# vocdoni/gnark-crypto-primitives

Hardware: AMD Instinct MI355X
Metric: proofs/sec, Arbo-160 Poseidon SMT-verifier circuit, Groth16/BN254 (higher is better)
Workload: dtype u32x8 Montgomery (254-bit integer)

## Files before the change

gnark_crypto_primitives_amd/csrc/api.hip:

```cpp
#include <algorithm>

#include "zkmi_internal.h"
#include "ff29.h"
#include "ec29.h"

using namespace zk;

namespace zk {

int ensure_scratch(zkmi_ctx* ctx, DevBuf& s, size_t bytes, void** out) {
  if (s.bytes < bytes) {
    if (s.p) {
      hipStreamSynchronize(ctx->stream);
      if (ctx->stream2) hipStreamSynchronize(ctx->stream2);
      if (ctx->stream3) hipStreamSynchronize(ctx->stream3);
      hipFree(s.p);
      s.p = nullptr;
      s.bytes = 0;
    }
    hipError_t e = hipMalloc(&s.p, bytes);
    if (e != hipSuccess) {
      ctx->err = "hipMalloc(" + std::to_string(bytes) + " B) failed: " + hipGetErrorString(e) +
                 " (the working set of this batch does not fit beside the MSM tables: load the key"
                 " with zkmi_pk_desc.max_batch >= the batch size, or with a table_budget_bytes cap)";
      s.p = nullptr;
      return ZKMI_ERR_OOM;
    }
    s.bytes = bytes;
  }
  if (out) *out = s.p;
  return ZKMI_OK;
}

int require_idle(zkmi_ctx* ctx) {
  if (!ctx->sets[0].pending && !ctx->sets[1].pending) return ZKMI_OK;
  ctx->err = "a submitted prove batch is in flight; collect it first";
  return ZKMI_ERR_ARG;
}

template <class P>
__global__ __launch_bounds__(256) void field_mul_kernel(const Fp<P>* a, const Fp<P>* b, Fp<P>* r,
                                                        size_t n) {
  size_t i = (size_t)blockIdx.x * blockDim.x + threadIdx.x;
  const size_t stride = (size_t)gridDim.x * blockDim.x;
  for (; i < n; i += stride) r[i] = mul(a[i], b[i]);
}

template <class P>
__global__ __launch_bounds__(256) void field_mul_bench_kernel(Fp<P>* io, int iters) {
  const size_t i = (size_t)blockIdx.x * blockDim.x + threadIdx.x;
  Fp<P> x = io[i], y = io[i];
  y.v[0] ^= 1;
  for (int k = 0; k < iters; k++) {
    x = mul(x, y);
    y = mul(y, x);
  }
  io[i] = add(x, y);
}

__global__ __launch_bounds__(256) void field_mul_bench_f29_kernel(Fq* io, int iters) {
  const size_t i = (size_t)blockIdx.x * blockDim.x + threadIdx.x;
  Fq29 x = unpack29<Fq29Params>(io[i].v), y = x;
  y.v[0] ^= 1;
  for (int k = 0; k < iters; k++) {
    x = mul(x, y);
    y = mul(y, x);
  }
  pack_canonical<Fq29Params>(io[i].v, norm(add(x, y)));
}

enum { FF29_MUL_ASM, FF29_SQR_ASM, FF29_MUL_ADD2_ASM, FF29_MUL_ASM_S, FF29_MUL, FF29_SQR,
       FF29_MUL_ADD2, FF29_MUL_ILP, FF29_WRED_PACK, FF29_PACK, FF29_N_OPS };
static constexpr int ff29_arity(int op) {
  if (op == FF29_MUL_ADD2_ASM || op == FF29_MUL_ADD2) return 4;
  if (op == FF29_SQR_ASM || op == FF29_SQR || op == FF29_WRED_PACK || op == FF29_PACK) return 1;
  return 2;
}
template <class P>
__device__ __forceinline__ F29<P> ld_raw29(const int32_t* p) {
  F29<P> r;
#pragma unroll
  for (int l = 0; l < 9; l++) r.v[l] = p[l];
  return r;
}
template <class P, int OP>
__global__ __launch_bounds__(64) void ff29_op_kernel(const int32_t* __restrict__ in,
                                                     int32_t* __restrict__ out, size_t n) {
#if defined(__HIP_DEVICE_COMPILE__)
  constexpr int AR = ff29_arity(OP);
  for (size_t w = blockIdx.x; w * 64 < n; w += gridDim.x) {
    F29<P> bs = F29<P>::zero();
    if constexpr (OP == FF29_MUL_ASM_S) bs = ld_raw29<P>(in + w * 64 * (AR * 9) + 9);
    const size_t i = w * 64 + threadIdx.x;
    if (i >= n) continue;
    const int32_t* e = in + i * (AR * 9);
    const F29<P> a = ld_raw29<P>(e);
    F29<P> r = F29<P>::zero();
    if constexpr (OP == FF29_MUL_ASM) r = mul_asm(a, ld_raw29<P>(e + 9));
    if constexpr (OP == FF29_SQR_ASM) r = sqr_asm(a);
    if constexpr (OP == FF29_MUL_ADD2_ASM)
      r = mul_add2_asm(a, ld_raw29<P>(e + 9), ld_raw29<P>(e + 18), ld_raw29<P>(e + 27));
    if constexpr (OP == FF29_MUL_ASM_S) r = mul_asm_s(a, bs);
    if constexpr (OP == FF29_MUL) r = mul(a, ld_raw29<P>(e + 9));
    if constexpr (OP == FF29_SQR) r = sqr(a);
    if constexpr (OP == FF29_MUL_ADD2)
      r = mul_add2(a, ld_raw29<P>(e + 9), ld_raw29<P>(e + 18), ld_raw29<P>(e + 27));
    if constexpr (OP == FF29_MUL_ILP) r = mul_ilp(a, ld_raw29<P>(e + 9));
    if constexpr (OP == FF29_WRED_PACK || OP == FF29_PACK) {
      uint32_t img[8];
      pack_canonical<P>(img, OP == FF29_WRED_PACK ? wred(a) : a);
#pragma unroll
      for (int l = 0; l < 8; l++) r.v[l] = (int32_t)img[l];
      r.v[8] = 0;
    }
#pragma unroll
    for (int l = 0; l < 9; l++) out[i * 9 + l] = r.v[l];
  }
#endif
}
typedef void (*ff29_kernel_t)(const int32_t*, int32_t*, size_t);
template <class P, int OP = 0>
static ff29_kernel_t ff29_kernel(int op) {
  if constexpr (OP < FF29_N_OPS)
    return op == OP ? ff29_op_kernel<P, OP> : ff29_kernel<P, OP + 1>(op);
  else
    return nullptr;
}

struct PkConsts {
  G1Affine alpha, beta1;
  G2Affine beta2;
};
struct ProofOut {
  G1Affine ar, krs;
  G2Affine bs;
};

__global__ __launch_bounds__(64) void rs_prep_kernel(Fr* rs, size_t Bp) {
  const size_t i = (size_t)blockIdx.x * blockDim.x + threadIdx.x;
  if (i >= Bp) return;
  bi_st(rs, 2, i, Bp, neg(mul(bi_ld(rs, 0, i, Bp), bi_ld(rs, 1, i, Bp))));
}

__device__ __forceinline__ void dbl29(G1Acc29& acc) {
  if (acc.inf) return;
  const Fq29 u = norm(add(acc.y, acc.y));
  const Fq29 v = msqr(u);
  const Fq29 w = mmul(u, v);
  const Fq29 s = mmul(acc.x, v);
  const Fq29 x2 = msqr(acc.x);
  const Fq29 m = norm(add(add(x2, x2), x2));
  const Fq29 x3 = norm(sub(msqr(m), add(s, s)));
  const Fq29 y3 = norm(sub(mmul(m, sub(s, x3)), mmul(w, acc.y)));
  acc.zz = mmul(v, acc.zz);
  acc.zzz = mmul(w, acc.zzz);
  acc.x = x3;
  acc.y = y3;
}

__global__ __launch_bounds__(64) void assemble_kernel(const G1XYZZ* sA, const G1XYZZ* sB1,
                                                      const G1XYZZ* sK, const G1XYZZ* sZ,
                                                      const G1XYZZ* tR, const G1XYZZ* tS,
                                                      const G1XYZZ* tNRS, const Fr* rs, size_t Bp,
                                                      PkConsts pk, ProofOut* out) {
  const size_t i = (size_t)blockIdx.x * blockDim.x + threadIdx.x;
  if (i >= Bp) return;
  const Fr r = from_mont(bi_ld(rs, 0, i, Bp)), s = from_mont(bi_ld(rs, 1, i, Bp));
  G1XYZZ AR = sA[i];
  madd(AR, pk.alpha);
  padd(AR, tR[i]);
  const G1Affine ar = to_affine(AR);
  G1XYZZ BS1 = sB1[i];
  madd(BS1, pk.beta1);
  padd(BS1, tS[i]);
  const G1Affine bs1 = to_affine(BS1);
  const bool ar_fin = !ar.is_inf(), bs_fin = !bs1.is_inf();
  const Fq29 ax = from_std<Fq29Params>(ar.x), ay = from_std<Fq29Params>(ar.y);
  const Fq29 bx = from_std<Fq29Params>(bs1.x), by = from_std<Fq29Params>(bs1.y);
  G1Acc29 acc29 = G1Acc29::infinity();
  for (int w = 7; w >= 0; w--) {
    const uint32_t sw = s.v[w], rw = r.v[w];
#pragma unroll 1
    for (int b = 31; b >= 0; b--) {
      dbl29(acc29);
      if (((sw >> b) & 1u) && ar_fin) madd29(acc29, ax, ay);
      if (((rw >> b) & 1u) && bs_fin) madd29(acc29, bx, by);
    }
  }
  G1XYZZ acc = to_std(acc29);
  padd(acc, sK[i]);
  padd(acc, sZ[i]);
  padd(acc, tNRS[i]);
  out[i].ar = ar;
  out[i].krs = to_affine(acc);
}

__global__ __launch_bounds__(64) void assemble_g2_kernel(const G2XYZZ* sB2, const G2XYZZ* tS2,
                                                         size_t Bp, G2Affine beta2, ProofOut* out) {
  const size_t i = (size_t)blockIdx.x * blockDim.x + threadIdx.x;
  if (i >= Bp) return;
  G2XYZZ BS = sB2[i];
  madd(BS, beta2);
  padd(BS, tS2[i]);
  out[i].bs = to_affine(BS);
}

struct SumsView {
  G1XYZZ *sA, *sB1, *sK, *sZ, *tR, *tS, *tNRS;
  G2XYZZ *sB2, *tS2;
  ProofOut* proofs;
  G1XYZZ* w1[4];
  G2XYZZ* w2;
  SumsView(void* base, size_t Bp) {
    char* m = (char*)base;
    sA = (G1XYZZ*)m;   m += Bp * 128;
    sB1 = (G1XYZZ*)m;  m += Bp * 128;
    sK = (G1XYZZ*)m;   m += Bp * 128;
    sZ = (G1XYZZ*)m;   m += Bp * 128;
    tR = (G1XYZZ*)m;   m += Bp * 128;
    tS = (G1XYZZ*)m;   m += Bp * 128;
    tNRS = (G1XYZZ*)m; m += Bp * 128;
    sB2 = (G2XYZZ*)m;  m += Bp * 256;
    tS2 = (G2XYZZ*)m;  m += Bp * 256;
    proofs = (ProofOut*)m;  m += Bp * 256;
    for (int i = 0; i < 4; i++) {
      w1[i] = (G1XYZZ*)m;
      m += 256 * Bp * 128;
    }
    w2 = (G2XYZZ*)m;
  }
};
static size_t sums_bytes(size_t Bp) { return Bp * (7 * 128 + 2 * 256 + 256 + 256 * (4 * 128 + 256)); }

struct SetBytes {
  size_t slots, abc, misc;
};
static SetBytes prove_set_bytes(size_t value_rows, size_t n, size_t n_staged, size_t batch, size_t Bp) {
  return {value_rows * Bp * 32, n * Bp * 32, Bp * (96 + 4) + batch * (n_staged * 32 + 64)};
}

int device_view(zkmi_ctx* ctx, const void* src, size_t bytes, void* stage, const void** out) {
  *out = src;
  if (pointer_kind(src) == PTR_DEVICE) return ZKMI_OK;
  ZK_HIP(hipMemcpyAsync(stage, src, bytes, hipMemcpyHostToDevice, ctx->stream));
  *out = stage;
  return ZKMI_OK;
}

int prove_set_begin(zkmi_ctx* ctx, const zkmi_pk* pk, size_t value_rows, size_t n_staged,
                    size_t batch, const void* rs, hipStream_t* main, char** stage) {
  zkmi_ctx::ProveSet& S = ctx->sets[ctx->next_submit];
  if (S.pending) {
    ctx->err = "prove: two batches already in flight; collect one first";
    return ZKMI_ERR_ARG;
  }
  const size_t Bp = round_up(batch, 64);
  const SetBytes sb = prove_set_bytes(value_rows, (size_t)1 << pk->log_n, n_staged, batch, Bp);
  int rc;
  for (zkmi_ctx::ProveSet* T : {&ctx->sets[ctx->next_submit ^ 1], &S}) {
    if (T->pending) continue;
    if ((rc = ensure_scratch(ctx, T->slots, sb.slots)) || (rc = ensure_scratch(ctx, T->a, sb.abc)) ||
        (rc = ensure_scratch(ctx, T->b, sb.abc)) || (rc = ensure_scratch(ctx, T->c, sb.abc)) ||
        (rc = ensure_scratch(ctx, T->misc, sb.misc)) ||
        (rc = ensure_scratch(ctx, T->sums, sums_bytes(Bp))))
      return rc;
  }
  char* const staged = (char*)S.misc.p + Bp * 100;
  S.rs = S.misc.p;
  S.st = (char*)S.misc.p + Bp * 96;
  if (stage) *stage = staged;
  S.heavy_enqueued = false;
  S.batch = batch;
  S.Bp = Bp;
  S.pk = pk;
  *main = ctx->stream;
  ctx->stream = ctx->stream2;
  hipEventRecord(S.ev0, ctx->stream);
  const void* rs_dev;
  rc = device_view(ctx, rs, batch * 64, staged + batch * n_staged * 32, &rs_dev);
  if (!rc) rc = transpose_in(ctx, rs_dev, S.rs, 2, batch, Bp, 32);
  return rc ? prove_set_end(ctx, *main, rc) : ZKMI_OK;
}

int prove_set_end(zkmi_ctx* ctx, hipStream_t main, int rc) {
  zkmi_ctx::ProveSet& S = ctx->sets[ctx->next_submit];
  hipEventRecord(S.ev1, ctx->stream);
  ctx->stream = main;
  if (rc) {
    hipStreamSynchronize(ctx->stream2);
    return rc;
  }
  S.pending = true;
  ctx->next_submit ^= 1;
  return ZKMI_OK;
}

}

extern "C" {

int zkmi_init(int device, zkmi_ctx** out) {
  if (!out) return ZKMI_ERR_ARG;
  *out = nullptr;
  int count = 0;
  if (hipGetDeviceCount(&count) != hipSuccess || count <= 0) return ZKMI_ERR_NO_DEVICE;
  if (device < 0 || device >= count) return ZKMI_ERR_ARG;
  if (hipSetDevice(device) != hipSuccess) return ZKMI_ERR_HIP;
  auto* ctx = new zkmi_ctx();
  ctx->device = device;
  if (hipStreamCreateWithFlags(&ctx->stream, hipStreamNonBlocking) != hipSuccess) {
    delete ctx;
    return ZKMI_ERR_HIP;
  }
  if (hipStreamCreateWithFlags(&ctx->stream2, hipStreamNonBlocking) != hipSuccess) {
    hipStreamDestroy(ctx->stream);
    delete ctx;
    return ZKMI_ERR_HIP;
  }
  if (hipStreamCreateWithFlags(&ctx->stream3, hipStreamNonBlocking) != hipSuccess) {
    hipStreamDestroy(ctx->stream2);
    hipStreamDestroy(ctx->stream);
    delete ctx;
    return ZKMI_ERR_HIP;
  }
  for (auto& st : ctx->sets) {
    hipEventCreate(&st.ev0);
    hipEventCreate(&st.ev1);
    for (auto& e : st.evq) hipEventCreate(&e);
    for (auto& e : st.eva) hipEventCreate(&e);
    for (auto& p : st.msm_ev) {
      hipEventCreate(&p[0]);
      hipEventCreate(&p[1]);
    }
  }
  for (auto& e : ctx->ev) hipEventCreate(&e);
  for (auto& e : ctx->part_ev) hipEventCreateWithFlags(&e, hipEventDisableTiming);
  for (auto& e : ctx->acc_ev) hipEventCreateWithFlags(&e, hipEventDisableTiming);
  ctx->plans.reserve(32);
  *out = ctx;
  return ZKMI_OK;
}

void zkmi_destroy(zkmi_ctx* ctx) {
  if (!ctx) return;
  hipSetDevice(ctx->device);
  hipStreamSynchronize(ctx->stream);
  hipStreamSynchronize(ctx->stream2);
  hipStreamSynchronize(ctx->stream3);
  for (auto& st : ctx->sets) {
    if (st.ev0) hipEventDestroy(st.ev0);
    if (st.ev1) hipEventDestroy(st.ev1);
    for (auto& e : st.evq)
      if (e) hipEventDestroy(e);
    for (auto& e : st.eva)
      if (e) hipEventDestroy(e);
    for (auto& p : st.msm_ev) {
      if (p[0]) hipEventDestroy(p[0]);
      if (p[1]) hipEventDestroy(p[1]);
    }
  }
  hipStreamDestroy(ctx->stream2);
  hipStreamDestroy(ctx->stream3);
  for (auto& p : ctx->plans) free_plan(p);
  for (auto& st : ctx->sets)
    for (DevBuf* b : {&st.slots, &st.a, &st.b, &st.c, &st.misc, &st.sums, &st.commit})
      if (b->p) hipFree(b->p);
  for (DevBuf* b : {&ctx->ntt_tmp, &ctx->build_tmp, &ctx->msm_digits, &ctx->msm_sint,
                    &ctx->msm_part[0], &ctx->msm_part[1], &ctx->side_part2, &ctx->side_part3})
    if (b->p) hipFree(b->p);
  witness_ring_free(ctx);
  for (auto& e : ctx->ev)
    if (e) hipEventDestroy(e);
  for (auto& e : ctx->part_ev)
    if (e) hipEventDestroy(e);
  for (auto& e : ctx->acc_ev)
    if (e) hipEventDestroy(e);
  hipStreamDestroy(ctx->stream);
  delete ctx;
}

const char* zkmi_last_error(zkmi_ctx* ctx) { return ctx ? ctx->err.c_str() : "null context"; }

int zkmi_sync(zkmi_ctx* ctx) {
  ZK_HIP(hipStreamSynchronize(ctx->stream));
  return ZKMI_OK;
}

void* zkmi_stream(zkmi_ctx* ctx) { return (void*)ctx->stream; }

int zkmi_field_mul(zkmi_ctx* ctx, int which, const void* a, const void* b, void* r, size_t n) {
  ZK_HIP(hipSetDevice(ctx->device));
  Staged sa(ctx), sb(ctx), sr(ctx);
  int rc;
  if ((rc = sa.in(a, n * 32)) || (rc = sb.in(b, n * 32)) || (rc = sr.out(r, n * 32))) return rc;
  if (n == 0) return ZKMI_OK;
  unsigned g = (unsigned)((n + 255) / 256);
  if (g > 8192) g = 8192;
  if (which == 0)
    hipLaunchKernelGGL((field_mul_kernel<FrParams>), dim3(g), dim3(256), 0, ctx->stream,
                       (const Fr*)sa.dev, (const Fr*)sb.dev, (Fr*)sr.dev, n);
  else
    hipLaunchKernelGGL((field_mul_kernel<FqParams>), dim3(g), dim3(256), 0, ctx->stream,
                       (const Fq*)sa.dev, (const Fq*)sb.dev, (Fq*)sr.dev, n);
  ZK_HIP(hipGetLastError());
  if ((rc = sr.finish())) return rc;
  ZK_HIP(hipStreamSynchronize(ctx->stream));
  return ZKMI_OK;
}

int zkmi_ff29_op(zkmi_ctx* ctx, int field, int op, const int32_t* in, int32_t* out, size_t n) {
  ZK_HIP(hipSetDevice(ctx->device));
  const ff29_kernel_t k = field == 0   ? ff29_kernel<Fr29Params>(op)
                          : field == 1 ? ff29_kernel<Fq29Params>(op)
                                       : nullptr;
  if (!k) {
    ctx->err = "ff29_op: field must be 0 (fr) or 1 (fq), op in [0, 9]";
    return ZKMI_ERR_ARG;
  }
  if (n == 0) return ZKMI_OK;
  Staged si(ctx), so(ctx);
  int rc;
  if ((rc = si.in(in, n * ff29_arity(op) * 36)) || (rc = so.out(out, n * 36))) return rc;
  const size_t waves = (n + 63) / 64;
  hipLaunchKernelGGL(k, dim3((unsigned)std::min(waves, (size_t)65536)), dim3(64), 0, ctx->stream,
                     (const int32_t*)si.dev, (int32_t*)so.dev, n);
  ZK_HIP(hipGetLastError());
  if ((rc = so.finish())) return rc;
  ZK_HIP(hipStreamSynchronize(ctx->stream));
  return ZKMI_OK;
}

int zkmi_field_mul_bench(zkmi_ctx* ctx, int which, size_t n_threads, int iters, double* rate) {
  ZK_HIP(hipSetDevice(ctx->device));
  int rc;
  if ((rc = require_idle(ctx))) return rc;
  n_threads = round_up(n_threads, 256);
  void* buf;
  if ((rc = ensure_scratch(ctx, ctx->sets[0].misc, n_threads * 32, &buf))) return rc;
  ZK_HIP(hipMemsetAsync(buf, 0x11, n_threads * 32, ctx->stream));
  auto launch = [&]() {
    if (which == 0)
      hipLaunchKernelGGL((field_mul_bench_kernel<FrParams>), dim3((unsigned)(n_threads / 256)),
                         dim3(256), 0, ctx->stream, (Fr*)buf, iters);
    else if (which == 2)
      hipLaunchKernelGGL(field_mul_bench_f29_kernel, dim3((unsigned)(n_threads / 256)), dim3(256),
                         0, ctx->stream, (Fq*)buf, iters);
    else
      hipLaunchKernelGGL((field_mul_bench_kernel<FqParams>), dim3((unsigned)(n_threads / 256)),
                         dim3(256), 0, ctx->stream, (Fq*)buf, iters);
  };
  launch();
  ZK_HIP(hipEventRecord(ctx->ev[6], ctx->stream));
  launch();
  ZK_HIP(hipEventRecord(ctx->ev[7], ctx->stream));
  ZK_HIP(hipEventSynchronize(ctx->ev[7]));
  float ms = 0;
  ZK_HIP(hipEventElapsedTime(&ms, ctx->ev[6], ctx->ev[7]));
  *rate = (double)n_threads * iters * 2.0 / (ms * 1e-3);
  return ZKMI_OK;
}

int zkmi_ntt_batch(zkmi_ctx* ctx, void* data, int log_n, size_t batch, int inverse, int coset) {
  ZK_HIP(hipSetDevice(ctx->device));
  int rc;
  if ((rc = require_idle(ctx))) return rc;
  if (batch == 0) return ZKMI_OK;
  NttPlan* plan;
  if ((rc = get_plan(ctx, log_n, &plan))) return rc;
  const size_t n = (size_t)1 << log_n, Bp = round_up(batch, 64);
  Staged sd(ctx), so(ctx);
  if ((rc = sd.in(data, batch * n * 32)) || (rc = so.out(data, batch * n * 32))) return rc;
  void *t0, *t1;
  if ((rc = ensure_scratch(ctx, ctx->sets[0].a, n * Bp * 32, &t0)) ||
      (rc = ensure_scratch(ctx, ctx->sets[0].b, n * Bp * 32, &t1)))
    return rc;
  if ((rc = transpose_in(ctx, sd.dev, t0, n, batch, Bp, 32))) return rc;
  if ((rc = ntt_bi(ctx, plan, (const Fr*)t0, (Fr*)t1, Bp, inverse != 0, coset != 0, n))) return rc;
  if ((rc = transpose_out(ctx, t1, so.dev, n, batch, Bp, 32))) return rc;
  if ((rc = so.finish())) return rc;
  ZK_HIP(hipStreamSynchronize(ctx->stream));
  return ZKMI_OK;
}

int zkmi_h_batch(zkmi_ctx* ctx, const void* a, const void* b, const void* c, void* h_out,
                 int log_n, size_t batch) {
  ZK_HIP(hipSetDevice(ctx->device));
  int rc;
  if ((rc = require_idle(ctx))) return rc;
  if (batch == 0) return ZKMI_OK;
  NttPlan* plan;
  if ((rc = get_plan(ctx, log_n, &plan))) return rc;
  const size_t n = (size_t)1 << log_n, Bp = round_up(batch, 64);
  Staged sa(ctx), sb(ctx), sc(ctx), sh(ctx);
  if ((rc = sa.in(a, batch * n * 32)) || (rc = sb.in(b, batch * n * 32)) ||
      (rc = sc.in(c, batch * n * 32)) || (rc = sh.out(h_out, batch * n * 32)))
    return rc;
  void* t[4];
  DevBuf* tb[4] = {&ctx->sets[0].a, &ctx->sets[0].b, &ctx->sets[0].c, &ctx->ntt_tmp};
  for (int i = 0; i < 4; i++)
    if ((rc = ensure_scratch(ctx, *tb[i], n * Bp * 32, &t[i]))) return rc;
  if ((rc = transpose_in(ctx, sa.dev, t[0], n, batch, Bp, 32)) ||
      (rc = transpose_in(ctx, sb.dev, t[1], n, batch, Bp, 32)) ||
      (rc = transpose_in(ctx, sc.dev, t[2], n, batch, Bp, 32)))
    return rc;
  Fr* h;
  if ((rc = compute_h_bi(ctx, plan, (Fr*)t[0], (Fr*)t[1], (Fr*)t[2], (Fr*)t[3], Bp, n, &h)))
    return rc;
  if ((rc = transpose_out(ctx, h, sh.dev, n, batch, Bp, 32))) return rc;
  if ((rc = sh.finish())) return rc;
  ZK_HIP(hipStreamSynchronize(ctx->stream));
  return ZKMI_OK;
}

int zkmi_ab_coset_batch(zkmi_ctx* ctx, const void* a, const void* b, void* out, int log_n,
                        size_t batch) {
  ZK_HIP(hipSetDevice(ctx->device));
  int rc;
  if ((rc = require_idle(ctx))) return rc;
  if (batch == 0) return ZKMI_OK;
  NttPlan* plan;
  if ((rc = get_plan(ctx, log_n, &plan))) return rc;
  const size_t n = (size_t)1 << log_n, Bp = round_up(batch, 64);
  Staged sa(ctx), sb(ctx), so(ctx);
  if ((rc = sa.in(a, batch * n * 32)) || (rc = sb.in(b, batch * n * 32)) ||
      (rc = so.out(out, batch * n * 32)))
    return rc;
  void* t[3];
  DevBuf* tb[3] = {&ctx->sets[0].a, &ctx->sets[0].b, &ctx->ntt_tmp};
  for (int i = 0; i < 3; i++)
    if ((rc = ensure_scratch(ctx, *tb[i], n * Bp * 32, &t[i]))) return rc;
  if ((rc = transpose_in(ctx, sa.dev, t[0], n, batch, Bp, 32)) ||
      (rc = transpose_in(ctx, sb.dev, t[1], n, batch, Bp, 32)))
    return rc;
  Fr* u;
  if ((rc = compute_ab_coset_bi(ctx, plan, (Fr*)t[0], (Fr*)t[1], (Fr*)t[2], Bp, n, &u))) return rc;
  if ((rc = transpose_out(ctx, u, so.dev, n, batch, Bp, 32))) return rc;
  if ((rc = so.finish())) return rc;
  ZK_HIP(hipStreamSynchronize(ctx->stream));
  return ZKMI_OK;
}

static int bases_load_plan(zkmi_ctx* ctx, int group, const void* bases_dev, size_t n, WinPlan plan,
                           bool may_relax, zkmi_msm_bases** out) {
  for (;;) {
    int rc = msm_bases_build(ctx, group, bases_dev, n, plan, out);
    if (rc != ZKMI_ERR_OOM || !may_relax) return rc;
    if (plan.comb) {
      if (plan.comb <= 8) return rc;
      plan = plan_comb(plan.comb - 1, plan.comb_signed != 0);
    } else if (plan.shared) {
      if (plan.bits[0] <= 4) return rc;
      plan = plan_shared(plan.bits[0] - 1);
    } else {
      if (plan.W >= 64) return rc;
      plan = plan_with_windows(plan.W + 1);
    }
  }
}

static bool window_bits_ok(int wb) {
  return wb == 0 || (wb >= 2 && wb <= 16) || (wb >= 104 && wb <= 116) ||
         (wb >= 202 && wb <= 220) || (wb >= 303 && wb <= 321);
}
static WinPlan plan_explicit(int wb) {
  return wb >= 300   ? plan_comb(wb - 300, true)
         : wb >= 200 ? plan_comb(wb - 200, false)
         : wb >= 100 ? plan_shared(wb - 100)
                     : plan_uniform(wb);
}
static double prove_working_set_bytes(uint32_t log_n, size_t n_slots, size_t n_in, size_t max_batch,
                                      size_t n_msm_max, size_t n_commitments) {
  const size_t Bp = round_up(max_batch ? max_batch : 1024, 64);
  const size_t n = (size_t)1 << log_n;
  const SetBytes sb = prove_set_bytes(n_slots, n, n_in, Bp, Bp);
  const double set = (double)(sb.slots + 3 * sb.abc + sb.misc + sums_bytes(Bp) +
                              commit_buffer_bytes(n_commitments, Bp));
  const double digits = 254.0 * (double)((n_msm_max + 15) / 16) * Bp * 4;
  const double sint = (double)n_msm_max * Bp * 32;
  const double partials = 2 * 21.0 * 254 * Bp * 256;
  const double ring = 3.0 * std::max(68e6, (double)n_in * 32 * 64);
  return 2 * set + (double)n * Bp * 32 + digits + sint + partials + ring + 2e9 + 1e9;
}
static double free_hbm_bytes() {
  size_t free_b = 0, total_b = 0;
  if (hipMemGetInfo(&free_b, &total_b) != hipSuccess) free_b = (size_t)64 << 30;
  return (double)free_b;
}
static double usable_table_bytes_standalone(size_t n) {
  const double ws = (double)n * 1024 * 32 * 2 + 254.0 * ((n + 15) / 16) * 1024 * 4 +
                    21.0 * 254 * 1024 * 256 + 3e9;
  const double usable = free_hbm_bytes() - ws;
  return usable > 0 ? usable : 0.0;
}

int zkmi_msm_bases_load(zkmi_ctx* ctx, int group, const void* bases, size_t n, int window_bits,
                        zkmi_msm_bases** out) {
  ZK_HIP(hipSetDevice(ctx->device));
  if (!out) return ZKMI_ERR_ARG;
  if (!window_bits_ok(window_bits)) {
    ctx->err = "window_bits must be 0 (auto), in [2,16], 100 + [4,16], 200 + [2,20] or 300 + [3,21]";
    return ZKMI_ERR_ARG;
  }
  Staged sb(ctx);
  int rc = sb.in(bases, n * (group == 1 ? 64 : 128));
  if (rc) return rc;
  WinPlan plan;
  if (window_bits) {
    plan = plan_explicit(window_bits);
  } else {
    const double usable = usable_table_bytes_standalone(n);
    plan = plan_windows_for_budget(n, group, (group == 1 ? 0.64 : 0.34) * usable);
    int c1, c2;
    plan_shared_for_budget(group == 1 ? n : 0, group == 2 ? n : 0, 0.9 * usable, &c1, &c2);
    const WinPlan ps = plan_shared(group == 1 ? c1 : c2);
    if (ps.W < plan.W) plan = ps;
    if (n >= 64) {
      int k1, k2;
      bool s1, s2;
      plan_comb_for_budget(group == 1 ? n : 0, group == 2 ? n : 0, 0.9 * usable, &k1, &k2, &s1, &s2);
      const int k = group == 1 ? k1 : k2;
      if ((double)COMB_W / k < (double)plan.W) plan = plan_comb(k, group == 1 ? s1 : s2);
    }
  }
  return bases_load_plan(ctx, group, sb.dev, n, plan, window_bits == 0, out);
}

void zkmi_msm_bases_free(zkmi_ctx* ctx, zkmi_msm_bases* b) {
  if (!b) return;
  if (ctx) {
    hipSetDevice(ctx->device);
    hipStreamSynchronize(ctx->stream);
  }
  if (b->table) hipFree(b->table);
  if (b->inf) hipFree(b->inf);
  delete b;
}

uint32_t zkmi_comb_min_groups_per_chunk(void) { return COMB_MIN_GROUPS_PER_CHUNK; }

int zkmi_msm_batch(zkmi_ctx* ctx, const zkmi_msm_bases* bases, const void* scalars, size_t batch,
                   void* out) {
  ZK_HIP(hipSetDevice(ctx->device));
  int rc;
  if ((rc = require_idle(ctx))) return rc;
  if (batch == 0) return ZKMI_OK;
  const size_t n = bases->n, Bp = round_up(batch, 64);
  const size_t pt = bases->group == 1 ? 64 : 128;
  Staged ss(ctx), so(ctx);
  if ((rc = ss.in(scalars, batch * n * 32)) || (rc = so.out(out, batch * pt))) return rc;
  void *sbi, *acc, *aff;
  if ((rc = ensure_scratch(ctx, ctx->sets[0].a, (n ? n : 1) * Bp * 32, &sbi)) ||
      (rc = ensure_scratch(ctx, ctx->sets[0].b, Bp * pt * 2, &acc)) ||
      (rc = ensure_scratch(ctx, ctx->sets[0].c, Bp * pt, &aff)))
    return rc;
  if ((rc = transpose_in(ctx, ss.dev, sbi, n, batch, Bp, 32))) return rc;
  if ((rc = msm_run(ctx, bases, (const Fr*)sbi, nullptr, Bp, batch, acc))) return rc;
  if ((rc = xyzz_to_affine(ctx, bases->group, acc, aff, Bp))) return rc;
  ZK_HIP(hipMemcpyAsync(so.dev, aff, batch * pt, hipMemcpyDeviceToDevice, ctx->stream));
  if ((rc = so.finish())) return rc;
  ZK_HIP(hipStreamSynchronize(ctx->stream));
  return ZKMI_OK;
}

int zkmi_fixed_base_mul(zkmi_ctx* ctx, int group, const void* base, const void* scalars, size_t n,
                        void* out) {
  ZK_HIP(hipSetDevice(ctx->device));
  int rc;
  if ((rc = require_idle(ctx))) return rc;
  if (n == 0) return ZKMI_OK;
  zkmi_msm_bases* b = nullptr;
  if ((rc = zkmi_msm_bases_load(ctx, group, base, 1, 8, &b))) return rc;
  const size_t Bp = round_up(n, 64);
  const size_t pt = group == 1 ? 64 : 128;
  Staged ss(ctx), so(ctx);
  void *sbi = nullptr, *acc = nullptr, *aff = nullptr;
  if ((rc = ss.in(scalars, n * 32)) || (rc = so.out(out, n * pt)) ||
      (rc = ensure_scratch(ctx, ctx->sets[0].a, Bp * 32, &sbi)) ||
      (rc = ensure_scratch(ctx, ctx->sets[0].b, Bp * pt * 2, &acc)) ||
      (rc = ensure_scratch(ctx, ctx->sets[0].c, Bp * pt, &aff))) {
    zkmi_msm_bases_free(ctx, b);
    return rc;
  }
  rc = transpose_in(ctx, ss.dev, sbi, 1, n, Bp, 32);
  if (!rc) rc = msm_run(ctx, b, (const Fr*)sbi, nullptr, Bp, n, acc);
  if (!rc) rc = xyzz_to_affine(ctx, group, acc, aff, Bp);
  if (!rc) {
    hipMemcpyAsync(so.dev, aff, n * pt, hipMemcpyDeviceToDevice, ctx->stream);
    rc = so.finish();
  }
  hipStreamSynchronize(ctx->stream);
  zkmi_msm_bases_free(ctx, b);
  return rc;
}

static int upload_u32(zkmi_ctx* ctx, const uint32_t* src, size_t n, uint32_t** out) {
  *out = nullptr;
  if (n == 0) return ZKMI_OK;
  ZK_HIP(hipMalloc((void**)out, n * 4));
  ZK_HIP(hipMemcpy(*out, src, n * 4, hipMemcpyDefault));
  return ZKMI_OK;
}

void zkmi_pk_free(zkmi_ctx* ctx, zkmi_pk* pk) {
  if (!pk) return;
  if (ctx) hipSetDevice(ctx->device);
  zkmi_msm_bases_free(ctx, pk->A);
  zkmi_msm_bases_free(ctx, pk->B1);
  zkmi_msm_bases_free(ctx, pk->K);
  zkmi_msm_bases_free(ctx, pk->Z);
  zkmi_msm_bases_free(ctx, pk->B2);
  zkmi_msm_bases_free(ctx, pk->D1);
  zkmi_msm_bases_free(ctx, pk->D2);
  commit_keys_free(ctx, pk);
  if (pk->idx3) hipFree(pk->idx3);
  if (pk->a_wire) hipFree(pk->a_wire);
  if (pk->b_wire) hipFree(pk->b_wire);
  if (pk->k_wire) hipFree(pk->k_wire);
  delete pk;
}

static int wires_from_infinity(zkmi_ctx* ctx, const uint8_t* inf, uint32_t n_wires, uint32_t want,
                               const char* name, std::vector<uint32_t>* out) {
  std::vector<uint8_t> host(n_wires);
  if (n_wires && hipMemcpy(host.data(), inf, n_wires, hipMemcpyDefault) != hipSuccess) {
    ctx->err = std::string("pk: cannot read ") + name;
    return ZKMI_ERR_HIP;
  }
  out->clear();
  for (uint32_t i = 0; i < n_wires; i++)
    if (!host[i]) out->push_back(i);
  if (out->size() != want) {
    ctx->err = std::string("pk: ") + name + " retains " + std::to_string(out->size()) +
               " wires but the key holds " + std::to_string(want) + " points";
    return ZKMI_ERR_ARG;
  }
  return ZKMI_OK;
}

int zkmi_pk_load(zkmi_ctx* ctx, const zkmi_pk_desc* d, zkmi_pk** out) {
  ZK_HIP(hipSetDevice(ctx->device));
  if (!d || !out) return ZKMI_ERR_ARG;
  if (d->log_n < 1 || d->log_n > 28) {
    ctx->err = "pk: log_n out of range [1,28]";
    return ZKMI_ERR_ARG;
  }
  if (d->n_z + 1 < (1u << d->log_n)) {
    ctx->err = "pk: n_z must be at least 2^log_n - 1";
    return ZKMI_ERR_ARG;
  }
  const uint32_t n_z = (1u << d->log_n) - 1;
  std::vector<uint32_t> wa, wb, wk;
  {
    int rc;
    struct { const uint32_t* p; uint32_t n; const char* name; std::vector<uint32_t>* v; } idx[3] = {
        {d->a_wire, d->n_a, "a_wire", &wa}, {d->b_wire, d->n_b, "b_wire", &wb},
        {d->k_wire, d->n_k, "k_wire", &wk}};
    for (auto& t : idx) {
      if (!t.p) continue;
      t.v->resize(t.n);
      if (t.n && hipMemcpy(t.v->data(), t.p, (size_t)t.n * 4, hipMemcpyDefault) != hipSuccess) {
        ctx->err = std::string("pk: cannot read ") + t.name;
        return ZKMI_ERR_HIP;
      }
    }
    if (!d->a_wire) {
      if (!d->infinity_a) {
        ctx->err = "pk: neither a_wire nor infinity_a given";
        return ZKMI_ERR_ARG;
      }
      if ((rc = wires_from_infinity(ctx, d->infinity_a, d->n_wires, d->n_a, "infinity_a", &wa)))
        return rc;
    }
    if (!d->b_wire) {
      if (!d->infinity_b) {
        ctx->err = "pk: neither b_wire nor infinity_b given";
        return ZKMI_ERR_ARG;
      }
      if ((rc = wires_from_infinity(ctx, d->infinity_b, d->n_wires, d->n_b, "infinity_b", &wb)))
        return rc;
    }
    if (!d->k_wire) {
      if (d->n_public < 1 || d->n_public > d->n_wires ||
          (d->n_commitments == 0 && d->n_wires - d->n_public != d->n_k)) {
        ctx->err = "pk: without k_wire, n_public must satisfy n_wires - n_public == n_k";
        return ZKMI_ERR_ARG;
      }
      std::vector<uint8_t> taken(d->n_wires, 0);
      for (uint32_t i = 0; i < d->n_commitments && d->commitments; i++) {
        const zkmi_commitment_desc& c = d->commitments[i];
        std::vector<uint32_t> pw(c.n_private);
        if (c.n_private && (!c.private_wires || hipMemcpy(pw.data(), c.private_wires, (size_t)c.n_private * 4,
                                                           hipMemcpyDefault) != hipSuccess)) {
          ctx->err = "pk: cannot read the private wires of commitment " + std::to_string(i);
          return ZKMI_ERR_ARG;
        }
        for (uint32_t w : pw)
          if (w < d->n_wires) taken[w] = 1;
        if (c.commitment_wire < d->n_wires) taken[c.commitment_wire] = 1;
      }
      wk.clear();
      for (uint32_t w = d->n_public; w < d->n_wires; w++)
        if (!taken[w]) wk.push_back(w);
      if (wk.size() != d->n_k) {
        ctx->err = "pk: n_k does not match n_wires - n_public - committed wires";
        return ZKMI_ERR_ARG;
      }
    }
    for (auto& t : idx)
      for (uint32_t w : *t.v)
        if (w >= d->n_wires) {
          ctx->err = std::string("pk: ") + t.name + " holds a wire index >= n_wires";
          return ZKMI_ERR_ARG;
        }
  }
  if (!window_bits_ok((int)d->window_bits_g1) || !window_bits_ok((int)d->window_bits_g2)) {
    ctx->err = "pk: window_bits must be 0 (auto), in [2,16], 100 + [4,16], 200 + [2,20] or 300 + [3,21]";
    return ZKMI_ERR_ARG;
  }
  if (d->msm_chunk_factor > 64) {
    ctx->err = "pk: msm_chunk_factor must be in [0,64]";
    return ZKMI_ERR_ARG;
  }
  FoldedKey fold;
  if (d->fold_r1cs) {
    const int frc = quotient_fold_key(ctx, d, wk, &fold);
    if (frc) return frc;
  }
  const uint32_t n_kb = fold.folded ? (uint32_t)fold.k_wire.size() : d->n_k;
  const uint32_t n_zb = fold.folded ? n_z + 1 : n_z;
  auto* pk = new zkmi_pk();
  pk->log_n = d->log_n;
  pk->n_wires = d->n_wires;
  pk->n_a = d->n_a;
  pk->n_b = d->n_b;
  pk->n_k = n_kb;
  pk->n_z = n_zb;
  pk->folded = fold.folded;
  pk->fold_n_constraints = fold.folded ? d->fold_r1cs->n_constraints : 0;
  pk->max_batch = d->max_batch ? d->max_batch : 1024;
  int rc;
  if ((rc = commit_keys_load(ctx, d, pk))) {
    zkmi_pk_free(ctx, pk);
    return rc;
  }
  const bool auto1 = d->window_bits_g1 == 0, auto2 = d->window_bits_g2 == 0;
  const size_t n1 = (size_t)d->n_a + d->n_b + n_kb + n_zb;
  const size_t n_msm_max = std::max(std::max((size_t)d->n_a, (size_t)d->n_b),
                                    std::max((size_t)n_kb, (size_t)n_zb));
  const size_t n_slots = d->n_slots_hint ? d->n_slots_hint : (size_t)d->n_wires + d->n_wires / 20;
  const double ws = prove_working_set_bytes(d->log_n, n_slots, d->n_wires, pk->max_batch, n_msm_max,
                                            pk->commits.size());
  double usable = free_hbm_bytes() - ws;
  if (usable < 0) usable = 0;
  if (d->table_budget_bytes && (double)d->table_budget_bytes < usable)
    usable = (double)d->table_budget_bytes;
  int sc1 = 0, sc2 = 0;
  plan_shared_for_budget(n1, d->n_b, 0.98 * usable, &sc1, &sc2);
  WinPlan p1 = auto1 ? plan_windows_for_budget(n1, 1, 0.64 * usable)
                     : plan_explicit((int)d->window_bits_g1);
  WinPlan p2 = auto2 ? plan_windows_for_budget(d->n_b, 2, 0.34 * usable)
                     : plan_explicit((int)d->window_bits_g2);
  if (auto1 && sc1 && plan_shared(sc1).W < p1.W) p1 = plan_shared(sc1);
  if (auto2 && sc2 && plan_shared(sc2).W < p2.W) p2 = plan_shared(sc2);
  if (n1 >= 4096) {
    int k1 = 0, k2 = 0;
    bool s1 = true, s2 = true;
    plan_comb_for_budget(auto1 ? n1 : 0, auto2 ? d->n_b : 0, 0.98 * usable, &k1, &k2, &s1, &s2,
                         d->sparse_witness == 0);
    if (auto1 && (double)COMB_W / k1 < (double)p1.W) p1 = plan_comb(k1, s1);
    if (auto2 && (double)COMB_W / k2 < (double)p2.W) p2 = plan_comb(k2, s2);
  }
  WinPlan p1z = p1;
  if (d->sparse_witness >= 2 && auto1 && auto2 && n1 >= 4096 && n_zb >= 4096) {
    const int kw = 12;
    const double wire_bytes =
        (double)((d->n_a + kw - 1) / kw + (d->n_b + kw - 1) / kw + (n_kb + kw - 1) / kw) *
            (double)(1u << kw) * 64.0 +
        (double)((d->n_b + kw - 1) / kw) * (double)(1u << kw) * 128.0;
    if (wire_bytes < 0.5 * usable) {
      int kz = 0, k2 = 0;
      bool sz = true, s2 = true;
      plan_comb_for_budget(n_zb, 0, 0.98 * usable - wire_bytes, &kz, &k2, &sz, &s2, true);
      p1 = plan_comb(kw, false);
      p2 = plan_comb(kw, false);
      p1z = plan_comb(kz, sz);
    }
  }
  auto load = [&](int group, const void* pts, size_t n, const WinPlan& plan, bool relax,
                  zkmi_msm_bases** out) -> int {
    Staged sb(ctx);
    int r = sb.in(pts, n * (group == 1 ? 64 : 128));
    if (r) return r;
    r = bases_load_plan(ctx, group, sb.dev, n, plan, relax, out);
    if (!r) (*out)->chunk_factor = d->msm_chunk_factor;
    return r;
  };
  if ((rc = upload_u32(ctx, wa.data(), d->n_a, &pk->a_wire)) ||
      (rc = upload_u32(ctx, wb.data(), d->n_b, &pk->b_wire)) ||
      (rc = upload_u32(ctx, fold.folded ? fold.k_wire.data() : wk.data(), n_kb, &pk->k_wire)) ||
      (rc = load(1, d->g1_a, d->n_a, p1, auto1, &pk->A)) ||
      (rc = load(1, d->g1_b, d->n_b, p1, auto1, &pk->B1)) ||
      (rc = load(1, fold.folded ? (const void*)fold.k.data() : d->g1_k, n_kb, p1, auto1, &pk->K)) ||
      (rc = load(1, fold.folded ? (const void*)fold.e.data() : d->g1_z, n_zb, p1z, auto1, &pk->Z)) ||
      (rc = load(2, d->g2_b, d->n_b, p2, auto2, &pk->B2))) {
    zkmi_pk_free(ctx, pk);
    return rc;
  }
  {
    const uint32_t idx[3] = {0, 1, 2};
    if ((rc = upload_u32(ctx, idx, 3, &pk->idx3)) ||
        (rc = zkmi_msm_bases_load(ctx, 1, d->g1_delta, 1, 8, &pk->D1)) ||
        (rc = zkmi_msm_bases_load(ctx, 2, d->g2_delta, 1, 8, &pk->D2))) {
      zkmi_pk_free(ctx, pk);
      return rc;
    }
    pk->D1->side = pk->D2->side = 2;
  }
  hipMemcpy(&pk->alpha, d->g1_alpha, 64, hipMemcpyDefault);
  hipMemcpy(&pk->beta1, d->g1_beta, 64, hipMemcpyDefault);
  hipMemcpy(&pk->delta1, d->g1_delta, 64, hipMemcpyDefault);
  hipMemcpy(&pk->beta2, d->g2_beta, 128, hipMemcpyDefault);
  hipMemcpy(&pk->delta2, d->g2_delta, 128, hipMemcpyDefault);
  *out = pk;
  return ZKMI_OK;
}

int zkmi_pk_info(const zkmi_pk* pk, uint64_t* info) {
  if (!pk || !info) return ZKMI_ERR_ARG;
  info[0] = (uint64_t)pk->Z->plan.W;
  info[1] = pk->Z->plan.per_base;
  info[2] = (uint64_t)pk->B2->plan.W;
  info[3] = pk->B2->plan.per_base;
  info[4] = pk->A->table_bytes + pk->B1->table_bytes + pk->K->table_bytes + pk->Z->table_bytes;
  info[5] = pk->B2->table_bytes;
  info[6] = pk->Z->plan.shared;
  info[7] = pk->B2->plan.shared;
  info[8] = pk->Z->plan.comb;
  info[9] = pk->B2->plan.comb;
  return ZKMI_OK;
}

int zkmi_pk_folded(const zkmi_pk* pk) { return pk && pk->folded ? 1 : 0; }

void zkmi_cs_free(zkmi_ctx* ctx, zkmi_cs* cs) {
  if (!cs) return;
  if (ctx) hipSetDevice(ctx->device);
  if (cs->program) hipFree(cs->program);
  if (cs->consts) hipFree(cs->consts);
  delete cs;
}

int zkmi_cs_load(zkmi_ctx* ctx, const zkmi_cs_desc* d, zkmi_cs** out) {
  ZK_HIP(hipSetDevice(ctx->device));
  if (!d || !out) return ZKMI_ERR_ARG;
  auto* cs = new zkmi_cs();
  const std::string err =
      vprog_validate({d->n_wires, d->n_slots, d->n_consts, d->n_constraints, d->n_rows,
                      d->lanes_per_proof},
                     d->program, &cs->commit_rows, &cs->has_emul);
  if (!err.empty()) {
    delete cs;
    ctx->err = err;
    return ZKMI_ERR_ARG;
  }
  cs->n_wires = d->n_wires;
  cs->n_public = d->n_public;
  cs->n_secret = d->n_secret;
  cs->n_constraints = d->n_constraints;
  cs->n_slots = d->n_slots;
  cs->n_rows = d->n_rows;
  cs->n_consts = d->n_consts;
  cs->lanes_per_proof = d->lanes_per_proof;
  int rc = upload_u32(ctx, d->program, (size_t)d->n_rows * (1 + d->lanes_per_proof) * 4,
                      &cs->program);
  if (rc) {
    delete cs;
    return rc;
  }
  if (d->n_consts) {
    if (hipMalloc((void**)&cs->consts, (size_t)d->n_consts * 32) != hipSuccess ||
        hipMemcpy(cs->consts, d->consts, (size_t)d->n_consts * 32, hipMemcpyDefault) !=
            hipSuccess) {
      ctx->err = "cs: constant pool upload failed";
      zkmi_cs_free(ctx, cs);
      return ZKMI_ERR_HIP;
    }
    if ((rc = array_to_f_domain(ctx, cs->consts, d->n_consts)) ||
        hipStreamSynchronize(ctx->stream) != hipSuccess) {
      zkmi_cs_free(ctx, cs);
      return rc ? rc : ZKMI_ERR_HIP;
    }
  }
  *out = cs;
  return ZKMI_OK;
}

static int stage_inputs(zkmi_ctx* ctx, const zkmi_cs* cs, const void* inputs_dev, size_t batch,
                        size_t Bp, Fr* slots) {
  const size_t n_in = cs->n_public - 1 + cs->n_secret;
  int rc = transpose_in(ctx, inputs_dev, slots + Bp, n_in, batch, Bp, 32);
  if (rc) return rc;
  return rows_to_f_domain(ctx, slots + Bp, n_in, Bp);
}

int zkmi_solve_batch(zkmi_ctx* ctx, const zkmi_cs* cs, const void* inputs, size_t batch,
                     void* wires_out, void* abc_out, int32_t* status_out) {
  ZK_HIP(hipSetDevice(ctx->device));
  int rc;
  if ((rc = require_idle(ctx))) return rc;
  if (batch == 0) return ZKMI_OK;
  if (!cs->commit_rows.empty()) {
    ctx->err = "solve_batch: this system has commitments; its commitment wires come from the "
               "proving key's Pedersen bases: use zkmi_prove_submit";
    return ZKMI_ERR_ARG;
  }
  const size_t Bp = round_up(batch, 64);
  const size_t n_in = cs->n_public - 1 + cs->n_secret;
  const size_t nc = cs->n_constraints ? cs->n_constraints : 1;
  Staged si(ctx), sw(ctx), sabc(ctx), sst(ctx);
  if ((rc = si.in(inputs, batch * n_in * 32))) return rc;
  if (wires_out && (rc = sw.out(wires_out, batch * (size_t)cs->n_wires * 32))) return rc;
  if (abc_out && (rc = sabc.out(abc_out, 3 * batch * (size_t)cs->n_constraints * 32))) return rc;
  if ((rc = sst.out(status_out, batch * 4))) return rc;
  void *slots, *a, *b, *c, *st;
  zkmi_ctx::ProveSet& S = ctx->sets[0];
  if ((rc = ensure_scratch(ctx, S.slots, (size_t)cs->n_slots * Bp * 32, &slots)) ||
      (rc = ensure_scratch(ctx, S.a, nc * Bp * 32, &a)) ||
      (rc = ensure_scratch(ctx, S.b, nc * Bp * 32, &b)) ||
      (rc = ensure_scratch(ctx, S.c, nc * Bp * 32, &c)) ||
      (rc = ensure_scratch(ctx, S.misc, Bp * 4, &st)))
    return rc;
  if ((rc = stage_inputs(ctx, cs, si.dev, batch, Bp, (Fr*)slots))) return rc;
  if ((rc = solve_bi(ctx, cs, (Fr*)slots, (Fr*)a, (Fr*)b, (Fr*)c, (int32_t*)st, Bp))) return rc;
  if (wires_out && ((rc = rows_to_std_domain(ctx, (Fr*)slots, cs->n_wires, Bp)) ||
                    (rc = transpose_out(ctx, slots, sw.dev, cs->n_wires, batch, Bp, 32))))
    return rc;
  if (abc_out) {
    if ((rc = rows_to_std_domain(ctx, (Fr*)a, cs->n_constraints, Bp)) ||
        (rc = rows_to_std_domain(ctx, (Fr*)b, cs->n_constraints, Bp)) ||
        (rc = rows_to_std_domain(ctx, (Fr*)c, cs->n_constraints, Bp)))
      return rc;
    const size_t stride = batch * (size_t)cs->n_constraints * 32;
    if ((rc = transpose_out(ctx, a, sabc.dev, cs->n_constraints, batch, Bp, 32)) ||
        (rc = transpose_out(ctx, b, (char*)sabc.dev + stride, cs->n_constraints, batch, Bp, 32)) ||
        (rc = transpose_out(ctx, c, (char*)sabc.dev + 2 * stride, cs->n_constraints, batch, Bp,
                            32)))
      return rc;
  }
  ZK_HIP(hipMemcpyAsync(sst.dev, st, batch * 4, hipMemcpyDeviceToDevice, ctx->stream));
  if ((rc = sw.finish()) || (rc = sabc.finish()) || (rc = sst.finish())) return rc;
  ZK_HIP(hipStreamSynchronize(ctx->stream));
  return ZKMI_OK;
}

int zkmi_prove_submit(zkmi_ctx* ctx, const zkmi_pk* pk, const zkmi_cs* cs, const void* inputs,
                      size_t batch, const void* rs) {
  ZK_HIP(hipSetDevice(ctx->device));
  if (batch == 0) {
    ctx->err = "prove: empty batch";
    return ZKMI_ERR_ARG;
  }
  if (pk->n_wires != cs->n_wires) {
    ctx->err = "prove: proving key and constraint system disagree on the number of wires";
    return ZKMI_ERR_ARG;
  }
  if (cs->n_constraints > (1u << pk->log_n)) {
    ctx->err = "prove: domain smaller than the number of constraints";
    return ZKMI_ERR_ARG;
  }
  if (pk->folded && cs->n_constraints != pk->fold_n_constraints) {
    ctx->err = "prove: the key was folded (zkmi_pk_desc.fold_r1cs) with a system of " +
               std::to_string(pk->fold_n_constraints) + " constraints, this one has " +
               std::to_string(cs->n_constraints);
    return ZKMI_ERR_ARG;
  }
  if (cs->commit_rows.size() != pk->commits.size()) {
    ctx->err = "prove: the constraint system has " + std::to_string(cs->commit_rows.size()) +
               " commitments, the proving key " + std::to_string(pk->commits.size());
    return ZKMI_ERR_ARG;
  }
  for (size_t i = 0; i < pk->commits.size(); i++)
    if (cs->commit_rows[i].second != pk->commits[i].wire) {
      ctx->err = "prove: commitment " + std::to_string(i) + " lands on different wires in the "
                 "constraint system and in the proving key";
      return ZKMI_ERR_ARG;
    }
  const size_t n_in = cs->n_public - 1 + cs->n_secret;
  hipStream_t main;
  char* stage;
  int rc = prove_set_begin(ctx, pk, cs->n_slots, n_in, batch, rs, &main, &stage);
  if (rc) return rc;
  zkmi_ctx::ProveSet& S = ctx->sets[ctx->next_submit];
  const size_t Bp = S.Bp;
  S.cs = cs;
  S.n_constraints = cs->n_constraints;
  S.f_domain = true;
  Fr *slots = (Fr*)S.slots.p, *a = (Fr*)S.a.p, *b = (Fr*)S.b.p, *c = (Fr*)S.c.p;
  int32_t* st = (int32_t*)S.st;
  const void* in_dev;
  rc = device_view(ctx, inputs, batch * n_in * 32, stage, &in_dev);
  if (!rc) rc = stage_inputs(ctx, cs, in_dev, batch, Bp, slots);
  if (!rc && cs->commit_rows.empty()) {
    rc = solve_bi(ctx, cs, slots, a, b, c, st, Bp);
  } else if (!rc) {
    rc = solve_init(ctx, slots, st, Bp);
    uint32_t begin = 0;
    for (size_t i = 0; !rc && i < cs->commit_rows.size(); i++) {
      rc = solve_rows(ctx, cs, slots, a, b, c, st, Bp, begin, cs->commit_rows[i].first);
      if (!rc) rc = commit_phase(ctx, S, (uint32_t)i, true);
      begin = cs->commit_rows[i].first + 1;
    }
    if (!rc) rc = solve_rows(ctx, cs, slots, a, b, c, st, Bp, begin, cs->n_rows);
    if (!rc) rc = commit_finish_submit(ctx, S);
  }
  return prove_set_end(ctx, main, rc);
}

static int enqueue_heavy(zkmi_ctx* ctx, int si) {
  zkmi_ctx::ProveSet& S = ctx->sets[si];
  const zkmi_pk* pk = S.pk;
  const bool fd = S.f_domain;
  const size_t Bp = S.Bp, batch = S.batch, n = (size_t)1 << pk->log_n;
  NttPlan* plan;
  int rc = get_plan(ctx, (int)pk->log_n, &plan);
  if (rc) return rc;
  void* t0;
  if ((rc = ensure_scratch(ctx, ctx->ntt_tmp, n * Bp * 32, &t0))) return rc;
  SumsView v(S.sums.p, Bp);
  Fr* rs_bi = (Fr*)S.rs;
  Fr* slots = (Fr*)S.slots.p;
  ZK_HIP(hipStreamWaitEvent(ctx->stream, S.ev1, 0));
  hipEventRecord(S.evq[0], ctx->stream);
  Fr* h;
  if ((rc = pk->folded ? compute_ab_coset_bi(ctx, plan, (Fr*)S.a.p, (Fr*)S.b.p, (Fr*)t0, Bp,
                                             S.n_constraints, &h, fd)
                       : compute_h_bi(ctx, plan, (Fr*)S.a.p, (Fr*)S.b.p, (Fr*)S.c.p, (Fr*)t0, Bp,
                                      S.n_constraints, &h, fd)))
    return rc;
  hipEventRecord(S.evq[1], ctx->stream);
  S.msm_ev_used = 0;
  ctx->msm_ev_set = si;
  const bool d1 = pk->Z->plan.shared || pk->Z->plan.comb;
  const bool d2 = pk->B2->plan.shared || pk->B2->plan.comb;
  hipStream_t q3 = ctx->stream3;
  if ((rc = msm_run(ctx, pk->A, slots, pk->a_wire, Bp, batch, v.sA, fd, d1 ? v.w1[0] : nullptr, q3)) ||
      (rc = msm_run(ctx, pk->B1, slots, pk->b_wire, Bp, batch, v.sB1, fd, d1 ? v.w1[1] : nullptr, q3)) ||
      (rc = msm_run(ctx, pk->K, slots, pk->k_wire, Bp, batch, v.sK, fd, d1 ? v.w1[2] : nullptr, q3)) ||
      (rc = msm_run(ctx, pk->Z, h, nullptr, Bp, batch, v.sZ, false, d1 ? v.w1[3] : nullptr, q3))) {
    ctx->msm_ev_set = -1;
    return rc;
  }
  hipEventRecord(S.evq[2], ctx->stream);
  rc = msm_run(ctx, pk->B2, slots, pk->b_wire, Bp, batch, v.sB2, fd, d2 ? v.w2 : nullptr, q3);
  ctx->msm_ev_set = -1;
  if (rc) return rc;
  hipEventRecord(S.evq[3], ctx->stream);
  {
    hipStream_t main_stream = ctx->stream;
    ZK_HIP(hipStreamWaitEvent(q3, S.ev1, 0));
    ctx->stream = q3;
    hipLaunchKernelGGL(rs_prep_kernel, dim3((unsigned)(Bp / 64)), dim3(64), 0, q3, rs_bi, Bp);
    (void)((rc = msm_run(ctx, pk->D1, rs_bi, pk->idx3 + 0, Bp, batch, v.tR)) ||
           (rc = msm_run(ctx, pk->D1, rs_bi, pk->idx3 + 1, Bp, batch, v.tS)) ||
           (rc = msm_run(ctx, pk->D1, rs_bi, pk->idx3 + 2, Bp, batch, v.tNRS)) ||
           (rc = msm_run(ctx, pk->D2, rs_bi, pk->idx3 + 1, Bp, batch, v.tS2)));
    ctx->stream = main_stream;
    if (rc) return rc;
  }
  if ((rc = commit_pok(ctx, S))) return rc;
  hipEventRecord(S.evq[4], ctx->stream);
  S.heavy_enqueued = true;
  return ZKMI_OK;
}

int zkmi_prove_collect(zkmi_ctx* ctx, void* proofs_out, int32_t* status_out) {
  return zkmi_prove_collect_ex(ctx, proofs_out, status_out, nullptr);
}

int zkmi_prove_collect_ex(zkmi_ctx* ctx, void* proofs_out, int32_t* status_out,
                          void* commitments_out) {
  ZK_HIP(hipSetDevice(ctx->device));
  const int si = ctx->next_collect;
  zkmi_ctx::ProveSet& S = ctx->sets[si];
  if (!S.pending) {
    ctx->err = "prove: nothing submitted";
    return ZKMI_ERR_ARG;
  }
  if (!S.pk->commits.empty() && !commitments_out) {
    ctx->err = "prove: this key has commitments: collect with zkmi_prove_collect_ex";
    return ZKMI_ERR_ARG;
  }
  const zkmi_pk* pk = S.pk;
  const size_t batch = S.batch, Bp = S.Bp;
  int rc;
  if (!S.heavy_enqueued && (rc = enqueue_heavy(ctx, si))) return rc;
  SumsView v(S.sums.p, Bp);
  hipStream_t q3 = ctx->stream3;
  ZK_HIP(hipStreamWaitEvent(q3, S.evq[4], 0));
  hipEventRecord(S.eva[0], q3);
  if (pk->Z->plan.shared || pk->Z->plan.comb) {
    void* ws[4] = {v.w1[0], v.w1[1], v.w1[2], v.w1[3]};
    void* os[4] = {v.sA, v.sB1, v.sK, v.sZ};
    const zkmi_msm_bases* ms[4] = {pk->A, pk->B1, pk->K, pk->Z};
    bool same = true;
    for (int i = 0; i < 3; i++)
      same = same && ms[i]->plan.bits[0] == pk->Z->plan.bits[0] &&
             ms[i]->plan.comb == pk->Z->plan.comb &&
             ms[i]->plan.comb_signed == pk->Z->plan.comb_signed;
    if (same) {
      if ((rc = msm_horner_run(ctx, q3, 4, ms, ws, os, Bp))) return rc;
    } else {
      for (int i = 0; i < 4; i++)
        if ((rc = msm_horner_run(ctx, q3, 1, ms + i, ws + i, os + i, Bp))) return rc;
    }
  }
  if (pk->B2->plan.shared || pk->B2->plan.comb) {
    void* ws[1] = {v.w2};
    void* os[1] = {v.sB2};
    const zkmi_msm_bases* ms[1] = {pk->B2};
    if ((rc = msm_horner_run(ctx, q3, 1, ms, ws, os, Bp))) return rc;
  }
  PkConsts pc{pk->alpha, pk->beta1, pk->beta2};
  hipLaunchKernelGGL(assemble_kernel, dim3((unsigned)(Bp / 64)), dim3(64), 0, q3, v.sA, v.sB1, v.sK,
                     v.sZ, v.tR, v.tS, v.tNRS, (const Fr*)S.rs, Bp, pc, v.proofs);
  hipLaunchKernelGGL(assemble_g2_kernel, dim3((unsigned)(Bp / 64)), dim3(64), 0, q3, v.sB2, v.tS2,
                     Bp, pk->beta2, v.proofs);
  ZK_HIP(hipGetLastError());
  ZK_HIP(hipMemcpyAsync(proofs_out, v.proofs, batch * 256, hipMemcpyDefault, q3));
  ZK_HIP(hipMemcpyAsync(status_out, S.st, batch * 4, hipMemcpyDefault, q3));
  if (const size_t nc = pk->commits.size()) {
    const size_t pitch = (nc + 1) * 64;
    for (size_t i = 0; i < nc; i++)
      ZK_HIP(hipMemcpy2DAsync((char*)commitments_out + i * 64, pitch,
                              (const char*)S.commit_pts + i * Bp * 64, 64, 64, batch, hipMemcpyDefault, q3));
    ZK_HIP(hipMemcpy2DAsync((char*)commitments_out + nc * 64, pitch,
                            (const char*)S.commit_pok + Bp * 128, 64, 64, batch, hipMemcpyDefault, q3));
  }
  hipEventRecord(S.eva[1], q3);
  zkmi_ctx::ProveSet& N = ctx->sets[si ^ 1];
  if (N.pending && !N.heavy_enqueued && (rc = enqueue_heavy(ctx, si ^ 1))) return rc;
  ZK_HIP(hipEventSynchronize(S.eva[1]));
  S.pending = false;
  S.heavy_enqueued = false;
  ctx->next_collect ^= 1;
  float ms = 0;
  hipEventElapsedTime(&ms, S.ev0, S.ev1);
  ctx->timings[0] = ms;
  for (int i = 0; i < 3; i++) {
    hipEventElapsedTime(&ms, S.evq[i], S.evq[i + 1]);
    ctx->timings[1 + i] = ms;
  }
  hipEventElapsedTime(&ms, S.eva[0], S.eva[1]);
  ctx->timings[4] = ms;
  hipEventElapsedTime(&ms, S.evq[0], S.evq[4]);
  ctx->timings[5] = ms;
  ctx->timings[6] = ctx->timings[7] = 0;
  for (int i = 0; i < S.msm_ev_used; i++) {
    hipEventElapsedTime(&ms, S.msm_ev[i][0], S.msm_ev[i][1]);
    ctx->timings[S.msm_ev_group[i] == 1 ? 6 : 7] += ms;
  }
  return ZKMI_OK;
}

int zkmi_prove_batch(zkmi_ctx* ctx, const zkmi_pk* pk, const zkmi_cs* cs, const void* inputs,
                     size_t batch, const void* rs, void* proofs_out, int32_t* status_out) {
  if (batch == 0) return ZKMI_OK;
  int rc;
  if ((rc = require_idle(ctx)) || (rc = zkmi_prove_submit(ctx, pk, cs, inputs, batch, rs))) return rc;
  return zkmi_prove_collect(ctx, proofs_out, status_out);
}

int zkmi_last_timings(zkmi_ctx* ctx, double* ms_out) {
  for (int i = 0; i < 8; i++) ms_out[i] = ctx->timings[i];
  return ZKMI_OK;
}

}
```

gnark_crypto_primitives_amd/csrc/msm.hip:

```cpp
#include "msm_impl.h"

namespace zk {

WinPlan plan_with_windows(int W) {
  WinPlan p;
  if (W < 16) W = 16;
  if (W > 64) W = 64;
  p.W = W;
  const int c0 = 255 / W, rem = 255 - c0 * W;
  uint32_t off = 0;
  for (int j = 0; j < W; j++) {
    p.bits[j] = (uint8_t)(j < rem ? c0 + 1 : c0);
    p.off[j] = off;
    off += 1u << (p.bits[j] - 1);
  }
  p.per_base = off;
  return p;
}
WinPlan plan_uniform(int c) {
  WinPlan p;
  p.W = (255 + c - 1) / c;
  uint32_t off = 0;
  for (int j = 0; j < p.W; j++) {
    p.bits[j] = (uint8_t)c;
    p.off[j] = off;
    off += 1u << (c - 1);
  }
  p.per_base = off;
  return p;
}
WinPlan plan_shared(int c) {
  WinPlan p;
  if (c < 4) c = 4;
  if (c > 16) c = 16;
  p.shared = 1;
  p.W = (255 + c - 1) / c;
  for (int j = 0; j < p.W; j++) {
    p.bits[j] = (uint8_t)(j + 1 < p.W ? c : 255 - (p.W - 1) * c);
    p.off[j] = 0;
  }
  p.per_base = 1u << (c - 1);
  return p;
}
WinPlan plan_comb(int k, bool signed_tables) {
  WinPlan p;
  if (k < 2) k = 2;
  if (k > 21) k = 21;
  if (!signed_tables && k > 20) k = 20;
  p.comb = (uint8_t)k;
  p.comb_signed = signed_tables ? 1 : 0;
  p.W = COMB_W + (signed_tables ? 1 : 0);
  p.per_base = 0;
  return p;
}
void plan_comb_for_budget(size_t n1, size_t n2, double usable_bytes, int* k1, int* k2, bool* sg1,
                          bool* sg2, bool allow_signed) {
  double best = 1e300;
  *k1 = *k2 = 8;
  *sg1 = *sg2 = allow_signed;
  for (int s1 = 0; s1 < (allow_signed ? 2 : 1); s1++)
    for (int s2 = 0; s2 < (allow_signed ? 2 : 1); s2++)
      for (int a = 8; a <= (s1 ? 21 : 20); a++)
        for (int b = 8; b <= (s2 ? 21 : 20); b++) {
          const double g1 = (double)((n1 + a - 1) / a), g2 = (double)((n2 + b - 1) / b);
          const double bytes = g1 * (double)(1u << (a - s1)) * 64.0 + g2 * (double)(1u << (b - s2)) * 128.0;
          if (bytes > usable_bytes) continue;
          const double cost = g1 * (s1 ? 255 * 62.8 : 254 * 61.1) + g2 * (s2 ? 255 * 178.5 : 254 * 171.6);
          if (cost < best) {
            best = cost;
            *k1 = a;
            *k2 = b;
            *sg1 = s1 != 0;
            *sg2 = s2 != 0;
          }
        }
}
void plan_shared_for_budget(size_t n1, size_t n2, double usable_bytes, int* c1, int* c2) {
  double best = 1e300;
  *c1 = *c2 = 4;
  for (int a = 4; a <= 16; a++)
    for (int b = 4; b <= 16; b++) {
      const double bytes = (double)n1 * (1u << (a - 1)) * 64.0 + (double)n2 * (1u << (b - 1)) * 128.0;
      if (bytes > usable_bytes) continue;
      const double cost = (double)n1 * ((255 + a - 1) / a) + 3.0 * (double)n2 * ((255 + b - 1) / b);
      if (cost < best) {
        best = cost;
        *c1 = a;
        *c2 = b;
      }
    }
}
WinPlan plan_windows_for_budget(size_t n_total, int group, double budget_bytes) {
  const double entry = group == 1 ? 64.0 : 128.0;
  for (int W = 16; W <= 64; W++) {
    WinPlan p = plan_with_windows(W);
    if ((double)n_total * p.per_base * entry <= budget_bytes) return p;
  }
  return plan_with_windows(64);
}

extern template int build_comb<Fq2>(zkmi_ctx*, const Affine<Fq2>*, size_t, const WinPlan&,
                                    Affine<Fq2>*, int*, Affine<Fq2>*);
extern template int build_impl<Fq2>(zkmi_ctx*, const Affine<Fq2>*, size_t, const WinPlan&,
                                    Affine<Fq2>*);
extern template int run_impl<Fq2>(zkmi_ctx*, const zkmi_msm_bases*, const Fr*, const uint32_t*,
                                  size_t, size_t, XYZZ<Fq2>*, bool, XYZZ<Fq2>*, hipStream_t);

template <class Fn>
static auto by_group(int group, Fn&& fn) {
  return group == 1 ? fn(Fq{}) : fn(Fq2{});
}

int msm_bases_build(zkmi_ctx* ctx, int group, const void* bases_dev, size_t n, const WinPlan& plan,
                    zkmi_msm_bases** out) {
  if (group != 1 && group != 2) {
    ctx->err = "group must be 1 (G1) or 2 (G2)";
    return ZKMI_ERR_ARG;
  }
  auto* b = new zkmi_msm_bases();
  b->group = group;
  b->n = n;
  b->plan = plan;
  const size_t entry = group == 1 ? sizeof(G1Affine) : sizeof(G2Affine);
  b->n_groups = plan.comb ? (n + plan.comb - 1) / plan.comb : 0;
  b->table_bytes = plan.comb ? b->n_groups * ((size_t)1 << (plan.comb - plan.comb_signed)) * entry
                             : n * (size_t)plan.per_base * entry;
  if (n == 0) {
    *out = b;
    return ZKMI_OK;
  }
  hipError_t e = hipMalloc(&b->table, b->table_bytes);
  if (e != hipSuccess) {
    (void)hipGetLastError();
    ctx->err = "hipMalloc of MSM window table failed (" + std::to_string(b->table_bytes) +
               " bytes): " + hipGetErrorString(e);
    delete b;
    return ZKMI_ERR_OOM;
  }
  if (hipMalloc(&b->inf, n) != hipSuccess) {
    (void)hipGetLastError();
    hipFree(b->table);
    delete b;
    return ZKMI_ERR_OOM;
  }
  const int rc = by_group(group, [&](auto f) {
    using F = decltype(f);
    const Affine<F>* bases = (const Affine<F>*)bases_dev;
    hipLaunchKernelGGL((msm_inf_flags<F>), dim3((unsigned)((n + 255) / 256)), dim3(256), 0,
                       ctx->stream, bases, (uint32_t)n, b->inf);
    return plan.comb ? build_comb<F>(ctx, bases, n, plan, (Affine<F>*)b->table,
                                     &b->entries_may_be_inf, &stotal_of(b, f))
                     : build_impl<F>(ctx, bases, n, plan, (Affine<F>*)b->table);
  });
  if (rc) {
    hipFree(b->table);
    hipFree(b->inf);
    delete b;
    return rc;
  }
  *out = b;
  return ZKMI_OK;
}

int msm_horner_run(zkmi_ctx* ctx, hipStream_t stream, int count,
                   const zkmi_msm_bases* const* bases, void* const* wsums, void* const* outs,
                   size_t Bp) {
  if (count < 1 || count > 4) return ZKMI_ERR_ARG;
  const WinPlan& plan = bases[0]->plan;
  by_group(bases[0]->group, [&](auto f) {
    using F = decltype(f);
    if (plan.comb) {
      HornerArgsRW<F> hw{};
      for (int i = 0; i < count; i++) {
        hw.wsum[i] = (XYZZ<F>*)wsums[i];
        hw.out[i] = (XYZZ<F>*)outs[i];
        hw.stotal[i] = stotal_of(bases[i], f);
      }
      launch_comb_horner<F>(stream, hw, count, Bp, plan);
    } else {
      HornerArgs<F> ha{};
      for (int i = 0; i < count; i++) {
        ha.wsum[i] = (const XYZZ<F>*)wsums[i];
        ha.out[i] = (XYZZ<F>*)outs[i];
      }
      hipLaunchKernelGGL((msm_horner<F>), dim3((unsigned)(Bp / 64), (unsigned)count), dim3(64), 0,
                         stream, ha, Bp, plan);
    }
  });
  ZK_HIP(hipGetLastError());
  return ZKMI_OK;
}

int msm_run(zkmi_ctx* ctx, const zkmi_msm_bases* bases, const Fr* scalars, const uint32_t* row_idx,
            size_t Bp, size_t batch, void* out_xyzz, bool scalars_f, void* wsum_out,
            hipStream_t finish_stream) {
  return by_group(bases->group, [&](auto f) -> int {
    using F = decltype(f);
    if (bases->n == 0) {
      const bool sums = wsum_out && (bases->plan.shared || bases->plan.comb);
      const size_t cnt = sums ? (size_t)bases->plan.W * Bp : Bp;
      hipLaunchKernelGGL((fill_inf<F>), dim3((unsigned)((cnt + 63) / 64)), dim3(64), 0, ctx->stream,
                         (XYZZ<F>*)(sums ? wsum_out : out_xyzz), cnt);
      ZK_HIP(hipGetLastError());
      return ZKMI_OK;
    }
    if (batch == 0 || batch > Bp) {
      ctx->err = "msm: batch must be in [1, Bp]";
      return ZKMI_ERR_ARG;
    }
    return run_impl<F>(ctx, bases, scalars, row_idx, Bp, batch, (XYZZ<F>*)out_xyzz, scalars_f,
                       (XYZZ<F>*)wsum_out, finish_stream);
  });
}

int xyzz_to_affine(zkmi_ctx* ctx, int group, const void* in, void* out, size_t n) {
  if (n == 0) return ZKMI_OK;
  by_group(group, [&](auto f) {
    using F = decltype(f);
    hipLaunchKernelGGL((xyzz_to_affine_kernel<F>), dim3((unsigned)((n + 63) / 64)), dim3(64), 0,
                       ctx->stream, (const XYZZ<F>*)in, (Affine<F>*)out, n);
  });
  ZK_HIP(hipGetLastError());
  return ZKMI_OK;
}

}
```

gnark_crypto_primitives_amd/csrc/msm_g2.hip:

```cpp
#include "msm_impl.h"

namespace zk {

template int build_comb<Fq2>(zkmi_ctx*, const Affine<Fq2>*, size_t, const WinPlan&, Affine<Fq2>*,
                             int*, Affine<Fq2>*);
template int build_impl<Fq2>(zkmi_ctx*, const Affine<Fq2>*, size_t, const WinPlan&, Affine<Fq2>*);
template int run_impl<Fq2>(zkmi_ctx*, const zkmi_msm_bases*, const Fr*, const uint32_t*, size_t,
                           size_t, XYZZ<Fq2>*, bool, XYZZ<Fq2>*, hipStream_t);

}
```

gnark_crypto_primitives_amd/csrc/msm_impl.h:

```cpp
#pragma once
#include "zkmi_internal.h"
#include "ec29.h"

namespace zk {

ZK_HD Fq to_r261_domain(const Fq& x) {
  Fq k;
#pragma unroll
  for (int i = 0; i < 8; i++) k.v[i] = Fq29Params::k261(i);
  return mul(x, k);
}
ZK_HD Fq2 to_r261_domain(const Fq2& x) { return Fq2{to_r261_domain(x.c0), to_r261_domain(x.c1)}; }

template <class F>
struct SegInv {
  F *szz, *szzz, *spre;
  size_t T;
  F pref = F::one();
  __device__ SegInv(F* scratch, uint32_t t, uint32_t T_, uint32_t seg_len)
      : szz(scratch + t), szzz(scratch + (size_t)seg_len * T_ + t),
        spre(scratch + (size_t)2 * seg_len * T_ + t), T(T_) {}
  __device__ void push(Affine<F>* seg, uint32_t d, const F& x, const F& y, const F& zz,
                       const F& zzz) {
    seg[d].x = x;
    seg[d].y = y;
    szz[d * T] = zz;
    szzz[d * T] = zzz;
    spre[d * T] = pref;
    pref = mul(pref, zzz);
  }
  __device__ void finish(Affine<F>* seg, uint32_t len) {
    F inv = inverse(pref);
    for (uint32_t d = len; d-- > 0;) {
      const F zzz = szzz[d * T];
      const F izzz = mul(inv, spre[d * T]);
      inv = mul(inv, zzz);
      const F izz = sqr(mul(izzz, szz[d * T]));
      seg[d].x = to_r261_domain(mul(seg[d].x, izz));
      seg[d].y = to_r261_domain(mul(seg[d].y, izzz));
    }
    pref = F::one();
  }
};

template <class F>
__global__ __launch_bounds__(64) void msm_build_table(const Affine<F>* __restrict__ bases,
                                                      uint64_t r0, uint64_t n_rows, WinPlan plan,
                                                      Affine<F>* __restrict__ table,
                                                      F* __restrict__ scratch, uint32_t T,
                                                      uint32_t seg_len) {
  const uint32_t t = blockIdx.x * blockDim.x + threadIdx.x;
  const uint64_t r = r0 + t;
  if (t >= T || r >= n_rows) return;
  uint32_t D;
  Affine<F>* row;
  Affine<F> Q;
  if (plan.shared) {
    D = plan.per_base;
    row = table + (size_t)r * plan.per_base;
    Q = bases[r];
  } else {
    const uint32_t i = (uint32_t)(r / (uint32_t)plan.W), j = (uint32_t)(r % (uint32_t)plan.W);
    D = 1u << (plan.bits[j] - 1);
    row = table + (size_t)i * plan.per_base + plan.off[j];
    Q = bases[i];
    if (!Q.is_inf() && j) {
      uint32_t shift = 0;
      for (uint32_t k = 0; k < j; k++) shift += plan.bits[k];
      XYZZ<F> a = XYZZ<F>::from_affine(Q);
      for (uint32_t k = 0; k < shift; k++) a = dbl(a);
      Q = to_affine(a);
    }
  }
  if (Q.is_inf()) {
    for (uint32_t d = 0; d < D; d++) row[d] = Affine<F>::inf();
    return;
  }
  SegInv<F> inv(scratch, t, T, seg_len);
  XYZZ<F> acc = XYZZ<F>::inf();
  for (uint32_t s0 = 0; s0 < D; s0 += seg_len) {
    Affine<F>* seg = row + s0;
    const uint32_t len = D - s0 < seg_len ? D - s0 : seg_len;
    for (uint32_t d = 0; d < len; d++) {
      madd(acc, Q);
      inv.push(seg, d, acc.x, acc.y, acc.zz, acc.zzz);
    }
    inv.finish(seg, len);
  }
}

template <class F> struct Acc29;
template <> struct Acc29<Fq> {
  typedef G1Acc29 type;
  static __device__ __forceinline__ void add(G1Acc29& acc, const G1Affine& e, bool negd) {
    madd29(acc, unpack29<Fq29Params>(e.x.v), cneg(unpack29<Fq29Params>(e.y.v), negd));
  }
};
template <> struct Acc29<Fq2> {
  typedef G2Acc29 type;
  static __device__ __forceinline__ void add(G2Acc29& acc, const G2Affine& e, bool negd) {
    madd29(acc, unpack2_29(e.x), cneg(unpack2_29(e.y), negd));
  }
};

template <class F> struct CombAcc;
template <> struct CombAcc<Fq> {
  static constexpr int LDS_ROWS = 1;
  typedef G1Acc29 type;
  static __device__ __forceinline__ type init(int32_t (*)[256], uint32_t) { return G1Acc29::infinity(); }
  static __device__ __forceinline__ void add(type& acc, const G1Affine& e, bool negd,
                                             int32_t (*)[256], uint32_t) {
    Acc29<Fq>::add(acc, e, negd);
  }
  static __device__ __forceinline__ Part29<Fq> result(const type& acc, int32_t (*)[256], uint32_t) {
    return pack_part(acc);
  }
};
struct G2AccL {
  Fq2_29 x, y;
  bool inf;
};
static __device__ __forceinline__ Fq2_29 lds_ld2(int32_t (*z)[256], int row0, uint32_t t) {
  Fq2_29 r;
#pragma unroll
  for (int l = 0; l < 9; l++) {
    r.c0.v[l] = z[row0 + l][t];
    r.c1.v[l] = z[row0 + 9 + l][t];
  }
  return r;
}
static __device__ __forceinline__ void lds_st2(int32_t (*z)[256], int row0, uint32_t t,
                                               const Fq2_29& a) {
#pragma unroll
  for (int l = 0; l < 9; l++) {
    z[row0 + l][t] = a.c0.v[l];
    z[row0 + 9 + l][t] = a.c1.v[l];
  }
}
template <> struct CombAcc<Fq2> {
  static constexpr int LDS_ROWS = 36;
  typedef G2AccL type;
  static __device__ __forceinline__ type init(int32_t (*)[256], uint32_t) {
    G2AccL a;
    a.x = a.y = Fq2_29::zero();
    a.inf = true;
    return a;
  }
  static __device__ __forceinline__ void add(type& acc, const G2Affine& e, bool negd,
                                             int32_t (*z)[256], uint32_t t) {
    const Fq2_29 qx = unpack2_29(e.x), qy = cneg(unpack2_29(e.y), negd);
    if (acc.inf) {
      acc.x = qx;
      acc.y = norm(qy);
      lds_st2(z, 0, t, Fq2_29::one());
      lds_st2(z, 18, t, Fq2_29::one());
      acc.inf = false;
      return;
    }
    const Fq2_29 u2 = mmul(qx, lds_ld2(z, 0, t));
    const Fq2_29 s2 = mmul(qy, lds_ld2(z, 18, t));
    const Fq2_29 p = sub(u2, acc.x);
    const Fq2_29 r = sub(s2, acc.y);
    const Fq2_29 pp = msqr(p);
    const Fq2_29 rr = msqr(r);
    if (is_zero_mulout(pp)) {
      if (is_zero_mulout(rr)) {
        G2Acc29 d;
        d.inf = false;
        mdbl29(d, qx, qy);
        acc.x = d.x;
        acc.y = d.y;
        lds_st2(z, 0, t, d.zz);
        lds_st2(z, 18, t, d.zzz);
      } else {
        acc.inf = true;
      }
      return;
    }
    const Fq2_29 ppp = mmul(p, pp);
    const Fq2_29 q = mmul(acc.x, pp);
    const Fq2_29 x3 = wred(sub(sub(rr, ppp), zk::add(q, q)));
    const Fq2_29 y3 = wred(sub(mmul(r, sub(q, x3)), mmul(acc.y, ppp)));
    uint32_t t2 = t;
    asm volatile("" : "+v"(t2));
    lds_st2(z, 0, t2, mmul(lds_ld2(z, 0, t2), pp));
    lds_st2(z, 18, t2, mmul(lds_ld2(z, 18, t2), ppp));
    acc.x = x3;
    acc.y = y3;
  }
  static __device__ __forceinline__ Part29<Fq2> result(const type& acc, int32_t (*z)[256], uint32_t t) {
    G2Acc29 a = G2Acc29::infinity();
    if (!acc.inf) {
      a.x = acc.x;
      a.y = acc.y;
      a.zz = lds_ld2(z, 0, t);
      a.zzz = lds_ld2(z, 18, t);
      a.inf = false;
    }
    return pack_part(a);
  }
};

template <class F, bool ONE_BASE>
__global__ __launch_bounds__(256) __attribute__((amdgpu_waves_per_eu(2))) void msm_accumulate(const Affine<F>* __restrict__ table,
                                                      const Fr* __restrict__ scalars,
                                                      const uint32_t* __restrict__ row_idx,
                                                      size_t Bp, uint32_t n, uint32_t per_chunk,
                                                      WinPlan plan, Part29<F>* __restrict__ partial,
                                                      Fr kmul, const uint8_t* __restrict__ inf) {
  const size_t b = (size_t)blockIdx.x * blockDim.x + threadIdx.x;
  const uint32_t chunk = blockIdx.y;
  const uint32_t i0 = chunk * per_chunk;
  uint32_t i1 = i0 + per_chunk;
  if (i1 > n) i1 = n;
  const int W = plan.W;
  typename Acc29<F>::type acc = Acc29<F>::type::infinity();
  for (uint32_t i = i0; i < i1; i++) {
    if (inf[i]) continue;
    const uint32_t row = row_idx ? row_idx[i] : i;
    Fr s = mul(bi_ld(scalars, row, b, Bp), kmul);
    if (s.is_zero()) continue;
    const Affine<F>* trow = table + (size_t)i * plan.per_base;
    uint32_t carry = 0;
    for (int j = 0; j < W; j++) {
      const int c = plan.bits[j];
      const uint32_t mask = (1u << c) - 1u;
      const uint32_t half = 1u << (c - 1);
      uint32_t d = (s.v[0] & mask) + carry;
#pragma unroll
      for (int l = 0; l < 7; l++) s.v[l] = (s.v[l] >> c) | (s.v[l + 1] << (32 - c));
      s.v[7] >>= c;
      const bool negd = d > half;
      carry = negd ? 1u : 0u;
      const uint32_t mag = negd ? (mask + 1u - d) : d;
      if (mag) {
        const Affine<F> e = trow[plan.off[j] + (mag - 1)];
        Acc29<F>::add(acc, e, negd);
      }
    }
  }
  partial[(size_t)chunk * Bp + b] = pack_part(acc);
}

static __global__ __launch_bounds__(256) void msm_digits_kernel(const Fr* __restrict__ scalars,
                                                         const uint32_t* __restrict__ row_idx,
                                                         size_t Bp, uint32_t n, WinPlan plan,
                                                         int32_t kmul32, Fr koff,
                                                         const uint8_t* __restrict__ inf,
                                                         int16_t* __restrict__ digits) {
  const size_t b = (size_t)blockIdx.x * blockDim.x + threadIdx.x;
  for (uint32_t i = blockIdx.y; i < n; i += gridDim.y) {
    if (inf[i]) {
      for (int j = 0; j < plan.W; j++) digits[((size_t)j * n + i) * Bp + b] = 0;
      continue;
    }
    const uint32_t row = row_idx ? row_idx[i] : i;
    Fr29 k = Fr29::zero();
    k.v[0] = kmul32;
    const Fr raw = bi_ld(scalars, row, b, Bp);
    Fr s;
    pack_canonical<Fr29Params>(s.v, mul(unpack29<Fr29Params>(raw.v), k));
    uint64_t cy = 0;
#pragma unroll
    for (int l = 0; l < 8; l++) {
      cy += (uint64_t)s.v[l] + koff.v[l];
      s.v[l] = (uint32_t)cy;
      cy >>= 32;
    }
    uint32_t pos = 0;
    for (int j = 0; j < plan.W; j++) {
      const uint32_t c = plan.bits[j];
      const uint32_t w = pos >> 5, sh = pos & 31u;
      uint32_t v = s.v[w] >> sh;
      if (sh && w + 1 < 8) v |= s.v[w + 1] << (32u - sh);
      const int32_t d = (int32_t)(v & ((1u << c) - 1u)) - (int32_t)(1u << (c - 1));
      digits[((size_t)j * n + i) * Bp + b] = (int16_t)d;
      pos += c;
    }
  }
}

template <class F>
__global__ __launch_bounds__(256) __attribute__((amdgpu_waves_per_eu(2))) void
msm_accumulate_shared(const Affine<F>* __restrict__ table, const int16_t* __restrict__ digits,
                      size_t Bp, uint32_t n, uint32_t per_chunk, uint32_t per_base,
                      Part29<F>* __restrict__ partial) {
  const size_t b = (size_t)blockIdx.x * blockDim.x + threadIdx.x;
  const uint32_t chunk = blockIdx.z, j = blockIdx.y;
  const uint32_t i0 = chunk * per_chunk;
  uint32_t i1 = i0 + per_chunk;
  if (i1 > n) i1 = n;
  const int16_t* dj = digits + (size_t)j * n * Bp + b;
  typename Acc29<F>::type acc = Acc29<F>::type::infinity();
  for (uint32_t i = i0; i < i1; i++) {
    const int32_t d = dj[(size_t)i * Bp];
    if (d) {
      const bool negd = d < 0;
      const uint32_t mag = (uint32_t)(negd ? -d : d);
      const Affine<F> e = table[(size_t)i * per_base + (mag - 1)];
      Acc29<F>::add(acc, e, negd);
    }
  }
  partial[((size_t)j * gridDim.z + chunk) * Bp + b] = pack_part(acc);
}

template <class F>
struct HornerArgs {
  const XYZZ<F>* wsum[4];
  XYZZ<F>* out[4];
};
template <class F>
__global__ __launch_bounds__(64) void msm_horner(HornerArgs<F> args, size_t Bp, WinPlan plan) {
  const size_t b = (size_t)blockIdx.x * blockDim.x + threadIdx.x;
  if (b >= Bp) return;
  const XYZZ<F>* __restrict__ wsum = args.wsum[blockIdx.y];
  XYZZ<F>* __restrict__ out = args.out[blockIdx.y];
  XYZZ<F> acc = wsum[(size_t)(plan.W - 1) * Bp + b];
  for (int j = plan.W - 2; j >= 0; j--) {
    const int c = plan.bits[j];
    for (int k = 0; k < c; k++)
      if (!acc.is_inf()) acc = dbl(acc);
    const XYZZ<F> p = wsum[(size_t)j * Bp + b];
    padd(acc, p);
  }
  out[b] = acc;
}

template <class F>
__global__ void comb_prep(const Affine<F>* __restrict__ bases, uint32_t n, uint32_t k,
                          uint32_t n_groups, Affine<F>* __restrict__ dpts,
                          Affine<F>* __restrict__ gsum, int twice) {
  const uint32_t g = blockIdx.x * blockDim.x + threadIdx.x;
  if (g >= n_groups) return;
  XYZZ<F> s = XYZZ<F>::inf();
  for (uint32_t t = 0; t < k; t++) {
    const size_t i = (size_t)g * k + t;
    const Affine<F> P = i < n ? bases[i] : Affine<F>::inf();
    XYZZ<F> d = s;
    d.y = neg(d.y);
    madd(d, P);
    if (twice) d = dbl(d);
    dpts[i] = to_affine(d);
    madd(s, P);
  }
  gsum[g] = to_affine(s);
}
template <class F>
__global__ void comb_total(const Affine<F>* __restrict__ gsum, uint32_t n_groups,
                           Affine<F>* __restrict__ out) {
  XYZZ<F> s = XYZZ<F>::inf();
  for (uint32_t g = 0; g < n_groups; g++) madd(s, gsum[g]);
  *out = to_affine(s);
}

template <class F, bool SIGNED>
__global__ __launch_bounds__(64) void comb_build(const Affine<F>* __restrict__ bases,
                                                 const Affine<F>* __restrict__ dpts, uint32_t n,
                                                 uint32_t k, uint64_t r0, uint64_t n_rows,
                                                 Affine<F>* __restrict__ table,
                                                 F* __restrict__ scratch, uint32_t T,
                                                 uint32_t seg_len, int* __restrict__ any_inf) {
  const uint32_t t = blockIdx.x * blockDim.x + threadIdx.x;
  const uint64_t r = r0 + t;
  if (t >= T || r >= n_rows) return;
  const uint32_t idx_bits = SIGNED ? k - 1 : k;
  const uint32_t per_group = 1u << idx_bits, segs = per_group / seg_len;
  const uint32_t g = (uint32_t)(r / segs), m0 = (uint32_t)(r % segs) * seg_len;
  Affine<F>* seg = table + (size_t)g * per_group + m0;
  XYZZ<F> acc = XYZZ<F>::inf();
  uint32_t live = 0;
  for (uint32_t i = 0; i < k; i++) {
    const size_t bi = (size_t)g * k + i;
    if (bi >= n) continue;
    const Affine<F> P = bases[bi];
    if (!P.is_inf()) live |= 1u << i;
    if (SIGNED) {
      if (i == k - 1 || ((m0 >> i) & 1u))
        madd(acc, P);
      else
        madd(acc, neg(P));
    } else if ((m0 >> i) & 1u) {
      madd(acc, P);
    }
  }
  SegInv<F> inv(scratch, t, T, seg_len);
  bool inf_seen = false;
  for (uint32_t d = 0; d < seg_len; d++) {
    const bool is_inf = acc.is_inf();
    const uint32_t m = m0 + d;
    inf_seen = inf_seen || (is_inf && (SIGNED ? live != 0 : (m != 0 && (m & ~live) == 0)));
    if (is_inf)
      inv.push(seg, d, F::zero(), F::zero(), F::one(), F::one());
    else
      inv.push(seg, d, acc.x, acc.y, acc.zz, acc.zzz);
    const uint32_t tz = (uint32_t)__builtin_ctz(m + 1);
    if (tz < idx_bits) madd(acc, dpts[(size_t)g * k + tz]);
  }
  inv.finish(seg, seg_len);
  if (inf_seen) atomicOr(any_inf, 1);
}

template <bool SIGNED>
__global__ __launch_bounds__(256) void comb_scalars_kernel(const Fr* __restrict__ scalars,
                                                           const uint32_t* __restrict__ row_idx,
                                                           size_t Bp, uint32_t n, int32_t kmul32,
                                                           const uint8_t* __restrict__ inf,
                                                           Fr* __restrict__ out, size_t batch,
                                                           uint32_t k, uint32_t* __restrict__ gvar) {
  const size_t b = (size_t)blockIdx.x * blockDim.x + threadIdx.x;
  for (uint32_t i = blockIdx.y; i < n; i += gridDim.y) {
    Fr s = Fr::zero();
    if (!inf[i]) {
      Fr29 kk = Fr29::zero();
      kk.v[0] = kmul32;
      const uint32_t row = row_idx ? row_idx[i] : i;
      const Fr raw = bi_ld(scalars, row, b, Bp);
      const Fr raw0 = bi_ld(scalars, row, 0, Bp);
      uint32_t diff = 0;
#pragma unroll
      for (int l = 0; l < 8; l++) diff |= raw.v[l] ^ raw0.v[l];
      if (__ballot(b < batch && diff != 0) != 0 && (threadIdx.x & 63u) == 0) gvar[i / k] = 1u;
      pack_canonical<Fr29Params>(s.v, mul(unpack29<Fr29Params>(raw.v), kk));
      if (SIGNED) {
        const uint32_t odd = s.v[0] & 1u;
        uint64_t cy = 0;
#pragma unroll
        for (int l = 0; l < 8; l++) {
          cy += (uint64_t)s.v[l] + (odd ? FrParams::p(l) : 0u);
          s.v[l] = (uint32_t)cy;
          cy >>= 32;
        }
#pragma unroll
        for (int l = 0; l < 7; l++) s.v[l] = (s.v[l] >> 1) | (s.v[l + 1] << 31);
        s.v[7] >>= 1;
        const uint32_t e = (s.v[0] & 1u) ^ 1u;
        s.v[0] &= ~1u;
        cy = 0;
#pragma unroll
        for (int l = 0; l < 8; l++) {
          cy += (uint64_t)s.v[l] + (l == 7 ? 0x40000000u : 0u);
          s.v[l] = (uint32_t)cy;
          cy >>= 32;
        }
#pragma unroll
        for (int l = 0; l < 7; l++) s.v[l] = (s.v[l] >> 1) | (s.v[l + 1] << 31);
        s.v[7] = (s.v[7] >> 1) | (e << 31);
      }
    }
    bi_st(out, i, b, Bp, s);
  }
}

static __global__ __launch_bounds__(1024) void comb_split_kernel(const uint32_t* __restrict__ gvar,
                                                                 uint32_t n_groups,
                                                                 uint32_t* __restrict__ vlist,
                                                                 uint32_t* __restrict__ ulist,
                                                                 uint32_t* __restrict__ vpos,
                                                                 uint32_t* __restrict__ counts) {
  __shared__ uint32_t wave_nv[16];
  const uint32_t t = threadIdx.x, lane = t & 63u, w = t >> 6;
  uint32_t nv = 0, nu = 0;
  for (uint32_t g0 = 0; g0 < n_groups; g0 += 1024) {
    const uint32_t g = g0 + t;
    const bool live = g < n_groups;
    const bool var = live && gvar[g] != 0;
    const unsigned long long vm = __ballot(var);
    if (lane == 0) wave_nv[w] = (uint32_t)__popcll(vm);
    __syncthreads();
    uint32_t before = 0, tile_nv = 0;
    for (uint32_t q = 0; q < 16; q++) {
      before += q < w ? wave_nv[q] : 0u;
      tile_nv += wave_nv[q];
    }
    const uint32_t vb = before + (uint32_t)__popcll(vm & ((1ull << lane) - 1ull));
    if (var) {
      vlist[nv + vb] = g;
      vpos[g] = nv + vb;
    } else if (live) {
      ulist[nu + t - vb] = g;
      vpos[g] = ~0u;
    }
    const uint32_t tile = n_groups - g0 < 1024u ? n_groups - g0 : 1024u;
    nv += tile_nv;
    nu += tile - tile_nv;
    __syncthreads();
  }
  if (t == 0) {
    counts[0] = nv;
    counts[1] = nu;
  }
}

template <int KMAX, bool SIGNED>
__global__ __launch_bounds__(256) void comb_digits_kernel(const Fr* __restrict__ sint, size_t Bp,
                                                          uint32_t n, uint32_t k, uint32_t n_groups,
                                                          const uint32_t* __restrict__ vpos,
                                                          uint32_t* __restrict__ digits,
                                                          uint32_t* __restrict__ d0) {
  const size_t b = (size_t)blockIdx.x * blockDim.x + threadIdx.x;
  const uint4* base = reinterpret_cast<const uint4*>(sint);
  const uint32_t low = (1u << (k - 1)) - 1u;
  for (uint32_t g = blockIdx.y; g < n_groups; g += gridDim.y) {
    const uint32_t p = vpos[g];
    const bool uni = p == ~0u;
    if (uni && (blockIdx.x != 0 || threadIdx.x >= 64)) continue;
#pragma unroll
    for (int h = 0; h < 2; h++) {
      uint4 wv[KMAX];
#pragma unroll
      for (int i = 0; i < KMAX; i++) {
        const size_t bi = (size_t)g * k + i;
        wv[i] = (i < (int)k && bi < n) ? base[(bi * 2 + h) * Bp + b] : make_uint4(0, 0, 0, 0);
      }
#pragma unroll
      for (int c = 0; c < 4; c++) {
        uint32_t m[32];
#pragma unroll
        for (int i = 0; i < 32; i++)
          m[i] = i < KMAX ? (c == 0 ? wv[i].x : c == 1 ? wv[i].y : c == 2 ? wv[i].z : wv[i].w) : 0u;
#pragma unroll
        for (int jj = 16; jj != 0; jj >>= 1) {
          const uint32_t mask = jj == 16 ? 0x0000ffffu : jj == 8 ? 0x00ff00ffu : jj == 4 ? 0x0f0f0f0fu
                                : jj == 2 ? 0x33333333u : 0x55555555u;
#pragma unroll
          for (int kk = 0; kk < 32; kk = (kk + jj + 1) & ~jj) {
            const uint32_t t = ((m[kk] >> jj) ^ m[kk + jj]) & mask;
            m[kk] ^= t << jj;
            m[kk + jj] ^= t;
          }
        }
#pragma unroll
        for (int bit = 0; bit < 32; bit++) {
          int j = (h * 4 + c) * 32 + bit;
          if (SIGNED) {
            if (j == 254) continue;
            if (j == 255) j = 254;
          } else if (j >= COMB_W) {
            break;
          }
          uint32_t idx = m[bit];
          if (SIGNED) idx = ((idx >> (k - 1)) & 1u) ? (idx & low) : ((~idx & low) | 0x80000000u);
          if (!uni)
            digits[((size_t)j * n_groups + p) * Bp + b] = idx;
          else if (b == 0)
            d0[(size_t)j * n_groups + g] = idx;
        }
      }
    }
  }
}

__host__ __device__ inline uint32_t comb_eff_chunks(uint32_t nv, uint32_t grid_chunks) {
  const uint32_t want = (nv + COMB_MIN_GROUPS_PER_CHUNK - 1) / COMB_MIN_GROUPS_PER_CHUNK;
  return want < 1 ? 1 : want > grid_chunks ? grid_chunks : want;
}

template <class F, bool CHECK_INF, bool SIGNED>
__global__ __launch_bounds__(256) __attribute__((amdgpu_waves_per_eu(2))) void
msm_accumulate_comb(const Affine<F>* __restrict__ table, const uint32_t* __restrict__ digits,
                    size_t Bp, uint32_t n_groups, const uint32_t* __restrict__ vlist,
                    const uint32_t* __restrict__ counts, uint32_t per_group,
                    Part29<F>* __restrict__ partial) {
  const uint32_t chunk = blockIdx.z, j = blockIdx.y;
  const uint32_t nv = counts[0];
  const uint32_t eff = comb_eff_chunks(nv, gridDim.z);
  if (chunk >= eff) return;
  const size_t b = (size_t)blockIdx.x * blockDim.x + threadIdx.x;
  const uint32_t per_chunk = (nv + eff - 1) / eff;
  const uint32_t p0 = chunk * per_chunk;
  uint32_t p1 = p0 + per_chunk;
  if (p1 > nv) p1 = nv;
  const uint32_t* dj = digits + (size_t)j * n_groups * Bp + b;
  __shared__ int32_t zl[CombAcc<F>::LDS_ROWS][256];
  const uint32_t t = threadIdx.x;
  typename CombAcc<F>::type acc = CombAcc<F>::init(zl, t);
  for (uint32_t p = p0; p < p1; p++) {
    const uint32_t m = dj[(size_t)p * Bp];
    const Affine<F>* tg = table + (size_t)vlist[p] * per_group;
    if (SIGNED) {
      const Affine<F> e = tg[m & 0x7fffffffu];
      if (CHECK_INF && e.is_inf()) continue;
      CombAcc<F>::add(acc, e, (m >> 31) != 0, zl, t);
    } else if (m) {
      const Affine<F> e = tg[m];
      if (CHECK_INF && e.is_inf()) continue;
      CombAcc<F>::add(acc, e, false, zl, t);
    }
  }
  partial[((size_t)j * gridDim.z + chunk) * Bp + b] = CombAcc<F>::result(acc, zl, t);
}

template <class T>
static __device__ __forceinline__ T shfl_xor_words(const T& x, int mask) {
  static_assert(sizeof(T) % 4 == 0, "word-sized value");
  T r;
  const uint32_t* s = reinterpret_cast<const uint32_t*>(&x);
  uint32_t* d = reinterpret_cast<uint32_t*>(&r);
#pragma unroll
  for (int i = 0; i < (int)(sizeof(T) / 4); i++) d[i] = (uint32_t)__shfl_xor((int)s[i], mask);
  return r;
}

template <class F, bool CHECK_INF, bool SIGNED>
__global__ __launch_bounds__(256) void comb_common_sums(const Affine<F>* __restrict__ table,
                                                        const uint32_t* __restrict__ d0,
                                                        uint32_t n_groups,
                                                        const uint32_t* __restrict__ ulist,
                                                        const uint32_t* __restrict__ counts,
                                                        uint32_t per_group,
                                                        Part29<F>* __restrict__ usum) {
  const uint32_t j = blockIdx.x, t = threadIdx.x;
  const uint32_t nu = counts[1];
  const uint32_t* dj = d0 + (size_t)j * n_groups;
  typename Acc29<F>::type acc = Acc29<F>::type::infinity();
  for (uint32_t c = t; c < nu; c += blockDim.x) {
    const uint32_t g = ulist[c];
    const uint32_t m = dj[g];
    if (!SIGNED && !m) continue;
    const Affine<F> e = table[(size_t)g * per_group + (SIGNED ? (m & 0x7fffffffu) : m)];
    if (CHECK_INF && e.is_inf()) continue;
    Acc29<F>::add(acc, e, SIGNED && (m >> 31) != 0);
  }
  XYZZ<F> s = to_std(acc);
#pragma unroll 1
  for (int off = 32; off > 0; off >>= 1) {
    const XYZZ<F> o = shfl_xor_words(s, off);
    padd(s, o);
  }
  constexpr int NW = (int)(sizeof(XYZZ<F>) / 4);
  __shared__ uint32_t wave_sum[4][NW];
  if ((t & 63u) == 0) {
    const uint32_t* sw = reinterpret_cast<const uint32_t*>(&s);
    for (int i = 0; i < NW; i++) wave_sum[t >> 6][i] = sw[i];
  }
  __syncthreads();
  if (t == 0) {
    for (uint32_t q = 1; q < blockDim.x / 64; q++) {
      XYZZ<F> o;
      uint32_t* ow = reinterpret_cast<uint32_t*>(&o);
      for (int i = 0; i < NW; i++) ow[i] = wave_sum[q][i];
      padd(s, o);
    }
    usum[j] = pack_part(from_std(s));
  }
}

template <class F>
struct HornerArgsRW {
  XYZZ<F>* wsum[4];
  XYZZ<F>* out[4];
  Affine<F> stotal[4];
};
template <class F>
__global__ __launch_bounds__(64) void comb_fold8(HornerArgsRW<F> args, size_t Bp, int W) {
  const size_t b = (size_t)blockIdx.x * blockDim.x + threadIdx.x;
  if (b >= Bp) return;
  XYZZ<F>* __restrict__ wsum = args.wsum[blockIdx.y];
  const int j0 = 8 * (int)blockIdx.z;
  int top = j0 + 7;
  if (top > W - 1) top = W - 1;
  XYZZ<F> acc = wsum[(size_t)top * Bp + b];
  for (int j = top - 1; j >= j0; j--) {
    acc = dbl(acc);
    const XYZZ<F> p = wsum[(size_t)j * Bp + b];
    padd(acc, p);
  }
  wsum[(size_t)j0 * Bp + b] = acc;
}
template <class F>
__global__ __launch_bounds__(64) void msm_horner_comb(HornerArgsRW<F> args, size_t Bp, int W,
                                                      int signed_tail) {
  const size_t b = (size_t)blockIdx.x * blockDim.x + threadIdx.x;
  if (b >= Bp) return;
  const XYZZ<F>* __restrict__ wsum = args.wsum[blockIdx.y];
  const int Q = (W + 7) / 8;
  XYZZ<F> acc = wsum[(size_t)(8 * (Q - 1)) * Bp + b];
  for (int q = Q - 2; q >= 0; q--) {
#pragma unroll 1
    for (int i = 0; i < 8; i++) acc = dbl(acc);
    const XYZZ<F> p = wsum[(size_t)(8 * q) * Bp + b];
    padd(acc, p);
  }
  if (signed_tail) {
    acc = dbl(acc);
    XYZZ<F> corr = wsum[(size_t)W * Bp + b];
    corr.y = neg(corr.y);
    padd(acc, corr);
    madd(acc, neg(args.stotal[blockIdx.y]));
  }
  args.out[blockIdx.y][b] = acc;
}
template <class F>
static void launch_comb_horner(hipStream_t stream, const HornerArgsRW<F>& ha, int count, size_t Bp,
                               const WinPlan& plan) {
  const int W = COMB_W;
  hipLaunchKernelGGL((comb_fold8<F>),
                     dim3((unsigned)(Bp / 64), (unsigned)count, (unsigned)((W + 7) / 8)), dim3(64), 0,
                     stream, ha, Bp, W);
  hipLaunchKernelGGL((msm_horner_comb<F>), dim3((unsigned)(Bp / 64), (unsigned)count), dim3(64), 0,
                     stream, ha, Bp, W, (int)plan.comb_signed);
}

template <class F, bool LAST>
__global__ __launch_bounds__(64) void msm_reduce(
    const Part29<F>* __restrict__ partial, size_t Bp, uint32_t chunks, uint32_t group,
    typename std::conditional<LAST, XYZZ<F>, Part29<F>>::type* __restrict__ out, size_t in_zstride,
    size_t out_zstride, const Part29<F>* __restrict__ addend, const uint32_t* __restrict__ counts,
    uint32_t grid_chunks, uint32_t div) {
  const size_t b = (size_t)blockIdx.x * blockDim.x + threadIdx.x;
  if (b >= Bp) return;
  if (counts) chunks = (comb_eff_chunks(counts[0], grid_chunks) + div - 1) / div;
  partial += (size_t)blockIdx.z * in_zstride;
  out += (size_t)blockIdx.z * out_zstride;
  const uint32_t k0 = blockIdx.y * group;
  if (k0 >= chunks) return;
  uint32_t k1 = k0 + group;
  if (k1 > chunks) k1 = chunks;
  typename Acc29<F>::type acc = unpack_part(partial[(size_t)k0 * Bp + b]);
  for (uint32_t k = k0 + 1; k < k1; k++) padd29(acc, unpack_part(partial[(size_t)k * Bp + b]));
  if (addend) padd29(acc, unpack_part(addend[blockIdx.z]));
  if constexpr (LAST)
    out[(size_t)blockIdx.y * Bp + b] = to_std(acc);
  else
    out[(size_t)blockIdx.y * Bp + b] = pack_part(acc);
}

template <class F>
__global__ __launch_bounds__(64) void xyzz_to_affine_kernel(const XYZZ<F>* __restrict__ in,
                                                            Affine<F>* __restrict__ out, size_t n) {
  const size_t i = (size_t)blockIdx.x * blockDim.x + threadIdx.x;
  if (i >= n) return;
  out[i] = to_affine(in[i]);
}

template <class F>
__global__ void msm_inf_flags(const Affine<F>* __restrict__ bases, uint32_t n,
                              uint8_t* __restrict__ inf) {
  const uint32_t i = blockIdx.x * blockDim.x + threadIdx.x;
  if (i < n) inf[i] = bases[i].is_inf() ? 1 : 0;
}

template <class F>
__global__ void fill_inf(XYZZ<F>* out, size_t n) {
  size_t i = (size_t)blockIdx.x * blockDim.x + threadIdx.x;
  if (i < n) out[i] = XYZZ<F>::inf();
}

struct BuildSlab {
  size_t T, bytes;
};
template <class F>
static BuildSlab build_slab(uint32_t seg_len, uint64_t n_rows) {
  const size_t per_thread = (size_t)3 * seg_len * sizeof(F);
  size_t T = (size_t)2e9 / per_thread;
  if (T > n_rows) T = (size_t)n_rows;
  T = round_up(T, 64);
  if (T > 262144) T = 262144;
  return {T, per_thread * T};
}

template <class B> static auto& stotal_of(B* b, Fq) { return b->stotal1; }
template <class B> static auto& stotal_of(B* b, Fq2) { return b->stotal2; }

template <class F>
int build_comb(zkmi_ctx* ctx, const Affine<F>* bases_dev, size_t n, const WinPlan& plan,
               Affine<F>* table, int* any_inf_host, Affine<F>* stotal_host) {
  const uint32_t k = plan.comb;
  const bool sg = plan.comb_signed != 0;
  const size_t n_groups = (n + k - 1) / k;
  const uint32_t per_group = 1u << (sg ? k - 1 : k);
  const uint32_t seg_len = per_group < 512u ? per_group : 512u;
  const uint64_t n_rows = (uint64_t)n_groups * (per_group / seg_len);
  const BuildSlab slab = build_slab<F>(seg_len, n_rows);
  const size_t T = slab.T;
  void* scratch;
  const size_t dp_bytes = round_up(n_groups * k * sizeof(Affine<F>), 256);
  const size_t gs_bytes = round_up((n_groups + 1) * sizeof(Affine<F>), 256);
  int rc = ensure_scratch(ctx, ctx->build_tmp, dp_bytes + gs_bytes + 256 + slab.bytes, &scratch);
  if (rc) return rc;
  Affine<F>* dpts = (Affine<F>*)scratch;
  Affine<F>* gsum = (Affine<F>*)((char*)scratch + dp_bytes);
  int* any_inf = (int*)((char*)scratch + dp_bytes + gs_bytes);
  F* inv_scratch = (F*)((char*)scratch + dp_bytes + gs_bytes + 256);
  ZK_HIP(hipMemsetAsync(any_inf, 0, sizeof(int), ctx->stream));
  hipLaunchKernelGGL((comb_prep<F>), dim3((unsigned)((n_groups + 63) / 64)), dim3(64), 0,
                     ctx->stream, bases_dev, (uint32_t)n, k, (uint32_t)n_groups, dpts, gsum,
                     sg ? 1 : 0);
  hipLaunchKernelGGL((comb_total<F>), dim3(1), dim3(1), 0, ctx->stream, (const Affine<F>*)gsum,
                     (uint32_t)n_groups, gsum + n_groups);
  const auto build = sg ? comb_build<F, true> : comb_build<F, false>;
  for (uint64_t r0 = 0; r0 < n_rows; r0 += T)
    hipLaunchKernelGGL(build, dim3((unsigned)(T / 64)), dim3(64), 0, ctx->stream, bases_dev,
                       (const Affine<F>*)dpts, (uint32_t)n, k, r0, n_rows, table, inv_scratch,
                       (uint32_t)T, seg_len, any_inf);
  ZK_HIP(hipGetLastError());
  ZK_HIP(hipMemcpyAsync(any_inf_host, any_inf, sizeof(int), hipMemcpyDeviceToHost, ctx->stream));
  ZK_HIP(hipMemcpyAsync(stotal_host, gsum + n_groups, sizeof(Affine<F>), hipMemcpyDeviceToHost,
                        ctx->stream));
  ZK_HIP(hipStreamSynchronize(ctx->stream));
  return ZKMI_OK;
}

template <class F>
int build_impl(zkmi_ctx* ctx, const Affine<F>* bases_dev, size_t n, const WinPlan& plan,
               Affine<F>* table) {
  const uint32_t Dmax = plan.shared ? plan.per_base : 1u << (plan.bits[0] - 1);
  const uint32_t seg_len = Dmax < 512u ? Dmax : 512u;
  const uint64_t n_rows = plan.shared ? (uint64_t)n : (uint64_t)n * (uint64_t)plan.W;
  const BuildSlab slab = build_slab<F>(seg_len, n_rows);
  const size_t T = slab.T;
  void* scratch;
  int rc = ensure_scratch(ctx, ctx->build_tmp, slab.bytes, &scratch);
  if (rc) return rc;
  for (uint64_t r0 = 0; r0 < n_rows; r0 += T)
    hipLaunchKernelGGL((msm_build_table<F>), dim3((unsigned)(T / 64)), dim3(64), 0, ctx->stream,
                       bases_dev, r0, n_rows, plan, table, (F*)scratch, (uint32_t)T, seg_len);
  ZK_HIP(hipGetLastError());
  ZK_HIP(hipStreamSynchronize(ctx->stream));
  return ZKMI_OK;
}

struct ChunkSplit {
  size_t chunks;
  uint32_t per_chunk, group, ngroups;
};
static inline ChunkSplit split_chunks(size_t items, size_t want) {
  size_t chunks = want;
  if (chunks < 1) chunks = 1;
  if (chunks > items) chunks = items;
  const uint32_t per_chunk = (uint32_t)((items + chunks - 1) / chunks);
  chunks = (items + per_chunk - 1) / per_chunk;
  uint32_t group = 1;
  while ((size_t)group * group < chunks) group++;
  return {chunks, per_chunk, group, (uint32_t)((chunks + group - 1) / group)};
}

template <class F>
static void reduce_partials(hipStream_t stream, const XYZZ<F>* partial, XYZZ<F>* mid, XYZZ<F>* out,
                            size_t Bp, const ChunkSplit& cs, int W, const XYZZ<F>* addend,
                            const uint32_t* counts) {
  const Part29<F>* in = (const Part29<F>*)partial;
  uint32_t count = (uint32_t)cs.chunks, div = 1;
  if (cs.ngroups > 1) {
    hipLaunchKernelGGL((msm_reduce<F, false>), dim3((unsigned)(Bp / 64), cs.ngroups, (unsigned)W),
                       dim3(64), 0, stream, in, Bp, count, cs.group, (Part29<F>*)mid,
                       (size_t)count * Bp, (size_t)cs.ngroups * Bp, (const Part29<F>*)nullptr, counts,
                       (uint32_t)cs.chunks, div);
    in = (const Part29<F>*)mid;
    count = cs.ngroups;
    div = cs.group;
  }
  hipLaunchKernelGGL((msm_reduce<F, true>), dim3((unsigned)(Bp / 64), 1, (unsigned)W), dim3(64), 0,
                     stream, in, Bp, count, count, out, (size_t)count * Bp, Bp,
                     (const Part29<F>*)addend, counts, (uint32_t)cs.chunks, div);
}

template <class F>
struct PartView {
  XYZZ<F> *partial, *mid, *wsum, *usum;
  uint32_t* counts;
  static size_t bytes(const ChunkSplit& cs, int W, size_t Bp, bool common_sums) {
    return ((cs.chunks + cs.ngroups + 1) * W * Bp + (common_sums ? W : 0)) * sizeof(XYZZ<F>) +
           (common_sums ? 2 * sizeof(uint32_t) : 0);
  }
  PartView(void* base, const ChunkSplit& cs, int W, size_t Bp) {
    partial = (XYZZ<F>*)base;
    mid = partial + cs.chunks * W * Bp;
    wsum = mid + (size_t)cs.ngroups * W * Bp;
    usum = wsum + (size_t)W * Bp;
    counts = (uint32_t*)(usum + W);
  }
};

static inline int wait_partials_free(zkmi_ctx* ctx, int pb) {
  if (ctx->part_ev_valid[pb]) {
    ZK_HIP(hipStreamWaitEvent(ctx->stream, ctx->part_ev[pb], 0));
    ctx->part_ev_valid[pb] = false;
  }
  return ZKMI_OK;
}

static inline hipEvent_t acc_timer_begin(zkmi_ctx* ctx, const zkmi_msm_bases* bases) {
  if (ctx->msm_ev_set < 0) return nullptr;
  zkmi_ctx::ProveSet& es = ctx->sets[ctx->msm_ev_set];
  if (es.msm_ev_used >= 8) return nullptr;
  const int ev = es.msm_ev_used++;
  es.msm_ev_group[ev] = bases->group;
  hipEventRecord(es.msm_ev[ev][0], ctx->stream);
  return es.msm_ev[ev][1];
}
static inline void acc_timer_end(zkmi_ctx* ctx, hipEvent_t end) {
  if (end) hipEventRecord(end, ctx->stream);
}

template <class F>
int run_comb(zkmi_ctx* ctx, const zkmi_msm_bases* bases, const Fr* scalars, const uint32_t* row_idx,
             size_t Bp, size_t batch, XYZZ<F>* out, bool scalars_f, XYZZ<F>* wsum_out,
             hipStream_t finish_stream) {
  const size_t n = bases->n;
  const uint32_t k = bases->plan.comb;
  const bool sg = bases->plan.comb_signed != 0;
  const size_t G = bases->n_groups;
  const int W = bases->plan.W;
  const size_t comb_factor = bases->chunk_factor ? bases->chunk_factor : 16;
  const ChunkSplit cs = split_chunks(G, comb_factor * 262144 / Bp / (size_t)W);
  void *part, *digits, *sint;
  const bool defer = wsum_out && finish_stream && finish_stream != ctx->stream;
  const int pb = defer ? (int)(ctx->part_next++ & 1u) : 0;
  int rc = ensure_scratch(ctx, ctx->msm_part[pb], PartView<F>::bytes(cs, W, Bp, true), &part);
  if (rc) return rc;
  if ((rc = wait_partials_free(ctx, pb))) return rc;
  if ((rc = ensure_scratch(ctx, ctx->msm_digits,
                           ((size_t)W * G * Bp + (size_t)(W + 4) * G) * sizeof(uint32_t),
                           &digits)))
    return rc;
  if ((rc = ensure_scratch(ctx, ctx->msm_sint, n * Bp * sizeof(Fr), &sint))) return rc;
  uint32_t* d0 = (uint32_t*)digits + (size_t)W * G * Bp;
  uint32_t* gvar = d0 + (size_t)W * G;
  uint32_t* vlist = gvar + G;
  uint32_t* ulist = vlist + G;
  uint32_t* vpos = ulist + G;
  const PartView<F> pv(part, cs, W, Bp);
  uint32_t* counts = pv.counts;
  XYZZ<F>* wsum = wsum_out ? wsum_out : pv.wsum;
  const unsigned bx = (Bp % 256 == 0) ? 256 : 64;
  const dim3 sgrid((unsigned)(Bp / bx), (unsigned)(n < 16384 ? n : 16384));
  const dim3 dgrid((unsigned)(Bp / bx), (unsigned)(G < 8192 ? G : 8192));
  const int32_t km = (int32_t)(scalars_f ? 1 : 32);
  ZK_HIP(hipMemsetAsync(gvar, 0, G * sizeof(uint32_t), ctx->stream));
  hipLaunchKernelGGL((sg ? comb_scalars_kernel<true> : comb_scalars_kernel<false>), sgrid, dim3(bx), 0,
                     ctx->stream, scalars, row_idx, Bp, (uint32_t)n, km, (const uint8_t*)bases->inf,
                     (Fr*)sint, batch, k, gvar);
  hipLaunchKernelGGL(comb_split_kernel, dim3(1), dim3(1024), 0, ctx->stream, (const uint32_t*)gvar,
                     (uint32_t)G, vlist, ulist, vpos, counts);
  hipLaunchKernelGGL((sg ? comb_digits_kernel<21, true> : comb_digits_kernel<20, false>), dgrid,
                     dim3(bx), 0, ctx->stream, (const Fr*)sint, Bp, (uint32_t)n, k, (uint32_t)G,
                     (const uint32_t*)vpos, (uint32_t*)digits, d0);
  const hipEvent_t timed = acc_timer_begin(ctx, bases);
  const dim3 grid((unsigned)(Bp / bx), (unsigned)W, (unsigned)cs.chunks);
  const uint32_t per_group = 1u << (sg ? k - 1 : k);
  const bool ci = bases->entries_may_be_inf != 0;
  const auto sums = ci ? (sg ? comb_common_sums<F, true, true> : comb_common_sums<F, true, false>)
                       : (sg ? comb_common_sums<F, false, true> : comb_common_sums<F, false, false>);
  const auto accumulate =
      ci ? (sg ? msm_accumulate_comb<F, true, true> : msm_accumulate_comb<F, true, false>)
         : (sg ? msm_accumulate_comb<F, false, true> : msm_accumulate_comb<F, false, false>);
  hipLaunchKernelGGL(sums, dim3((unsigned)W), dim3(256), 0, ctx->stream,
                     (const Affine<F>*)bases->table, (const uint32_t*)d0, (uint32_t)G,
                     (const uint32_t*)ulist, (const uint32_t*)counts, per_group,
                     (Part29<F>*)pv.usum);
  hipLaunchKernelGGL(accumulate, grid, dim3(bx), 0, ctx->stream, (const Affine<F>*)bases->table,
                     (const uint32_t*)digits, Bp, (uint32_t)G, (const uint32_t*)vlist,
                     (const uint32_t*)counts, per_group, (Part29<F>*)pv.partial);
  acc_timer_end(ctx, timed);
  hipStream_t rq = ctx->stream;
  if (defer) {
    ZK_HIP(hipEventRecord(ctx->acc_ev[pb], ctx->stream));
    ZK_HIP(hipStreamWaitEvent(finish_stream, ctx->acc_ev[pb], 0));
    rq = finish_stream;
  }
  reduce_partials<F>(rq, pv.partial, pv.mid, wsum, Bp, cs, W, pv.usum, counts);
  if (defer) {
    ZK_HIP(hipEventRecord(ctx->part_ev[pb], finish_stream));
    ctx->part_ev_valid[pb] = true;
  }
  if (!wsum_out) {
    HornerArgsRW<F> ha{};
    ha.wsum[0] = wsum;
    ha.out[0] = out;
    ha.stotal[0] = stotal_of(bases, F{});
    launch_comb_horner<F>(ctx->stream, ha, 1, Bp, bases->plan);
  }
  ZK_HIP(hipGetLastError());
  return ZKMI_OK;
}

template <class F>
int run_shared(zkmi_ctx* ctx, const zkmi_msm_bases* bases, const Fr* scalars,
               const uint32_t* row_idx, size_t Bp, XYZZ<F>* out, bool scalars_f,
               XYZZ<F>* wsum_out) {
  const size_t n = bases->n;
  const WinPlan& plan = bases->plan;
  const int W = plan.W;
  Fr koff = Fr::zero();
  {
    uint32_t pos = 0;
    for (int j = 0; j < W; j++) {
      const uint32_t bit = pos + plan.bits[j] - 1;
      koff.v[bit >> 5] |= 1u << (bit & 31);
      pos += plan.bits[j];
    }
  }
  const size_t shared_factor = bases->chunk_factor ? bases->chunk_factor : 8;
  const ChunkSplit cs = split_chunks(n, shared_factor * 262144 / Bp / (size_t)W);
  void *part, *digits;
  int rc = ensure_scratch(ctx, ctx->msm_part[0], PartView<F>::bytes(cs, W, Bp, false), &part);
  if (rc) return rc;
  if ((rc = wait_partials_free(ctx, 0))) return rc;
  if ((rc = ensure_scratch(ctx, ctx->msm_digits, (size_t)W * n * Bp * sizeof(int16_t), &digits)))
    return rc;
  const PartView<F> pv(part, cs, W, Bp);
  XYZZ<F>* wsum = wsum_out ? wsum_out : pv.wsum;
  const unsigned bx = (Bp % 256 == 0) ? 256 : 64;
  hipLaunchKernelGGL(msm_digits_kernel,
                     dim3((unsigned)(Bp / bx), (unsigned)(n < 16384 ? n : 16384)), dim3(bx), 0,
                     ctx->stream, scalars, row_idx, Bp, (uint32_t)n, plan,
                     (int32_t)(scalars_f ? 1 : 32), koff, (const uint8_t*)bases->inf,
                     (int16_t*)digits);
  const hipEvent_t timed = acc_timer_begin(ctx, bases);
  hipLaunchKernelGGL((msm_accumulate_shared<F>),
                     dim3((unsigned)(Bp / bx), (unsigned)W, (unsigned)cs.chunks), dim3(bx), 0,
                     ctx->stream, (const Affine<F>*)bases->table, (const int16_t*)digits, Bp,
                     (uint32_t)n, cs.per_chunk, plan.per_base, (Part29<F>*)pv.partial);
  acc_timer_end(ctx, timed);
  reduce_partials<F>(ctx->stream, pv.partial, pv.mid, wsum, Bp, cs, W, nullptr, nullptr);
  if (!wsum_out) {
    HornerArgs<F> ha{};
    ha.wsum[0] = wsum;
    ha.out[0] = out;
    hipLaunchKernelGGL((msm_horner<F>), dim3((unsigned)(Bp / 64), 1), dim3(64), 0, ctx->stream,
                       ha, Bp, plan);
  }
  ZK_HIP(hipGetLastError());
  return ZKMI_OK;
}

template <class F>
int run_windows(zkmi_ctx* ctx, const zkmi_msm_bases* bases, const Fr* scalars,
                const uint32_t* row_idx, size_t Bp, XYZZ<F>* out, bool scalars_f) {
  const size_t n = bases->n;
  Fr kmul = Fr::zero();
  kmul.v[0] = 1;
  if (scalars_f) {
    Fr t = Fr::zero();
    t.v[0] = 32;
    kmul = from_mont(inverse(to_mont(t)));
  }
  const size_t chunk_factor = bases->chunk_factor ? bases->chunk_factor : 8;
  const ChunkSplit cs = split_chunks(n, chunk_factor * (size_t)262144 / Bp);
  void* part;
  DevBuf& buf = bases->side == 2 ? ctx->side_part3 : bases->side ? ctx->side_part2 : ctx->msm_part[0];
  int rc = ensure_scratch(ctx, buf, (cs.chunks + 256) * Bp * sizeof(XYZZ<F>), &part);
  if (rc) return rc;
  if (!bases->side && (rc = wait_partials_free(ctx, 0))) return rc;
  XYZZ<F>* partial = (XYZZ<F>*)part;
  const unsigned bx = (Bp % 256 == 0) ? 256 : 64;
  const dim3 grid((unsigned)(Bp / bx), (unsigned)cs.chunks);
  const hipEvent_t timed = (bases->side || n == 1) ? nullptr : acc_timer_begin(ctx, bases);
  hipLaunchKernelGGL((n == 1 ? msm_accumulate<F, true> : msm_accumulate<F, false>), grid, dim3(bx), 0,
                     ctx->stream, (const Affine<F>*)bases->table, scalars, row_idx, Bp, (uint32_t)n,
                     cs.per_chunk, bases->plan, (Part29<F>*)partial, kmul,
                     (const uint8_t*)bases->inf);
  acc_timer_end(ctx, timed);
  reduce_partials<F>(ctx->stream, partial, partial + cs.chunks * Bp, out, Bp, cs, 1, nullptr,
                     nullptr);
  ZK_HIP(hipGetLastError());
  return ZKMI_OK;
}

template <class F>
int run_impl(zkmi_ctx* ctx, const zkmi_msm_bases* bases, const Fr* scalars,
             const uint32_t* row_idx, size_t Bp, size_t batch, XYZZ<F>* out, bool scalars_f,
             XYZZ<F>* wsum_out, hipStream_t finish_stream) {
  if (bases->plan.comb)
    return run_comb<F>(ctx, bases, scalars, row_idx, Bp, batch, out, scalars_f, wsum_out,
                       finish_stream);
  if (bases->plan.shared)
    return run_shared<F>(ctx, bases, scalars, row_idx, Bp, out, scalars_f, wsum_out);
  if (wsum_out) {
    ctx->err = "msm: deferred window sums need a shared-table plan";
    return ZKMI_ERR_ARG;
  }
  return run_windows<F>(ctx, bases, scalars, row_idx, Bp, out, scalars_f);
}

}
```

gnark_crypto_primitives_amd/csrc/zkmi_internal.h:

```cpp
#pragma once
#include <hip/hip_runtime.h>
#include <stdint.h>
#include <string>
#include <utility>
#include <vector>

#include "../../include/zkmi.h"
#include "ec.h"
#include "vprog.h"

namespace zk {


struct DevBuf {
  void* p = nullptr;
  size_t bytes = 0;
};

struct NttPlan {
  int log_n = 0;
  Fr* tw_fwd = nullptr;
  Fr* tw_inv = nullptr;
  Fr* coset_fwd = nullptr;
  Fr* coset_inv = nullptr;
  Fr* coset_inv_den = nullptr;
  Fr n_inv;
  Fr den;
  Fr ninv_den;
  Fr* tw29_fwd = nullptr;
  Fr* tw29_inv = nullptr;
  Fr* coset29_fwd = nullptr;
  Fr* coset29n_fwd = nullptr;
};

}

struct zkmi_ctx {
  int device = 0;
  hipStream_t stream = nullptr;
  std::string err;
  std::vector<zk::NttPlan> plans;
  hipEvent_t ev[8] = {};
  double timings[8] = {};
  zk::DevBuf ntt_tmp;
  zk::DevBuf build_tmp;
  zk::DevBuf msm_digits, msm_sint;
  zk::DevBuf msm_part[2];
  zk::DevBuf side_part2;
  zk::DevBuf side_part3;
  hipStream_t stream2 = nullptr, stream3 = nullptr;
  struct ProveSet {
    bool pending = false;
    bool heavy_enqueued = false;
    zk::DevBuf slots, a, b, c, misc, sums, commit;
    hipEvent_t evq[5] = {};
    hipEvent_t eva[2] = {};
    hipEvent_t msm_ev[8][2] = {};
    int msm_ev_group[8] = {};
    int msm_ev_used = 0;
    size_t batch = 0, Bp = 0;
    const zkmi_pk* pk = nullptr;
    const zkmi_cs* cs = nullptr;
    size_t n_constraints = 0;
    bool f_domain = true;
    void *rs = nullptr, *st = nullptr;
    hipEvent_t ev0 = nullptr, ev1 = nullptr;
    void *commit_pts = nullptr, *commit_ch = nullptr, *commit_pok = nullptr, *commit_acc = nullptr;
    std::vector<zk::Fr> commit_host;
  } sets[2];
  int next_submit = 0, next_collect = 0;
  int msm_ev_set = -1;
  hipEvent_t part_ev[2] = {}, acc_ev[2] = {};
  bool part_ev_valid[2] = {false, false};
  unsigned part_next = 0;
  struct StageRing {
    void* pinned[3] = {};
    void* dev[3] = {};
    hipEvent_t done[3] = {};
    bool busy[3] = {false, false, false};
    size_t bytes = 0;
    unsigned next = 0;
  } ring;
  int copy_threads = 0;
};

struct WinPlan {
  int W = 0;
  uint32_t per_base = 0;
  uint8_t bits[64] = {};
  uint32_t off[64] = {};
  uint8_t shared = 0;
  uint8_t comb = 0;
  uint8_t comb_signed = 0;
};

struct zkmi_msm_bases {
  int group = 1;
  size_t n = 0;
  WinPlan plan;
  void* table = nullptr;
  size_t table_bytes = 0;
  uint8_t* inf = nullptr;
  size_t n_groups = 0;
  int entries_may_be_inf = 0;
  uint32_t chunk_factor = 0;
  zk::G1Affine stotal1 = {};
  zk::G2Affine stotal2 = {};
  int side = 0;
};

struct zkmi_commit_key {
  uint32_t n_private = 0, n_hashed = 0, wire = 0;
  std::vector<uint32_t> hashed;
  std::vector<uint32_t> priv;
  uint32_t* private_dev = nullptr;
  zkmi_msm_bases* basis = nullptr;
  zkmi_msm_bases* sigma = nullptr;
};

struct zkmi_pk {
  uint32_t log_n = 0, n_wires = 0, n_a = 0, n_b = 0, n_k = 0, n_z = 0, max_batch = 1024;
  uint32_t *a_wire = nullptr, *b_wire = nullptr, *k_wire = nullptr;
  zkmi_msm_bases *A = nullptr, *B1 = nullptr, *K = nullptr, *Z = nullptr, *B2 = nullptr;
  zkmi_msm_bases *D1 = nullptr, *D2 = nullptr;
  uint32_t* idx3 = nullptr;
  zk::G1Affine alpha, beta1, delta1;
  zk::G2Affine beta2, delta2;
  std::vector<zkmi_commit_key> commits;
  bool folded = false;
  uint32_t fold_n_constraints = 0;
};

struct zkmi_cs {
  uint32_t n_wires = 0, n_public = 0, n_secret = 0, n_constraints = 0, n_slots = 0, n_rows = 0,
           n_consts = 0, lanes_per_proof = 1;
  uint32_t* program = nullptr;
  zk::Fr* consts = nullptr;
  std::vector<std::pair<uint32_t, uint32_t>> commit_rows;
  bool has_emul = false;
};

struct zkmi_r1cs {
  uint32_t n_wires = 0, n_constraints = 0, n_coeffs = 0;
  uint32_t* ptr[3] = {};
  uint2* terms[3] = {};
  size_t nnz[3] = {};
  zk::Fr* coeffs = nullptr;
};

namespace zk {

#if defined(__HIPCC__)
__device__ __forceinline__ Fr bi_ld(const Fr* base, size_t row, size_t b, size_t Bp) {
  const uint4* p = reinterpret_cast<const uint4*>(base) + row * 2 * Bp + b;
  const uint4 lo = p[0], hi = p[Bp];
  Fr r;
  r.v[0] = lo.x; r.v[1] = lo.y; r.v[2] = lo.z; r.v[3] = lo.w;
  r.v[4] = hi.x; r.v[5] = hi.y; r.v[6] = hi.z; r.v[7] = hi.w;
  return r;
}
__device__ __forceinline__ void bi_st(Fr* base, size_t row, size_t b, size_t Bp, const Fr& x) {
  uint4* p = reinterpret_cast<uint4*>(base) + row * 2 * Bp + b;
  p[0] = make_uint4(x.v[0], x.v[1], x.v[2], x.v[3]);
  p[Bp] = make_uint4(x.v[4], x.v[5], x.v[6], x.v[7]);
}
__device__ __forceinline__ void bi_st_nt(Fr* base, size_t row, size_t b, size_t Bp, const Fr& x) {
  typedef uint32_t u32x4 __attribute__((ext_vector_type(4)));
  u32x4* p = reinterpret_cast<u32x4*>(base) + row * 2 * Bp + b;
  u32x4 lo = {x.v[0], x.v[1], x.v[2], x.v[3]}, hi = {x.v[4], x.v[5], x.v[6], x.v[7]};
  __builtin_nontemporal_store(lo, p);
  __builtin_nontemporal_store(hi, p + Bp);
}
#endif

#define ZK_HIP(call)                                                         \
  do {                                                                       \
    hipError_t _e = (call);                                                  \
    if (_e != hipSuccess) {                                                  \
      ctx->err = std::string(#call) + ": " + hipGetErrorString(_e);          \
      return ZKMI_ERR_HIP;                                                   \
    }                                                                        \
  } while (0)

static inline size_t round_up(size_t x, size_t m) { return (x + m - 1) / m * m; }

int ensure_scratch(zkmi_ctx* ctx, DevBuf& buf, size_t bytes, void** out = nullptr);
int require_idle(zkmi_ctx* ctx);
enum { PTR_PAGEABLE = 0, PTR_PINNED = 1, PTR_DEVICE = 2 };
int pointer_kind(const void* p);
void witness_ring_free(zkmi_ctx* ctx);

struct Staged {
  zkmi_ctx* ctx;
  void* dev = nullptr;
  void* host = nullptr;
  size_t bytes = 0;
  bool owned = false;
  Staged(zkmi_ctx* c) : ctx(c) {}
  int in(const void* p, size_t n) {
    bytes = n;
    if (n == 0) return ZKMI_OK;
    if (pointer_kind(p) == PTR_DEVICE) {
      dev = const_cast<void*>(p);
      return ZKMI_OK;
    }
    ZK_HIP(hipMalloc(&dev, n));
    owned = true;
    ZK_HIP(hipMemcpyAsync(dev, p, n, hipMemcpyHostToDevice, ctx->stream));
    return ZKMI_OK;
  }
  int out(void* p, size_t n) {
    bytes = n;
    if (n == 0) return ZKMI_OK;
    if (pointer_kind(p) == PTR_DEVICE) {
      dev = p;
      return ZKMI_OK;
    }
    ZK_HIP(hipMalloc(&dev, n));
    owned = true;
    host = p;
    return ZKMI_OK;
  }
  int finish() {
    if (host && dev) {
      ZK_HIP(hipMemcpyAsync(host, dev, bytes, hipMemcpyDeviceToHost, ctx->stream));
      ZK_HIP(hipStreamSynchronize(ctx->stream));
      host = nullptr;
    }
    return ZKMI_OK;
  }
  ~Staged() {
    if (owned && dev) {
      hipStreamSynchronize(ctx->stream);
      hipFree(dev);
    }
  }
};
int device_view(zkmi_ctx* ctx, const void* src, size_t bytes, void* stage, const void** out);

int prove_set_begin(zkmi_ctx* ctx, const zkmi_pk* pk, size_t value_rows, size_t n_staged,
                    size_t batch, const void* rs, hipStream_t* main, char** stage);
int prove_set_end(zkmi_ctx* ctx, hipStream_t main, int rc);

int transpose_in(zkmi_ctx* ctx, const void* src_pm, void* dst_bi, size_t rows, size_t batch,
                 size_t Bp, size_t elem_bytes);
int transpose_out(zkmi_ctx* ctx, const void* src_bi, void* dst_pm, size_t rows, size_t batch,
                  size_t Bp, size_t elem_bytes);

int get_plan(zkmi_ctx* ctx, int log_n, NttPlan** out);
void free_plan(NttPlan& p);
int ntt_bi(zkmi_ctx* ctx, const NttPlan* plan, const Fr* src, Fr* dst, size_t Bp, bool inverse,
           bool coset, size_t n_valid);
int compute_h_bi(zkmi_ctx* ctx, const NttPlan* plan, Fr* a, Fr* b, Fr* c, Fr* t0, size_t Bp,
                 size_t n_valid, Fr** h_out, bool abc_f = false);

int compute_ab_coset_bi(zkmi_ctx* ctx, const NttPlan* plan, Fr* a, Fr* b, Fr* t0, size_t Bp,
                        size_t n_valid, Fr** u_out, bool abc_f = false);

struct FoldedKey {
  bool folded = false;
  std::vector<G1Affine> e, k;
  std::vector<uint32_t> k_wire;
};
int quotient_fold_key(zkmi_ctx* ctx, const zkmi_pk_desc* d, const std::vector<uint32_t>& k_wire,
                      FoldedKey* out);
int quotient_bases_dev(zkmi_ctx* ctx, const NttPlan* plan, const G1Affine* z_dev, uint32_t n_z,
                       G1Affine* pts);

constexpr int COMB_W = 254;
constexpr uint32_t COMB_MIN_GROUPS_PER_CHUNK = 32;
WinPlan plan_with_windows(int W);
WinPlan plan_uniform(int c);
WinPlan plan_shared(int c);
WinPlan plan_comb(int k, bool signed_tables = true);
WinPlan plan_windows_for_budget(size_t n_total, int group, double budget_bytes);
void plan_comb_for_budget(size_t n1, size_t n2, double usable_bytes, int* k1, int* k2, bool* sg1,
                          bool* sg2, bool allow_signed = true);
void plan_shared_for_budget(size_t n1, size_t n2, double usable_bytes, int* c1, int* c2);
int msm_bases_build(zkmi_ctx* ctx, int group, const void* bases_dev, size_t n, const WinPlan& plan,
                    zkmi_msm_bases** out);
int msm_run(zkmi_ctx* ctx, const zkmi_msm_bases* bases, const Fr* scalars, const uint32_t* row_idx,
            size_t Bp, size_t batch, void* out_xyzz, bool scalars_f = false,
            void* wsum_out = nullptr, hipStream_t finish_stream = nullptr);
int msm_horner_run(zkmi_ctx* ctx, hipStream_t stream, int count,
                   const zkmi_msm_bases* const* bases, void* const* wsums, void* const* outs,
                   size_t Bp);
int xyzz_to_affine(zkmi_ctx* ctx, int group, const void* in, void* out, size_t n);

int solve_bi(zkmi_ctx* ctx, const zkmi_cs* cs, Fr* slots, Fr* a, Fr* b, Fr* c, int32_t* status,
             size_t Bp);
int solve_init(zkmi_ctx* ctx, Fr* slots, int32_t* status, size_t Bp);
int solve_rows(zkmi_ctx* ctx, const zkmi_cs* cs, Fr* slots, Fr* a, Fr* b, Fr* c, int32_t* status,
               size_t Bp, uint32_t row_begin, uint32_t row_end);

size_t commit_buffer_bytes(size_t n_commitments, size_t Bp);
int commit_phase(zkmi_ctx* ctx, zkmi_ctx::ProveSet& S, uint32_t index, bool write_wire);
int commit_finish_submit(zkmi_ctx* ctx, zkmi_ctx::ProveSet& S);
int commit_pok(zkmi_ctx* ctx, zkmi_ctx::ProveSet& S);
int commit_keys_load(zkmi_ctx* ctx, const zkmi_pk_desc* d, zkmi_pk* pk);
void commit_keys_free(zkmi_ctx* ctx, zkmi_pk* pk);
int rows_to_f_domain(zkmi_ctx* ctx, Fr* base, size_t rows, size_t Bp);
int rows_to_std_domain(zkmi_ctx* ctx, Fr* base, size_t rows, size_t Bp);
int array_to_f_domain(zkmi_ctx* ctx, Fr* a, size_t n);

}
```

gnark_crypto_primitives_amd/lib.py:

```python
from __future__ import annotations

import ctypes as C
import os

import numpy as np

_HERE = os.path.dirname(os.path.abspath(__file__))
LIB_PATH = os.environ.get("ZKMI_LIB", os.path.join(_HERE, "libzkmi.so"))

ZKMI_OK = 0
ZKMI_ERR_UNSATISFIED = -5


class ZkmiError(RuntimeError):
    pass


class PkDesc(C.Structure):
    _fields_ = [("log_n", C.c_uint32), ("n_wires", C.c_uint32), ("n_a", C.c_uint32),
                ("n_b", C.c_uint32), ("n_k", C.c_uint32), ("n_z", C.c_uint32),
                ("a_wire", C.c_void_p), ("b_wire", C.c_void_p), ("k_wire", C.c_void_p),
                ("g1_a", C.c_void_p), ("g1_b", C.c_void_p), ("g1_k", C.c_void_p),
                ("g1_z", C.c_void_p), ("g2_b", C.c_void_p), ("g1_alpha", C.c_void_p),
                ("g1_beta", C.c_void_p), ("g1_delta", C.c_void_p), ("g2_beta", C.c_void_p),
                ("g2_delta", C.c_void_p), ("window_bits_g1", C.c_uint32),
                ("window_bits_g2", C.c_uint32),
                ("infinity_a", C.c_void_p), ("infinity_b", C.c_void_p), ("n_public", C.c_uint32),
                ("max_batch", C.c_uint32), ("table_budget_bytes", C.c_uint64),
                ("n_slots_hint", C.c_uint32), ("msm_chunk_factor", C.c_uint32),
                ("sparse_witness", C.c_uint32), ("n_commitments", C.c_uint32),
                ("commitments", C.c_void_p), ("fold_r1cs", C.c_void_p)]


class CommitmentDesc(C.Structure):
    _fields_ = [("n_private", C.c_uint32), ("n_hashed", C.c_uint32),
                ("commitment_wire", C.c_uint32), ("reserved", C.c_uint32),
                ("private_wires", C.c_void_p), ("hashed_wires", C.c_void_p),
                ("basis", C.c_void_p), ("basis_exp_sigma", C.c_void_p)]


class CsDesc(C.Structure):
    _fields_ = [("n_wires", C.c_uint32), ("n_public", C.c_uint32), ("n_secret", C.c_uint32),
                ("n_constraints", C.c_uint32), ("n_slots", C.c_uint32), ("n_rows", C.c_uint32),
                ("n_consts", C.c_uint32), ("lanes_per_proof", C.c_uint32), ("program", C.c_void_p),
                ("consts", C.c_void_p)]


class R1csDesc(C.Structure):
    _fields_ = [("n_wires", C.c_uint32), ("n_constraints", C.c_uint32), ("n_coeffs", C.c_uint32),
                ("coeffs", C.c_void_p), ("l_ptr", C.c_void_p), ("l_terms", C.c_void_p),
                ("r_ptr", C.c_void_p), ("r_terms", C.c_void_p), ("o_ptr", C.c_void_p),
                ("o_terms", C.c_void_p)]


class R1csSolverDesc(C.Structure):
    _fields_ = [("n_public", C.c_uint32), ("n_secret", C.c_uint32), ("n_instr", C.c_uint32),
                ("n_hints", C.c_uint32), ("instr", C.c_void_p), ("hint_kind", C.c_void_p),
                ("hint_in_ptr", C.c_void_p), ("hint_lc_ptr", C.c_void_p), ("hint_terms", C.c_void_p),
                ("hint_out_ptr", C.c_void_p), ("hint_out", C.c_void_p),
                ("lanes_per_proof", C.c_uint32), ("hint_set", C.c_uint32)]


HINTS_BASIC, HINTS_STD = 0, 1


_P, _SZ, _I = C.c_void_p, C.c_size_t, C.c_int
SYMBOLS = [
    ("zkmi_init", _I, [_I, C.POINTER(_P)]),
    ("zkmi_destroy", None, [_P]),
    ("zkmi_last_error", C.c_char_p, [_P]),
    ("zkmi_sync", _I, [_P]),
    ("zkmi_stream", _P, [_P]),
    ("zkmi_field_mul", _I, [_P, _I, _P, _P, _P, _SZ]),
    ("zkmi_ff29_op", _I, [_P, _I, _I, _P, _P, _SZ]),
    ("zkmi_field_mul_bench", _I, [_P, _I, _SZ, _I, C.POINTER(C.c_double)]),
    ("zkmi_ntt_batch", _I, [_P, _P, _I, _SZ, _I, _I]),
    ("zkmi_h_batch", _I, [_P, _P, _P, _P, _P, _I, _SZ]),
    ("zkmi_ab_coset_batch", _I, [_P, _P, _P, _P, _I, _SZ]),
    ("zkmi_quotient_bases", _I, [_P, _P, _SZ, _I, _P, _P]),
    ("zkmi_msm_bases_load", _I, [_P, _I, _P, _SZ, _I, C.POINTER(_P)]),
    ("zkmi_msm_bases_free", None, [_P, _P]),
    ("zkmi_msm_batch", _I, [_P, _P, _P, _SZ, _P]),
    ("zkmi_comb_min_groups_per_chunk", C.c_uint32, []),
    ("zkmi_fixed_base_mul", _I, [_P, _I, _P, _P, _SZ, _P]),
    ("zkmi_pk_load", _I, [_P, C.POINTER(PkDesc), C.POINTER(_P)]),
    ("zkmi_pk_free", None, [_P, _P]),
    ("zkmi_pk_info", _I, [_P, C.POINTER(C.c_uint64)]),
    ("zkmi_pk_folded", _I, [_P]),
    ("zkmi_cs_load", _I, [_P, C.POINTER(CsDesc), C.POINTER(_P)]),
    ("zkmi_cs_free", None, [_P, _P]),
    ("zkmi_solve_batch", _I, [_P, _P, _P, _SZ, _P, _P, _P]),
    ("zkmi_prove_batch", _I, [_P, _P, _P, _P, _SZ, _P, _P, _P]),
    ("zkmi_prove_submit", _I, [_P, _P, _P, _P, _SZ, _P]),
    ("zkmi_prove_collect", _I, [_P, _P, _P]),
    ("zkmi_prove_collect_ex", _I, [_P, _P, _P, _P]),
    ("zkmi_prove_witness_batch", _I, [_P, _P, _P, _P, _P, _P, _SZ, _SZ, _P, _P]),
    ("zkmi_host_alloc", _P, [_P, _SZ]),
    ("zkmi_host_free", None, [_P, _P]),
    ("zkmi_set_copy_threads", _I, [_P, _I]),
    ("zkmi_r1cs_load", _I, [_P, C.POINTER(R1csDesc), C.POINTER(_P)]),
    ("zkmi_r1cs_free", None, [_P, _P]),
    ("zkmi_prove_witness_submit", _I, [_P, _P, _P, _P, _P, _P, _P, _SZ, _SZ, _P]),
    ("zkmi_r1cs_solver_load", _I, [_P, _P, C.POINTER(R1csSolverDesc), C.POINTER(_P)]),
    ("zkmi_r1cs_solver_free", None, [_P, _P]),
    ("zkmi_r1cs_solver_info", _I, [_P, C.POINTER(C.c_uint64)]),
    ("zkmi_r1cs_solve_batch", _I, [_P, _P, _P, _SZ, _P, _P, _P]),
    ("zkmi_prove_r1cs_submit", _I, [_P, _P, _P, _P, _SZ, _P]),
    ("zkmi_last_timings", _I, [_P, C.POINTER(C.c_double)]),
    ("zkmi_plonk_pk_load", _I, [_P, _P, C.POINTER(_P)]),
    ("zkmi_plonk_pk_free", None, [_P, _P]),
    ("zkmi_plonk_round1", _I, [_P, _P, _P, _P, _SZ, _P, _P, _P]),
    ("zkmi_plonk_round2", _I, [_P, _P, _P, _P]),
    ("zkmi_plonk_round3", _I, [_P, _P, _P, _P]),
    ("zkmi_plonk_round4", _I, [_P, _P, _P, _P]),
    ("zkmi_plonk_round5", _I, [_P, _P, _P, _P]),
    ("zkmi_plonk_prove", _I, [_P, _P, _P, _P, _SZ, _P, _P, _P, _P]),
]

_lib = None


def load():
    global _lib
    if _lib is not None:
        return _lib
    if not os.path.exists(LIB_PATH):
        raise ZkmiError(f"{LIB_PATH} not found: build it with `python -c 'import __graft_entry__ as "
                        "g; g.build()'` (hipcc --offload-arch=gfx950). There is no CPU fallback.")
    lib = C.CDLL(LIB_PATH)
    for name, res, args in SYMBOLS:
        fn = getattr(lib, name)
        fn.restype = res
        fn.argtypes = args
    _lib = lib
    return lib


def _ptr(x):
    if x is None:
        return None
    if isinstance(x, np.ndarray):
        if not x.flags["C_CONTIGUOUS"]:
            raise ValueError("array must be C-contiguous")
        return x.ctypes.data
    if hasattr(x, "data_ptr"):
        if not x.is_contiguous():
            raise ValueError("tensor must be contiguous")
        return x.data_ptr()
    return int(x)


class Context:

    def __init__(self, device: int = 0):
        self.lib = load()
        h = C.c_void_p()
        rc = self.lib.zkmi_init(device, C.byref(h))
        if rc != 0:
            raise ZkmiError(f"zkmi_init(device={device}) failed with {rc} "
                            "(-3 = no HIP device: this library only runs on a GPU)")
        self.h = h
        self.device = device

    def close(self):
        if getattr(self, "h", None):
            self.lib.zkmi_destroy(self.h)
            self.h = None

    def __del__(self):
        try:
            self.close()
        except Exception:
            pass

    def _check(self, rc, what):
        if rc != 0:
            msg = self.lib.zkmi_last_error(self.h)
            raise ZkmiError(f"{what} failed ({rc}): {msg.decode() if msg else ''}")

    def sync(self):
        self._check(self.lib.zkmi_sync(self.h), "zkmi_sync")

    def stream(self) -> int:
        return self.lib.zkmi_stream(self.h) or 0

    def field_mul(self, which, a, b, out=None):
        n = a.shape[0]
        out = np.empty_like(a) if out is None else out
        self._check(self.lib.zkmi_field_mul(self.h, which, _ptr(a), _ptr(b), _ptr(out), n),
                    "zkmi_field_mul")
        return out

    def ff29_op(self, field, op, operands, out=None):
        n = operands.shape[0]
        out = np.empty((n, 9), dtype=np.int32) if out is None else out
        self._check(self.lib.zkmi_ff29_op(self.h, field, op, _ptr(operands), _ptr(out), n),
                    "zkmi_ff29_op")
        return out

    def field_mul_bench(self, which=1, n_threads=1 << 20, iters=256) -> float:
        r = C.c_double()
        self._check(self.lib.zkmi_field_mul_bench(self.h, which, n_threads, iters, C.byref(r)),
                    "zkmi_field_mul_bench")
        return r.value

    def ntt_batch(self, data, log_n, batch, inverse=False, coset=False):
        self._check(self.lib.zkmi_ntt_batch(self.h, _ptr(data), log_n, batch, int(inverse),
                                            int(coset)), "zkmi_ntt_batch")
        return data

    def h_batch(self, a, b, c, out, log_n, batch):
        self._check(self.lib.zkmi_h_batch(self.h, _ptr(a), _ptr(b), _ptr(c), _ptr(out), log_n,
                                          batch), "zkmi_h_batch")
        return out

    def ab_coset_batch(self, a, b, out, log_n, batch):
        self._check(self.lib.zkmi_ab_coset_batch(self.h, _ptr(a), _ptr(b), _ptr(out), log_n, batch),
                    "zkmi_ab_coset_batch")
        return out

    def quotient_bases(self, g1_z, log_n):
        n = 1 << log_n
        e, l = np.zeros((n, 8), dtype=np.uint64), np.zeros((n, 8), dtype=np.uint64)
        self._check(self.lib.zkmi_quotient_bases(self.h, _ptr(g1_z), g1_z.shape[0], log_n, _ptr(e),
                                                 _ptr(l)), "zkmi_quotient_bases")
        return e, l

    def msm_bases_load(self, group, bases, n, window_bits=0):
        h = C.c_void_p()
        self._check(self.lib.zkmi_msm_bases_load(self.h, group, _ptr(bases), n, window_bits,
                                                 C.byref(h)), "zkmi_msm_bases_load")
        return h

    def msm_bases_free(self, h):
        self.lib.zkmi_msm_bases_free(self.h, h)

    def msm_batch(self, bases_h, scalars, batch, out):
        self._check(self.lib.zkmi_msm_batch(self.h, bases_h, _ptr(scalars), batch, _ptr(out)),
                    "zkmi_msm_batch")
        return out

    def comb_min_groups_per_chunk(self):
        return int(self.lib.zkmi_comb_min_groups_per_chunk())

    def fixed_base_mul(self, group, base, scalars, n, out):
        self._check(self.lib.zkmi_fixed_base_mul(self.h, group, _ptr(base), _ptr(scalars), n,
                                                 _ptr(out)), "zkmi_fixed_base_mul")
        return out

    def pk_load(self, desc: PkDesc):
        h = C.c_void_p()
        self._check(self.lib.zkmi_pk_load(self.h, C.byref(desc), C.byref(h)), "zkmi_pk_load")
        return h

    def pk_info(self, h):
        arr = (C.c_uint64 * 10)()
        self._check(self.lib.zkmi_pk_info(h, arr), "zkmi_pk_info")
        return dict(zip(("g1_windows", "g1_entries_per_base", "g2_windows", "g2_entries_per_base",
                         "g1_table_bytes", "g2_table_bytes", "g1_shared", "g2_shared",
                         "g1_comb_k", "g2_comb_k"), [int(x) for x in arr]))

    def pk_folded(self, h) -> bool:
        return bool(self.lib.zkmi_pk_folded(h))

    def pk_free(self, h):
        self.lib.zkmi_pk_free(self.h, h)

    def cs_load(self, desc: CsDesc):
        h = C.c_void_p()
        self._check(self.lib.zkmi_cs_load(self.h, C.byref(desc), C.byref(h)), "zkmi_cs_load")
        return h

    def cs_free(self, h):
        self.lib.zkmi_cs_free(self.h, h)

    def solve_batch(self, cs_h, inputs, batch, wires_out=None, abc_out=None, status_out=None):
        if status_out is None:
            status_out = np.zeros(batch, dtype=np.int32)
        self._check(self.lib.zkmi_solve_batch(self.h, cs_h, _ptr(inputs), batch, _ptr(wires_out),
                                              _ptr(abc_out), _ptr(status_out)), "zkmi_solve_batch")
        return status_out

    def prove_batch(self, pk_h, cs_h, inputs, batch, rs, proofs_out, status_out):
        self._check(self.lib.zkmi_prove_batch(self.h, pk_h, cs_h, _ptr(inputs), batch, _ptr(rs),
                                              _ptr(proofs_out), _ptr(status_out)),
                    "zkmi_prove_batch")

    def prove_submit(self, pk_h, cs_h, inputs, batch, rs):
        self._check(self.lib.zkmi_prove_submit(self.h, pk_h, cs_h, _ptr(inputs), batch, _ptr(rs)),
                    "zkmi_prove_submit")

    def prove_collect(self, proofs_out, status_out, commitments_out=None):
        if commitments_out is None:
            self._check(self.lib.zkmi_prove_collect(self.h, _ptr(proofs_out), _ptr(status_out)),
                        "zkmi_prove_collect")
        else:
            self._check(self.lib.zkmi_prove_collect_ex(self.h, _ptr(proofs_out), _ptr(status_out),
                                                       _ptr(commitments_out)),
                        "zkmi_prove_collect_ex")

    def prove_witness_batch(self, pk_h, wires, a, b, c, n_constraints, batch, rs, proofs_out):
        self._check(self.lib.zkmi_prove_witness_batch(self.h, pk_h, _ptr(wires), _ptr(a), _ptr(b),
                                                      _ptr(c), n_constraints, batch, _ptr(rs),
                                                      _ptr(proofs_out)),
                    "zkmi_prove_witness_batch")

    def prove_witness_submit(self, pk_h, r1cs_h, wires, a, b, c, n_constraints, batch, rs):
        self._check(self.lib.zkmi_prove_witness_submit(self.h, pk_h, r1cs_h, _ptr(wires), _ptr(a),
                                                       _ptr(b), _ptr(c), n_constraints, batch,
                                                       _ptr(rs)), "zkmi_prove_witness_submit")

    def r1cs_load(self, desc: "R1csDesc"):
        h = C.c_void_p()
        self._check(self.lib.zkmi_r1cs_load(self.h, C.byref(desc), C.byref(h)), "zkmi_r1cs_load")
        return h

    def r1cs_free(self, h):
        self.lib.zkmi_r1cs_free(self.h, h)

    def r1cs_solver_load(self, r1cs_h, desc: "R1csSolverDesc"):
        h = C.c_void_p()
        self._check(self.lib.zkmi_r1cs_solver_load(self.h, r1cs_h, C.byref(desc), C.byref(h)),
                    "zkmi_r1cs_solver_load")
        return h

    def r1cs_solver_free(self, h):
        self.lib.zkmi_r1cs_solver_free(self.h, h)

    def r1cs_solver_info(self, h):
        arr = (C.c_uint64 * 8)()
        self._check(self.lib.zkmi_r1cs_solver_info(h, arr), "zkmi_r1cs_solver_info")
        return dict(zip(("n_instr", "lanes_per_proof", "n_terms", "longest", "n_inversions",
                         "n_wires", "n_constraints", "n_inputs"), [int(x) for x in arr]))

    def r1cs_solve_batch(self, solver_h, inputs, batch, wires_out=None, abc_out=None,
                         status_out=None):
        if status_out is None:
            status_out = np.zeros(batch, dtype=np.int32)
        self._check(self.lib.zkmi_r1cs_solve_batch(self.h, solver_h, _ptr(inputs), batch,
                                                   _ptr(wires_out), _ptr(abc_out),
                                                   _ptr(status_out)), "zkmi_r1cs_solve_batch")
        return status_out

    def prove_r1cs_submit(self, pk_h, solver_h, inputs, batch, rs):
        self._check(self.lib.zkmi_prove_r1cs_submit(self.h, pk_h, solver_h, _ptr(inputs), batch,
                                                    _ptr(rs)), "zkmi_prove_r1cs_submit")

    def host_alloc(self, shape, dtype=np.uint64):
        nbytes = int(np.prod(shape)) * np.dtype(dtype).itemsize
        p = self.lib.zkmi_host_alloc(self.h, nbytes)
        if not p:
            raise ZkmiError(f"zkmi_host_alloc({nbytes}) failed")
        buf = (C.c_uint8 * nbytes).from_address(p)
        arr = np.frombuffer(buf, dtype=dtype).reshape(shape)
        self._pinned = getattr(self, "_pinned", {})
        self._pinned[arr.ctypes.data] = p
        return arr

    def host_free(self, arr):
        p = getattr(self, "_pinned", {}).pop(arr.ctypes.data, None)
        if p:
            self.lib.zkmi_host_free(self.h, p)

    def set_copy_threads(self, n):
        self._check(self.lib.zkmi_set_copy_threads(self.h, n), "zkmi_set_copy_threads")

    def last_timings(self):
        arr = (C.c_double * 8)()
        self.lib.zkmi_last_timings(self.h, arr)
        return list(arr)
```

include/zkmi.h:

```cpp
#ifndef ZKMI_H
#define ZKMI_H
#include <stddef.h>
#include <stdint.h>

#ifdef __cplusplus
extern "C" {
#endif

typedef struct zkmi_ctx zkmi_ctx;
typedef struct zkmi_pk zkmi_pk;
typedef struct zkmi_cs zkmi_cs;
typedef struct zkmi_r1cs_desc zkmi_r1cs_desc;

enum zkmi_status {
  ZKMI_OK = 0,
  ZKMI_ERR_ARG = -1,
  ZKMI_ERR_HIP = -2,
  ZKMI_ERR_NO_DEVICE = -3,
  ZKMI_ERR_OOM = -4,
  ZKMI_ERR_UNSATISFIED = -5
};

int zkmi_init(int device, zkmi_ctx** out);
void zkmi_destroy(zkmi_ctx* ctx);
const char* zkmi_last_error(zkmi_ctx* ctx);
int zkmi_sync(zkmi_ctx* ctx);
void* zkmi_stream(zkmi_ctx* ctx);

int zkmi_field_mul(zkmi_ctx* ctx, int which, const void* a, const void* b, void* r, size_t n);
int zkmi_ff29_op(zkmi_ctx* ctx, int field, int op, const int32_t* in, int32_t* out, size_t n);
int zkmi_field_mul_bench(zkmi_ctx* ctx, int which, size_t n_threads, int iters, double* rate);

int zkmi_ntt_batch(zkmi_ctx* ctx, void* data, int log_n, size_t batch, int inverse, int coset);

int zkmi_h_batch(zkmi_ctx* ctx, const void* a, const void* b, const void* c, void* h_out,
                 int log_n, size_t batch);
int zkmi_ab_coset_batch(zkmi_ctx* ctx, const void* a, const void* b, void* out, int log_n,
                        size_t batch);
int zkmi_quotient_bases(zkmi_ctx* ctx, const void* g1_z, size_t n_z, int log_n, void* e_out,
                        void* l_out);

typedef struct zkmi_msm_bases zkmi_msm_bases;
int zkmi_msm_bases_load(zkmi_ctx* ctx, int group, const void* bases, size_t n, int window_bits,
                        zkmi_msm_bases** out);
void zkmi_msm_bases_free(zkmi_ctx* ctx, zkmi_msm_bases* b);
int zkmi_msm_batch(zkmi_ctx* ctx, const zkmi_msm_bases* bases, const void* scalars, size_t batch,
                   void* out);
uint32_t zkmi_comb_min_groups_per_chunk(void);
int zkmi_fixed_base_mul(zkmi_ctx* ctx, int group, const void* base, const void* scalars, size_t n,
                        void* out);

typedef struct {
  uint32_t n_private;
  uint32_t n_hashed;
  uint32_t commitment_wire;
  uint32_t reserved;
  const uint32_t* private_wires;
  const uint32_t* hashed_wires;
  const void* basis;
  const void* basis_exp_sigma;
} zkmi_commitment_desc;

typedef struct {
  uint32_t log_n;
  uint32_t n_wires;
  uint32_t n_a, n_b, n_k, n_z;
  const uint32_t* a_wire;
  const uint32_t* b_wire;
  const uint32_t* k_wire;
  const void* g1_a;
  const void* g1_b;
  const void* g1_k;
  const void* g1_z;
  const void* g2_b;
  const void* g1_alpha;
  const void* g1_beta;
  const void* g1_delta;
  const void* g2_beta;
  const void* g2_delta;
  uint32_t window_bits_g1;
  uint32_t window_bits_g2;
  const uint8_t* infinity_a;
  const uint8_t* infinity_b;
  uint32_t n_public;
  uint32_t max_batch;
  uint64_t table_budget_bytes;
  uint32_t n_slots_hint;
  uint32_t msm_chunk_factor;
  uint32_t sparse_witness;
  uint32_t n_commitments;
  const zkmi_commitment_desc* commitments;
  const zkmi_r1cs_desc* fold_r1cs;
} zkmi_pk_desc;
int zkmi_pk_load(zkmi_ctx* ctx, const zkmi_pk_desc* desc, zkmi_pk** out);
void zkmi_pk_free(zkmi_ctx* ctx, zkmi_pk* pk);
int zkmi_pk_info(const zkmi_pk* pk, uint64_t* info );
int zkmi_pk_folded(const zkmi_pk* pk);

typedef struct {
  uint32_t n_wires, n_public, n_secret, n_constraints;
  uint32_t n_slots, n_rows, n_consts;
  uint32_t lanes_per_proof;
  const uint32_t* program;
  const void* consts;
} zkmi_cs_desc;
int zkmi_cs_load(zkmi_ctx* ctx, const zkmi_cs_desc* desc, zkmi_cs** out);
void zkmi_cs_free(zkmi_ctx* ctx, zkmi_cs* cs);

int zkmi_solve_batch(zkmi_ctx* ctx, const zkmi_cs* cs, const void* inputs, size_t batch,
                     void* wires_out, void* abc_out, int32_t* status_out);

int zkmi_prove_batch(zkmi_ctx* ctx, const zkmi_pk* pk, const zkmi_cs* cs, const void* inputs,
                     size_t batch, const void* rs, void* proofs_out, int32_t* status_out);

int zkmi_prove_submit(zkmi_ctx* ctx, const zkmi_pk* pk, const zkmi_cs* cs, const void* inputs,
                      size_t batch, const void* rs);
int zkmi_prove_collect(zkmi_ctx* ctx, void* proofs_out, int32_t* status_out);
int zkmi_prove_collect_ex(zkmi_ctx* ctx, void* proofs_out, int32_t* status_out,
                          void* commitments_out);

void* zkmi_host_alloc(zkmi_ctx* ctx, size_t bytes);
void zkmi_host_free(zkmi_ctx* ctx, void* p);
int zkmi_set_copy_threads(zkmi_ctx* ctx, int threads);

typedef struct {
  uint32_t coeff;
  uint32_t wire;
} zkmi_term;
struct zkmi_r1cs_desc {
  uint32_t n_wires, n_constraints, n_coeffs;
  const void* coeffs;
  const uint32_t* l_ptr;
  const zkmi_term* l_terms;
  const uint32_t* r_ptr;
  const zkmi_term* r_terms;
  const uint32_t* o_ptr;
  const zkmi_term* o_terms;
};
typedef struct zkmi_r1cs zkmi_r1cs;
int zkmi_r1cs_load(zkmi_ctx* ctx, const zkmi_r1cs_desc* desc, zkmi_r1cs** out);
void zkmi_r1cs_free(zkmi_ctx* ctx, zkmi_r1cs* r1cs);

int zkmi_prove_witness_submit(zkmi_ctx* ctx, const zkmi_pk* pk, const zkmi_r1cs* r1cs,
                              const void* wires, const void* a, const void* b, const void* c,
                              size_t n_constraints, size_t batch, const void* rs);
int zkmi_prove_witness_batch(zkmi_ctx* ctx, const zkmi_pk* pk, const void* wires, const void* a,
                             const void* b, const void* c, size_t n_constraints, size_t batch,
                             const void* rs, void* proofs_out);

enum zkmi_hint_kind {
  ZKMI_HINT_INVZERO = 1,
  ZKMI_HINT_NBITS = 2,
  ZKMI_HINT_LIMBS = 3,
  ZKMI_HINT_COUNT = 4,
  ZKMI_HINT_COMMIT = 5,
  ZKMI_HINT_BYTEOP = 6
};
enum zkmi_hint_set {
  ZKMI_HINTS_BASIC = 0,
  ZKMI_HINTS_STD = 1
};
typedef struct {
  uint32_t n_public;
  uint32_t n_secret;
  uint32_t n_instr, n_hints;
  const uint32_t* instr;
  const uint32_t* hint_kind;
  const uint32_t* hint_in_ptr;
  const uint32_t* hint_lc_ptr;
  const zkmi_term* hint_terms;
  const uint32_t* hint_out_ptr;
  const uint32_t* hint_out;
  uint32_t lanes_per_proof;
  uint32_t hint_set;
} zkmi_r1cs_solver_desc;
typedef struct zkmi_r1cs_solver zkmi_r1cs_solver;
int zkmi_r1cs_solver_load(zkmi_ctx* ctx, const zkmi_r1cs* r1cs, const zkmi_r1cs_solver_desc* desc,
                          zkmi_r1cs_solver** out);
void zkmi_r1cs_solver_free(zkmi_ctx* ctx, zkmi_r1cs_solver* solver);
int zkmi_r1cs_solver_info(const zkmi_r1cs_solver* solver, uint64_t* info );
int zkmi_r1cs_solve_batch(zkmi_ctx* ctx, const zkmi_r1cs_solver* solver, const void* inputs,
                          size_t batch, void* wires_out, void* abc_out, int32_t* status_out);
int zkmi_prove_r1cs_submit(zkmi_ctx* ctx, const zkmi_pk* pk, const zkmi_r1cs_solver* solver,
                           const void* inputs, size_t batch, const void* rs);

typedef struct zkmi_plonk_pk zkmi_plonk_pk;
typedef struct {
  uint32_t log_n;
  uint32_t n_public;
  const void* coef;
  const void* coset;
  const void* sigma;
  const void* omega;
  const void* coset_x;
  const void* l1_coset;
  const void* zh_inv;
  const void* srs_g1;
  uint32_t window_bits;
  uint32_t max_batch;
  const void* lag_g1[3];
  const uint32_t* lag_rows[3];
  uint32_t lag_k;
} zkmi_plonk_pk_desc;
int zkmi_plonk_pk_load(zkmi_ctx* ctx, const zkmi_plonk_pk_desc* desc, zkmi_plonk_pk** out);
void zkmi_plonk_pk_free(zkmi_ctx* ctx, zkmi_plonk_pk* pk);
int zkmi_plonk_round1(zkmi_ctx* ctx, zkmi_plonk_pk* pk, const zkmi_cs* cs, const void* inputs,
                      size_t batch, const void* blind, void* commits_out, int32_t* status_out);
int zkmi_plonk_round2(zkmi_ctx* ctx, zkmi_plonk_pk* pk, const void* beta_gamma, void* commit_z_out);
int zkmi_plonk_round3(zkmi_ctx* ctx, zkmi_plonk_pk* pk, const void* alpha, void* commits_t_out);
int zkmi_plonk_round4(zkmi_ctx* ctx, zkmi_plonk_pk* pk, const void* zeta_zetaw, void* evals_out);
int zkmi_plonk_round5(zkmi_ctx* ctx, zkmi_plonk_pk* pk, const void* scalars, void* commits_w_out);

int zkmi_plonk_prove(zkmi_ctx* ctx, zkmi_plonk_pk* pk, const zkmi_cs* cs, const void* inputs,
                     size_t batch, const void* blind, const uint8_t* vk_digest, void* proofs_out,
                     int32_t* status_out);

int zkmi_last_timings(zkmi_ctx* ctx, double* ms_out );

#ifdef __cplusplus
}
#endif
#endif
```

Measured before the change: 8077.

## Fold scalar Montgomery factor into comb bases and share per-wire variance flags

Proving-key comb tables for A, B1, K and B2 are built from bases prescaled by a constant (an 'F image'), so signed comb MSMs can read the slot scalars directly instead of first running a scalar-conversion kernel into a separate buffer. Row-variance detection moves to a standalone kernel computed once per wire set and shared across the A/B1/K/B2 MSMs, and the Z MSM is marked dense so it skips variance detection. This removes repeated scalar-conversion passes and duplicated variance scans, at the cost of a more complex table-build path, a new row-index plumbing for digit extraction, and new API entry points.

```diff
diff --git a/gnark_crypto_primitives_amd/csrc/api.hip b/gnark_crypto_primitives_amd/csrc/api.hip
--- a/gnark_crypto_primitives_amd/csrc/api.hip
+++ b/gnark_crypto_primitives_amd/csrc/api.hip
@@ -366,7 +366,7 @@
     for (DevBuf* b : {&st.slots, &st.a, &st.b, &st.c, &st.misc, &st.sums, &st.commit})
       if (b->p) hipFree(b->p);
   for (DevBuf* b : {&ctx->ntt_tmp, &ctx->build_tmp, &ctx->msm_digits, &ctx->msm_sint,
-                    &ctx->msm_part[0], &ctx->msm_part[1], &ctx->side_part2, &ctx->side_part3})
+                    &ctx->msm_rowvar, &ctx->msm_part[0], &ctx->msm_part[1], &ctx->side_part2, &ctx->side_part3})
     if (b->p) hipFree(b->p);
   witness_ring_free(ctx);
   for (auto& e : ctx->ev)
@@ -541,9 +541,9 @@
 }
 
 static int bases_load_plan(zkmi_ctx* ctx, int group, const void* bases_dev, size_t n, WinPlan plan,
-                           bool may_relax, zkmi_msm_bases** out) {
+                           bool may_relax, zkmi_msm_bases** out, int image = MSM_IMAGE_STD) {
   for (;;) {
-    int rc = msm_bases_build(ctx, group, bases_dev, n, plan, out);
+    int rc = msm_bases_build(ctx, group, bases_dev, n, plan, out, image);
     if (rc != ZKMI_ERR_OOM || !may_relax) return rc;
     if (plan.comb) {
       if (plan.comb <= 8) return rc;
@@ -595,8 +595,17 @@
 
 int zkmi_msm_bases_load(zkmi_ctx* ctx, int group, const void* bases, size_t n, int window_bits,
                         zkmi_msm_bases** out) {
+  return zkmi_msm_bases_load_image(ctx, group, bases, n, window_bits, 0, out);
+}
+
+int zkmi_msm_bases_load_image(zkmi_ctx* ctx, int group, const void* bases, size_t n,
+                              int window_bits, int image, zkmi_msm_bases** out) {
   ZK_HIP(hipSetDevice(ctx->device));
   if (!out) return ZKMI_ERR_ARG;
+  if (image != 0 && image != 1) {
+    ctx->err = "image must be 0 (x * 2^256) or 1 (x * 2^261)";
+    return ZKMI_ERR_ARG;
+  }
   if (!window_bits_ok(window_bits)) {
     ctx->err = "window_bits must be 0 (auto), in [2,16], 100 + [4,16], 200 + [2,20] or 300 + [3,21]";
     return ZKMI_ERR_ARG;
@@ -622,7 +631,8 @@
       if ((double)COMB_W / k < (double)plan.W) plan = plan_comb(k, group == 1 ? s1 : s2);
     }
   }
-  return bases_load_plan(ctx, group, sb.dev, n, plan, window_bits == 0, out);
+  return bases_load_plan(ctx, group, sb.dev, n, plan, window_bits == 0, out,
+                         image ? MSM_IMAGE_F : MSM_IMAGE_STD);
 }
 
 void zkmi_msm_bases_free(zkmi_ctx* ctx, zkmi_msm_bases* b) {
@@ -655,6 +665,57 @@
     return rc;
   if ((rc = transpose_in(ctx, ss.dev, sbi, n, batch, Bp, 32))) return rc;
   if ((rc = msm_run(ctx, bases, (const Fr*)sbi, nullptr, Bp, batch, acc))) return rc;
+  if ((rc = xyzz_to_affine(ctx, bases->group, acc, aff, Bp))) return rc;
+  ZK_HIP(hipMemcpyAsync(so.dev, aff, batch * pt, hipMemcpyDeviceToDevice, ctx->stream));
+  if ((rc = so.finish())) return rc;
+  ZK_HIP(hipStreamSynchronize(ctx->stream));
+  return ZKMI_OK;
+}
+
+int zkmi_msm_batch_rows(zkmi_ctx* ctx, const zkmi_msm_bases* bases, const void* scalars,
+                        size_t n_rows, const uint32_t* row_idx, size_t batch, int image, int uniform,
+                        void* out) {
+  ZK_HIP(hipSetDevice(ctx->device));
+  int rc;
+  if ((rc = require_idle(ctx))) return rc;
+  if (batch == 0) return ZKMI_OK;
+  const size_t n = bases->n, Bp = round_up(batch, 64);
+  if ((image != 0 && image != 1) || uniform < 0 || uniform > 2 || n_rows == 0) {
+    ctx->err = "msm_batch_rows: image in {0, 1}, uniform in {0, 1, 2}, n_rows > 0";
+    return ZKMI_ERR_ARG;
+  }
+  std::vector<uint32_t> idx(n);
+  if (row_idx) {
+    if (n && hipMemcpy(idx.data(), row_idx, n * sizeof(uint32_t), hipMemcpyDefault) != hipSuccess) {
+      (void)hipGetLastError();
+      ctx->err = "msm_batch_rows: cannot read row_idx";
+      return ZKMI_ERR_ARG;
+    }
+  } else {
+    for (size_t i = 0; i < n; i++) idx[i] = (uint32_t)i;
+  }
+  for (uint32_t r : idx)
+    if (r >= n_rows) {
+      ctx->err = "msm_batch_rows: row_idx holds a row >= n_rows";
+      return ZKMI_ERR_ARG;
+    }
+  const size_t pt = bases->group == 1 ? 64 : 128;
+  Staged ss(ctx), so(ctx), si(ctx);
+  if ((rc = ss.in(scalars, batch * n_rows * 32)) || (rc = so.out(out, batch * pt)) ||
+      (rc = si.in(idx.data(), n * sizeof(uint32_t))))
+    return rc;
+  void *sbi, *acc, *aff, *flags = nullptr;
+  if ((rc = ensure_scratch(ctx, ctx->sets[0].a, n_rows * Bp * 32, &sbi)) ||
+      (rc = ensure_scratch(ctx, ctx->sets[0].b, Bp * pt * 2, &acc)) ||
+      (rc = ensure_scratch(ctx, ctx->sets[0].c, Bp * pt, &aff)))
+    return rc;
+  if ((rc = transpose_in(ctx, ss.dev, sbi, n_rows, batch, Bp, 32))) return rc;
+  if (uniform == 1 && ((rc = ensure_scratch(ctx, ctx->msm_rowvar, n_rows, &flags)) ||
+                       (rc = msm_rows_vary(ctx, (const Fr*)sbi, n_rows, Bp, batch, (uint8_t*)flags))))
+    return rc;
+  if ((rc = msm_run(ctx, bases, (const Fr*)sbi, (const uint32_t*)si.dev, Bp, batch, acc, image == 1,
+                    nullptr, nullptr, (const uint8_t*)flags, uniform == 2)))
+    return rc;
   if ((rc = xyzz_to_affine(ctx, bases->group, acc, aff, Bp))) return rc;
   ZK_HIP(hipMemcpyAsync(so.dev, aff, batch * pt, hipMemcpyDeviceToDevice, ctx->stream));
   if ((rc = so.finish())) return rc;
@@ -887,22 +948,24 @@
     }
   }
   auto load = [&](int group, const void* pts, size_t n, const WinPlan& plan, bool relax,
-                  zkmi_msm_bases** out) -> int {
+                  zkmi_msm_bases** out, int image) -> int {
     Staged sb(ctx);
     int r = sb.in(pts, n * (group == 1 ? 64 : 128));
     if (r) return r;
-    r = bases_load_plan(ctx, group, sb.dev, n, plan, relax, out);
+    r = bases_load_plan(ctx, group, sb.dev, n, plan, relax, out, image);
     if (!r) (*out)->chunk_factor = d->msm_chunk_factor;
     return r;
   };
   if ((rc = upload_u32(ctx, wa.data(), d->n_a, &pk->a_wire)) ||
       (rc = upload_u32(ctx, wb.data(), d->n_b, &pk->b_wire)) ||
       (rc = upload_u32(ctx, fold.folded ? fold.k_wire.data() : wk.data(), n_kb, &pk->k_wire)) ||
-      (rc = load(1, d->g1_a, d->n_a, p1, auto1, &pk->A)) ||
-      (rc = load(1, d->g1_b, d->n_b, p1, auto1, &pk->B1)) ||
-      (rc = load(1, fold.folded ? (const void*)fold.k.data() : d->g1_k, n_kb, p1, auto1, &pk->K)) ||
-      (rc = load(1, fold.folded ? (const void*)fold.e.data() : d->g1_z, n_zb, p1z, auto1, &pk->Z)) ||
-      (rc = load(2, d->g2_b, d->n_b, p2, auto2, &pk->B2))) {
+      (rc = load(1, d->g1_a, d->n_a, p1, auto1, &pk->A, MSM_IMAGE_F)) ||
+      (rc = load(1, d->g1_b, d->n_b, p1, auto1, &pk->B1, MSM_IMAGE_F)) ||
+      (rc = load(1, fold.folded ? (const void*)fold.k.data() : d->g1_k, n_kb, p1, auto1, &pk->K,
+                 MSM_IMAGE_F)) ||
+      (rc = load(1, fold.folded ? (const void*)fold.e.data() : d->g1_z, n_zb, p1z, auto1, &pk->Z,
+                 MSM_IMAGE_STD)) ||
+      (rc = load(2, d->g2_b, d->n_b, p2, auto2, &pk->B2, MSM_IMAGE_F))) {
     zkmi_pk_free(ctx, pk);
     return rc;
   }
@@ -1143,15 +1206,29 @@
   const bool d1 = pk->Z->plan.shared || pk->Z->plan.comb;
   const bool d2 = pk->B2->plan.shared || pk->B2->plan.comb;
   hipStream_t q3 = ctx->stream3;
-  if ((rc = msm_run(ctx, pk->A, slots, pk->a_wire, Bp, batch, v.sA, fd, d1 ? v.w1[0] : nullptr, q3)) ||
-      (rc = msm_run(ctx, pk->B1, slots, pk->b_wire, Bp, batch, v.sB1, fd, d1 ? v.w1[1] : nullptr, q3)) ||
-      (rc = msm_run(ctx, pk->K, slots, pk->k_wire, Bp, batch, v.sK, fd, d1 ? v.w1[2] : nullptr, q3)) ||
-      (rc = msm_run(ctx, pk->Z, h, nullptr, Bp, batch, v.sZ, false, d1 ? v.w1[3] : nullptr, q3))) {
+  uint8_t* rv = nullptr;
+  if (pk->A->plan.comb || pk->B2->plan.comb) {
+    void* p;
+    if ((rc = ensure_scratch(ctx, ctx->msm_rowvar, pk->n_wires, &p)) ||
+        (rc = msm_rows_vary(ctx, slots, pk->n_wires, Bp, batch, (uint8_t*)p))) {
+      ctx->msm_ev_set = -1;
+      return rc;
+    }
+    rv = (uint8_t*)p;
+  }
+  if ((rc = msm_run(ctx, pk->A, slots, pk->a_wire, Bp, batch, v.sA, fd, d1 ? v.w1[0] : nullptr, q3,
+                    rv)) ||
+      (rc = msm_run(ctx, pk->B1, slots, pk->b_wire, Bp, batch, v.sB1, fd, d1 ? v.w1[1] : nullptr, q3,
+                    rv)) ||
+      (rc = msm_run(ctx, pk->K, slots, pk->k_wire, Bp, batch, v.sK, fd, d1 ? v.w1[2] : nullptr, q3,
+                    rv)) ||
+      (rc = msm_run(ctx, pk->Z, h, nullptr, Bp, batch, v.sZ, false, d1 ? v.w1[3] : nullptr, q3,
+                    nullptr, true))) {
     ctx->msm_ev_set = -1;
     return rc;
   }
   hipEventRecord(S.evq[2], ctx->stream);
-  rc = msm_run(ctx, pk->B2, slots, pk->b_wire, Bp, batch, v.sB2, fd, d2 ? v.w2 : nullptr, q3);
+  rc = msm_run(ctx, pk->B2, slots, pk->b_wire, Bp, batch, v.sB2, fd, d2 ? v.w2 : nullptr, q3, rv);
   ctx->msm_ev_set = -1;
   if (rc) return rc;
   hipEventRecord(S.evq[3], ctx->stream);
diff --git a/gnark_crypto_primitives_amd/csrc/comb_sign.h b/gnark_crypto_primitives_amd/csrc/comb_sign.h
--- /dev/null
+++ b/gnark_crypto_primitives_amd/csrc/comb_sign.h
@@ -0,0 +1,27 @@
+#pragma once
+#include "ff.h"
+
+namespace zk {
+
+constexpr int COMB_SIGN_ONES = 253;
+constexpr int COMB_SIGN_PARITY = 254;
+
+ZK_HD int comb_sign_window(int word, int bit, bool* complement) {
+  const int q = word * 32 + bit;
+  *complement = q == 0;
+  if (q == 0) return COMB_SIGN_PARITY;
+  if (q <= COMB_SIGN_ONES) return q - 1;
+  return -1;
+}
+
+ZK_HD uint32_t comb_sign_bit(const uint32_t t[8], int j) {
+  if (j == COMB_SIGN_ONES) return 1u;
+  for (int w = 0; w < 8; w++)
+    for (int b = 0; b < 32; b++) {
+      bool comp;
+      if (comb_sign_window(w, b, &comp) == j) return ((t[w] >> b) & 1u) ^ (comp ? 1u : 0u);
+    }
+  return 0u;
+}
+
+}
diff --git a/gnark_crypto_primitives_amd/csrc/msm.hip b/gnark_crypto_primitives_amd/csrc/msm.hip
--- a/gnark_crypto_primitives_amd/csrc/msm.hip
+++ b/gnark_crypto_primitives_amd/csrc/msm.hip
@@ -99,12 +99,13 @@
   return plan_with_windows(64);
 }
 
-extern template int build_comb<Fq2>(zkmi_ctx*, const Affine<Fq2>*, size_t, const WinPlan&,
+extern template int build_comb<Fq2>(zkmi_ctx*, const Affine<Fq2>*, size_t, const WinPlan&, int,
                                     Affine<Fq2>*, int*, Affine<Fq2>*);
 extern template int build_impl<Fq2>(zkmi_ctx*, const Affine<Fq2>*, size_t, const WinPlan&,
                                     Affine<Fq2>*);
 extern template int run_impl<Fq2>(zkmi_ctx*, const zkmi_msm_bases*, const Fr*, const uint32_t*,
-                                  size_t, size_t, XYZZ<Fq2>*, bool, XYZZ<Fq2>*, hipStream_t);
+                                  size_t, size_t, XYZZ<Fq2>*, bool, XYZZ<Fq2>*, hipStream_t,
+                                  const uint8_t*, bool);
 
 template <class Fn>
 static auto by_group(int group, Fn&& fn) {
@@ -112,7 +113,7 @@
 }
 
 int msm_bases_build(zkmi_ctx* ctx, int group, const void* bases_dev, size_t n, const WinPlan& plan,
-                    zkmi_msm_bases** out) {
+                    zkmi_msm_bases** out, int image) {
   if (group != 1 && group != 2) {
     ctx->err = "group must be 1 (G1) or 2 (G2)";
     return ZKMI_ERR_ARG;
@@ -121,6 +122,7 @@
   b->group = group;
   b->n = n;
   b->plan = plan;
+  b->image = image;
   const size_t entry = group == 1 ? sizeof(G1Affine) : sizeof(G2Affine);
   b->n_groups = plan.comb ? (n + plan.comb - 1) / plan.comb : 0;
   b->table_bytes = plan.comb ? b->n_groups * ((size_t)1 << (plan.comb - plan.comb_signed)) * entry
@@ -148,7 +150,7 @@
     const Affine<F>* bases = (const Affine<F>*)bases_dev;
     hipLaunchKernelGGL((msm_inf_flags<F>), dim3((unsigned)((n + 255) / 256)), dim3(256), 0,
                        ctx->stream, bases, (uint32_t)n, b->inf);
-    return plan.comb ? build_comb<F>(ctx, bases, n, plan, (Affine<F>*)b->table,
+    return plan.comb ? build_comb<F>(ctx, bases, n, plan, image, (Affine<F>*)b->table,
                                      &b->entries_may_be_inf, &stotal_of(b, f))
                      : build_impl<F>(ctx, bases, n, plan, (Affine<F>*)b->table);
   });
@@ -193,7 +195,7 @@
 
 int msm_run(zkmi_ctx* ctx, const zkmi_msm_bases* bases, const Fr* scalars, const uint32_t* row_idx,
             size_t Bp, size_t batch, void* out_xyzz, bool scalars_f, void* wsum_out,
-            hipStream_t finish_stream) {
+            hipStream_t finish_stream, const uint8_t* row_varies, bool dense) {
   return by_group(bases->group, [&](auto f) -> int {
     using F = decltype(f);
     if (bases->n == 0) {
@@ -209,8 +211,17 @@
       return ZKMI_ERR_ARG;
     }
     return run_impl<F>(ctx, bases, scalars, row_idx, Bp, batch, (XYZZ<F>*)out_xyzz, scalars_f,
-                       (XYZZ<F>*)wsum_out, finish_stream);
-  });
+                       (XYZZ<F>*)wsum_out, finish_stream, row_varies, dense);
+  });
+}
+
+int msm_rows_vary(zkmi_ctx* ctx, const Fr* rows, size_t n_rows, size_t Bp, size_t batch,
+                  uint8_t* flags) {
+  if (n_rows == 0) return ZKMI_OK;
+  hipLaunchKernelGGL(rows_vary_kernel, dim3((unsigned)((n_rows + 3) / 4)), dim3(256), 0, ctx->stream,
+                     rows, (const uint32_t*)nullptr, (uint32_t)n_rows, Bp, batch, flags);
+  ZK_HIP(hipGetLastError());
+  return ZKMI_OK;
 }
 
 int xyzz_to_affine(zkmi_ctx* ctx, int group, const void* in, void* out, size_t n) {
diff --git a/gnark_crypto_primitives_amd/csrc/msm_g2.hip b/gnark_crypto_primitives_amd/csrc/msm_g2.hip
--- a/gnark_crypto_primitives_amd/csrc/msm_g2.hip
+++ b/gnark_crypto_primitives_amd/csrc/msm_g2.hip
@@ -2,10 +2,10 @@
 
 namespace zk {
 
-template int build_comb<Fq2>(zkmi_ctx*, const Affine<Fq2>*, size_t, const WinPlan&, Affine<Fq2>*,
-                             int*, Affine<Fq2>*);
+template int build_comb<Fq2>(zkmi_ctx*, const Affine<Fq2>*, size_t, const WinPlan&, int,
+                             Affine<Fq2>*, int*, Affine<Fq2>*);
 template int build_impl<Fq2>(zkmi_ctx*, const Affine<Fq2>*, size_t, const WinPlan&, Affine<Fq2>*);
 template int run_impl<Fq2>(zkmi_ctx*, const zkmi_msm_bases*, const Fr*, const uint32_t*, size_t,
-                           size_t, XYZZ<Fq2>*, bool, XYZZ<Fq2>*, hipStream_t);
+                           size_t, XYZZ<Fq2>*, bool, XYZZ<Fq2>*, hipStream_t, const uint8_t*, bool);
 
 }
diff --git a/gnark_crypto_primitives_amd/csrc/msm_impl.h b/gnark_crypto_primitives_amd/csrc/msm_impl.h
--- a/gnark_crypto_primitives_amd/csrc/msm_impl.h
+++ b/gnark_crypto_primitives_amd/csrc/msm_impl.h
@@ -1,6 +1,7 @@
 #pragma once
 #include "zkmi_internal.h"
 #include "ec29.h"
+#include "comb_sign.h"
 
 namespace zk {
 
@@ -351,6 +352,15 @@
   XYZZ<F> s = XYZZ<F>::inf();
   for (uint32_t g = 0; g < n_groups; g++) madd(s, gsum[g]);
   *out = to_affine(s);
+}
+
+template <class F>
+__global__ __launch_bounds__(64) void comb_scale_bases(const Affine<F>* __restrict__ bases,
+                                                       uint32_t n, Fr c,
+                                                       Affine<F>* __restrict__ out) {
+  const uint32_t i = blockIdx.x * blockDim.x + threadIdx.x;
+  if (i >= n) return;
+  out[i] = to_affine(scalar_mul(bases[i], c.v));
 }
 
 template <class F, bool SIGNED>
@@ -388,7 +398,7 @@
   for (uint32_t d = 0; d < seg_len; d++) {
     const bool is_inf = acc.is_inf();
     const uint32_t m = m0 + d;
-    inf_seen = inf_seen || (is_inf && (SIGNED ? live != 0 : (m != 0 && (m & ~live) == 0)));
+    inf_seen = inf_seen || (is_inf && (SIGNED || (m != 0 && (m & ~live) == 0)));
     if (is_inf)
       inv.push(seg, d, F::zero(), F::zero(), F::one(), F::one());
     else
@@ -400,58 +410,48 @@
   if (inf_seen) atomicOr(any_inf, 1);
 }
 
-template <bool SIGNED>
-__global__ __launch_bounds__(256) void comb_scalars_kernel(const Fr* __restrict__ scalars,
-                                                           const uint32_t* __restrict__ row_idx,
-                                                           size_t Bp, uint32_t n, int32_t kmul32,
-                                                           const uint8_t* __restrict__ inf,
-                                                           Fr* __restrict__ out, size_t batch,
-                                                           uint32_t k, uint32_t* __restrict__ gvar) {
+static __global__ __launch_bounds__(256) void comb_scalars_kernel(const Fr* __restrict__ scalars,
+                                                                  const uint32_t* __restrict__ row_idx,
+                                                                  size_t Bp, uint32_t n, Fr29 kk,
+                                                                  const uint8_t* __restrict__ inf,
+                                                                  Fr* __restrict__ out) {
   const size_t b = (size_t)blockIdx.x * blockDim.x + threadIdx.x;
   for (uint32_t i = blockIdx.y; i < n; i += gridDim.y) {
     Fr s = Fr::zero();
     if (!inf[i]) {
-      Fr29 kk = Fr29::zero();
-      kk.v[0] = kmul32;
       const uint32_t row = row_idx ? row_idx[i] : i;
       const Fr raw = bi_ld(scalars, row, b, Bp);
-      const Fr raw0 = bi_ld(scalars, row, 0, Bp);
-      uint32_t diff = 0;
-#pragma unroll
-      for (int l = 0; l < 8; l++) diff |= raw.v[l] ^ raw0.v[l];
-      if (__ballot(b < batch && diff != 0) != 0 && (threadIdx.x & 63u) == 0) gvar[i / k] = 1u;
       pack_canonical<Fr29Params>(s.v, mul(unpack29<Fr29Params>(raw.v), kk));
-      if (SIGNED) {
-        const uint32_t odd = s.v[0] & 1u;
-        uint64_t cy = 0;
-#pragma unroll
-        for (int l = 0; l < 8; l++) {
-          cy += (uint64_t)s.v[l] + (odd ? FrParams::p(l) : 0u);
-          s.v[l] = (uint32_t)cy;
-          cy >>= 32;
-        }
-#pragma unroll
-        for (int l = 0; l < 7; l++) s.v[l] = (s.v[l] >> 1) | (s.v[l + 1] << 31);
-        s.v[7] >>= 1;
-        const uint32_t e = (s.v[0] & 1u) ^ 1u;
-        s.v[0] &= ~1u;
-        cy = 0;
-#pragma unroll
-        for (int l = 0; l < 8; l++) {
-          cy += (uint64_t)s.v[l] + (l == 7 ? 0x40000000u : 0u);
-          s.v[l] = (uint32_t)cy;
-          cy >>= 32;
-        }
-#pragma unroll
-        for (int l = 0; l < 7; l++) s.v[l] = (s.v[l] >> 1) | (s.v[l + 1] << 31);
-        s.v[7] = (s.v[7] >> 1) | (e << 31);
-      }
     }
     bi_st(out, i, b, Bp, s);
   }
 }
 
-static __global__ __launch_bounds__(1024) void comb_split_kernel(const uint32_t* __restrict__ gvar,
+static __global__ __launch_bounds__(256) void rows_vary_kernel(const Fr* __restrict__ scalars,
+                                                               const uint32_t* __restrict__ row_idx,
+                                                               uint32_t n_rows, size_t Bp,
+                                                               size_t batch,
+                                                               uint8_t* __restrict__ flags) {
+  const uint32_t lane = threadIdx.x & 63u;
+  const uint32_t i = blockIdx.x * (blockDim.x >> 6) + (threadIdx.x >> 6);
+  if (i >= n_rows) return;
+  const uint32_t row = row_idx ? row_idx[i] : i;
+  const Fr raw0 = bi_ld(scalars, row, 0, Bp);
+  bool var = false;
+  for (size_t b0 = 0; b0 < batch && !var; b0 += 64) {
+    const size_t b = b0 + lane;
+    const Fr raw = bi_ld(scalars, row, b, Bp);
+    uint32_t diff = 0;
+#pragma unroll
+    for (int l = 0; l < 8; l++) diff |= raw.v[l] ^ raw0.v[l];
+    var = __ballot(b < batch && diff != 0) != 0;
+  }
+  if (lane == 0) flags[i] = var ? 1 : 0;
+}
+
+static __global__ __launch_bounds__(1024) void comb_split_kernel(const uint8_t* __restrict__ flags,
+                                                                 const uint32_t* __restrict__ flag_idx,
+                                                                 uint32_t n, uint32_t k, int dense,
                                                                  uint32_t n_groups,
                                                                  uint32_t* __restrict__ vlist,
                                                                  uint32_t* __restrict__ ulist,
@@ -463,7 +463,16 @@
   for (uint32_t g0 = 0; g0 < n_groups; g0 += 1024) {
     const uint32_t g = g0 + t;
     const bool live = g < n_groups;
-    const bool var = live && gvar[g] != 0;
+    bool var = live && dense;
+    if (live && !dense) {
+      uint32_t any = 0;
+#pragma unroll 8
+      for (uint32_t q = 0; q < k; q++) {
+        const size_t i = (size_t)g * k + q;
+        if (i < n) any |= flags[flag_idx ? flag_idx[i] : i];
+      }
+      var = any != 0;
+    }
     const unsigned long long vm = __ballot(var);
     if (lane == 0) wave_nv[w] = (uint32_t)__popcll(vm);
     __syncthreads();
@@ -492,8 +501,10 @@
 }
 
 template <int KMAX, bool SIGNED>
-__global__ __launch_bounds__(256) void comb_digits_kernel(const Fr* __restrict__ sint, size_t Bp,
-                                                          uint32_t n, uint32_t k, uint32_t n_groups,
+__global__ __launch_bounds__(256) __attribute__((amdgpu_waves_per_eu(3))) void comb_digits_kernel(const Fr* __restrict__ sint,
+                                                          const uint32_t* __restrict__ row_idx,
+                                                          size_t Bp, uint32_t n, uint32_t k,
+                                                          uint32_t n_groups,
                                                           const uint32_t* __restrict__ vpos,
                                                           uint32_t* __restrict__ digits,
                                                           uint32_t* __restrict__ d0) {
@@ -504,14 +515,24 @@
     const uint32_t p = vpos[g];
     const bool uni = p == ~0u;
     if (uni && (blockIdx.x != 0 || threadIdx.x >= 64)) continue;
+    if (SIGNED) {
+      if (!uni)
+        digits[((size_t)COMB_SIGN_ONES * n_groups + p) * Bp + b] = low;
+      else if (b == 0)
+        d0[(size_t)COMB_SIGN_ONES * n_groups + g] = low;
+    }
+    size_t rows[KMAX];
+#pragma unroll
+    for (int i = 0; i < KMAX; i++) {
+      const size_t bi = (size_t)g * k + i;
+      rows[i] = (i < (int)k && bi < n) ? (row_idx ? (size_t)row_idx[bi] : bi) : ~(size_t)0;
+    }
 #pragma unroll
     for (int h = 0; h < 2; h++) {
       uint4 wv[KMAX];
 #pragma unroll
-      for (int i = 0; i < KMAX; i++) {
-        const size_t bi = (size_t)g * k + i;
-        wv[i] = (i < (int)k && bi < n) ? base[(bi * 2 + h) * Bp + b] : make_uint4(0, 0, 0, 0);
-      }
+      for (int i = 0; i < KMAX; i++)
+        wv[i] = rows[i] != ~(size_t)0 ? base[(rows[i] * 2 + h) * Bp + b] : make_uint4(0, 0, 0, 0);
 #pragma unroll
       for (int c = 0; c < 4; c++) {
         uint32_t m[32];
@@ -532,13 +553,14 @@
 #pragma unroll
         for (int bit = 0; bit < 32; bit++) {
           int j = (h * 4 + c) * 32 + bit;
+          bool comp = false;
           if (SIGNED) {
-            if (j == 254) continue;
-            if (j == 255) j = 254;
+            j = comb_sign_window(h * 4 + c, bit, &comp);
+            if (j < 0) continue;
           } else if (j >= COMB_W) {
             break;
           }
-          uint32_t idx = m[bit];
+          uint32_t idx = comp ? ~m[bit] : m[bit];
           if (SIGNED) idx = ((idx >> (k - 1)) & 1u) ? (idx & low) : ((~idx & low) | 0x80000000u);
           if (!uni)
             digits[((size_t)j * n_groups + p) * Bp + b] = idx;
@@ -762,8 +784,15 @@
 template <class B> static auto& stotal_of(B* b, Fq) { return b->stotal1; }
 template <class B> static auto& stotal_of(B* b, Fq2) { return b->stotal2; }
 
-template <class F>
-int build_comb(zkmi_ctx* ctx, const Affine<F>* bases_dev, size_t n, const WinPlan& plan,
+static inline Fr comb_base_scale(int image) {
+  Fr x = Fr::one();
+  const int e = image == MSM_IMAGE_F ? 262 : 257;
+  for (int i = 0; i < e; i++) x = dbl(x);
+  return from_mont(inverse(x));
+}
+
+template <class F>
+int build_comb(zkmi_ctx* ctx, const Affine<F>* bases_dev, size_t n, const WinPlan& plan, int image,
                Affine<F>* table, int* any_inf_host, Affine<F>* stotal_host) {
   const uint32_t k = plan.comb;
   const bool sg = plan.comb_signed != 0;
@@ -776,12 +805,20 @@
   void* scratch;
   const size_t dp_bytes = round_up(n_groups * k * sizeof(Affine<F>), 256);
   const size_t gs_bytes = round_up((n_groups + 1) * sizeof(Affine<F>), 256);
-  int rc = ensure_scratch(ctx, ctx->build_tmp, dp_bytes + gs_bytes + 256 + slab.bytes, &scratch);
+  const size_t sc_bytes = sg ? round_up(n * sizeof(Affine<F>), 256) : 0;
+  int rc = ensure_scratch(ctx, ctx->build_tmp, dp_bytes + gs_bytes + 256 + slab.bytes + sc_bytes,
+                          &scratch);
   if (rc) return rc;
   Affine<F>* dpts = (Affine<F>*)scratch;
   Affine<F>* gsum = (Affine<F>*)((char*)scratch + dp_bytes);
   int* any_inf = (int*)((char*)scratch + dp_bytes + gs_bytes);
   F* inv_scratch = (F*)((char*)scratch + dp_bytes + gs_bytes + 256);
+  if (sg) {
+    Affine<F>* scaled = (Affine<F>*)((char*)inv_scratch + slab.bytes);
+    hipLaunchKernelGGL((comb_scale_bases<F>), dim3((unsigned)((n + 63) / 64)), dim3(64), 0,
+                       ctx->stream, bases_dev, (uint32_t)n, comb_base_scale(image), scaled);
+    bases_dev = scaled;
+  }
   ZK_HIP(hipMemsetAsync(any_inf, 0, sizeof(int), ctx->stream));
   hipLaunchKernelGGL((comb_prep<F>), dim3((unsigned)((n_groups + 63) / 64)), dim3(64), 0,
                      ctx->stream, bases_dev, (uint32_t)n, k, (uint32_t)n_groups, dpts, gsum,
@@ -896,7 +933,7 @@
 template <class F>
 int run_comb(zkmi_ctx* ctx, const zkmi_msm_bases* bases, const Fr* scalars, const uint32_t* row_idx,
              size_t Bp, size_t batch, XYZZ<F>* out, bool scalars_f, XYZZ<F>* wsum_out,
-             hipStream_t finish_stream) {
+             hipStream_t finish_stream, const uint8_t* row_varies, bool dense) {
   const size_t n = bases->n;
   const uint32_t k = bases->plan.comb;
   const bool sg = bases->plan.comb_signed != 0;
@@ -911,30 +948,46 @@
   if (rc) return rc;
   if ((rc = wait_partials_free(ctx, pb))) return rc;
   if ((rc = ensure_scratch(ctx, ctx->msm_digits,
-                           ((size_t)W * G * Bp + (size_t)(W + 4) * G) * sizeof(uint32_t),
+                           ((size_t)W * G * Bp + (size_t)(W + 3) * G) * sizeof(uint32_t) + n,
                            &digits)))
     return rc;
-  if ((rc = ensure_scratch(ctx, ctx->msm_sint, n * Bp * sizeof(Fr), &sint))) return rc;
   uint32_t* d0 = (uint32_t*)digits + (size_t)W * G * Bp;
-  uint32_t* gvar = d0 + (size_t)W * G;
-  uint32_t* vlist = gvar + G;
+  uint32_t* vlist = d0 + (size_t)W * G;
   uint32_t* ulist = vlist + G;
   uint32_t* vpos = ulist + G;
   const PartView<F> pv(part, cs, W, Bp);
   uint32_t* counts = pv.counts;
   XYZZ<F>* wsum = wsum_out ? wsum_out : pv.wsum;
   const unsigned bx = (Bp % 256 == 0) ? 256 : 64;
-  const dim3 sgrid((unsigned)(Bp / bx), (unsigned)(n < 16384 ? n : 16384));
   const dim3 dgrid((unsigned)(Bp / bx), (unsigned)(G < 8192 ? G : 8192));
-  const int32_t km = (int32_t)(scalars_f ? 1 : 32);
-  ZK_HIP(hipMemsetAsync(gvar, 0, G * sizeof(uint32_t), ctx->stream));
-  hipLaunchKernelGGL((sg ? comb_scalars_kernel<true> : comb_scalars_kernel<false>), sgrid, dim3(bx), 0,
-                     ctx->stream, scalars, row_idx, Bp, (uint32_t)n, km, (const uint8_t*)bases->inf,
-                     (Fr*)sint, batch, k, gvar);
-  hipLaunchKernelGGL(comb_split_kernel, dim3(1), dim3(1024), 0, ctx->stream, (const uint32_t*)gvar,
-                     (uint32_t)G, vlist, ulist, vpos, counts);
+  const uint8_t* flags = row_varies;
+  const uint32_t* flag_idx = row_idx;
+  if (!flags && !dense) {
+    uint8_t* own = (uint8_t*)(vpos + G);
+    hipLaunchKernelGGL(rows_vary_kernel, dim3((unsigned)((n + 3) / 4)), dim3(256), 0, ctx->stream,
+                       scalars, row_idx, (uint32_t)n, Bp, batch, own);
+    flags = own;
+    flag_idx = nullptr;
+  }
+  hipLaunchKernelGGL(comb_split_kernel, dim3(1), dim3(1024), 0, ctx->stream, flags, flag_idx,
+                     (uint32_t)n, k, dense ? 1 : 0, (uint32_t)G, vlist, ulist, vpos, counts);
+  const Fr* dsrc = scalars;
+  const uint32_t* didx = row_idx;
+  if (!(sg && scalars_f == (bases->image == MSM_IMAGE_F))) {
+    if ((rc = ensure_scratch(ctx, ctx->msm_sint, n * Bp * sizeof(Fr), &sint))) return rc;
+    Fr29 kk = Fr29::zero();
+    if (!sg)
+      kk.v[0] = scalars_f ? 1 : 32;
+    else
+      for (int i = 0; i < 9; i++) kk.v[i] = scalars_f ? Fr29Params::c256(i) : Fr29Params::c266(i);
+    const dim3 sgrid((unsigned)(Bp / bx), (unsigned)(n < 16384 ? n : 16384));
+    hipLaunchKernelGGL(comb_scalars_kernel, sgrid, dim3(bx), 0, ctx->stream, scalars, row_idx, Bp,
+                       (uint32_t)n, kk, (const uint8_t*)bases->inf, (Fr*)sint);
+    dsrc = (const Fr*)sint;
+    didx = nullptr;
+  }
   hipLaunchKernelGGL((sg ? comb_digits_kernel<21, true> : comb_digits_kernel<20, false>), dgrid,
-                     dim3(bx), 0, ctx->stream, (const Fr*)sint, Bp, (uint32_t)n, k, (uint32_t)G,
+                     dim3(bx), 0, ctx->stream, dsrc, didx, Bp, (uint32_t)n, k, (uint32_t)G,
                      (const uint32_t*)vpos, (uint32_t*)digits, d0);
   const hipEvent_t timed = acc_timer_begin(ctx, bases);
   const dim3 grid((unsigned)(Bp / bx), (unsigned)W, (unsigned)cs.chunks);
@@ -1061,10 +1114,10 @@
 template <class F>
 int run_impl(zkmi_ctx* ctx, const zkmi_msm_bases* bases, const Fr* scalars,
              const uint32_t* row_idx, size_t Bp, size_t batch, XYZZ<F>* out, bool scalars_f,
-             XYZZ<F>* wsum_out, hipStream_t finish_stream) {
+             XYZZ<F>* wsum_out, hipStream_t finish_stream, const uint8_t* row_varies, bool dense) {
   if (bases->plan.comb)
     return run_comb<F>(ctx, bases, scalars, row_idx, Bp, batch, out, scalars_f, wsum_out,
-                       finish_stream);
+                       finish_stream, row_varies, dense);
   if (bases->plan.shared)
     return run_shared<F>(ctx, bases, scalars, row_idx, Bp, out, scalars_f, wsum_out);
   if (wsum_out) {
diff --git a/gnark_crypto_primitives_amd/csrc/zkmi_internal.h b/gnark_crypto_primitives_amd/csrc/zkmi_internal.h
--- a/gnark_crypto_primitives_amd/csrc/zkmi_internal.h
+++ b/gnark_crypto_primitives_amd/csrc/zkmi_internal.h
@@ -45,6 +45,7 @@
   zk::DevBuf ntt_tmp;
   zk::DevBuf build_tmp;
   zk::DevBuf msm_digits, msm_sint;
+  zk::DevBuf msm_rowvar;
   zk::DevBuf msm_part[2];
   zk::DevBuf side_part2;
   zk::DevBuf side_part3;
@@ -104,6 +105,7 @@
   size_t n_groups = 0;
   int entries_may_be_inf = 0;
   uint32_t chunk_factor = 0;
+  int image = 0;
   zk::G1Affine stotal1 = {};
   zk::G2Affine stotal2 = {};
   int side = 0;
@@ -277,11 +279,15 @@
 void plan_comb_for_budget(size_t n1, size_t n2, double usable_bytes, int* k1, int* k2, bool* sg1,
                           bool* sg2, bool allow_signed = true);
 void plan_shared_for_budget(size_t n1, size_t n2, double usable_bytes, int* c1, int* c2);
+enum { MSM_IMAGE_STD = 0, MSM_IMAGE_F = 1 };
 int msm_bases_build(zkmi_ctx* ctx, int group, const void* bases_dev, size_t n, const WinPlan& plan,
-                    zkmi_msm_bases** out);
+                    zkmi_msm_bases** out, int image = MSM_IMAGE_STD);
 int msm_run(zkmi_ctx* ctx, const zkmi_msm_bases* bases, const Fr* scalars, const uint32_t* row_idx,
             size_t Bp, size_t batch, void* out_xyzz, bool scalars_f = false,
-            void* wsum_out = nullptr, hipStream_t finish_stream = nullptr);
+            void* wsum_out = nullptr, hipStream_t finish_stream = nullptr,
+            const uint8_t* row_varies = nullptr, bool dense = false);
+int msm_rows_vary(zkmi_ctx* ctx, const Fr* rows, size_t n_rows, size_t Bp, size_t batch,
+                  uint8_t* flags);
 int msm_horner_run(zkmi_ctx* ctx, hipStream_t stream, int count,
                    const zkmi_msm_bases* const* bases, void* const* wsums, void* const* outs,
                    size_t Bp);
diff --git a/gnark_crypto_primitives_amd/lib.py b/gnark_crypto_primitives_amd/lib.py
--- a/gnark_crypto_primitives_amd/lib.py
+++ b/gnark_crypto_primitives_amd/lib.py
@@ -81,6 +81,8 @@
     ("zkmi_msm_bases_load", _I, [_P, _I, _P, _SZ, _I, C.POINTER(_P)]),
     ("zkmi_msm_bases_free", None, [_P, _P]),
     ("zkmi_msm_batch", _I, [_P, _P, _P, _SZ, _P]),
+    ("zkmi_msm_bases_load_image", _I, [_P, _I, _P, _SZ, _I, _I, C.POINTER(_P)]),
+    ("zkmi_msm_batch_rows", _I, [_P, _P, _P, _SZ, _P, _SZ, _I, _I, _P]),
     ("zkmi_comb_min_groups_per_chunk", C.c_uint32, []),
     ("zkmi_fixed_base_mul", _I, [_P, _I, _P, _P, _SZ, _P]),
     ("zkmi_pk_load", _I, [_P, C.POINTER(PkDesc), C.POINTER(_P)]),
@@ -240,6 +242,19 @@
                     "zkmi_msm_batch")
         return out
 
+    def msm_bases_load_image(self, group, bases, n, window_bits, image):
+        h = C.c_void_p()
+        self._check(self.lib.zkmi_msm_bases_load_image(self.h, group, _ptr(bases), n, window_bits,
+                                                       image, C.byref(h)),
+                    "zkmi_msm_bases_load_image")
+        return h
+
+    def msm_batch_rows(self, bases_h, scalars, n_rows, row_idx, batch, image, uniform, out):
+        self._check(self.lib.zkmi_msm_batch_rows(self.h, bases_h, _ptr(scalars), n_rows,
+                                                 _ptr(row_idx), batch, image, uniform, _ptr(out)),
+                    "zkmi_msm_batch_rows")
+        return out
+
     def comb_min_groups_per_chunk(self):
         return int(self.lib.zkmi_comb_min_groups_per_chunk())
 
diff --git a/include/zkmi.h b/include/zkmi.h
--- a/include/zkmi.h
+++ b/include/zkmi.h
@@ -46,6 +46,11 @@
 void zkmi_msm_bases_free(zkmi_ctx* ctx, zkmi_msm_bases* b);
 int zkmi_msm_batch(zkmi_ctx* ctx, const zkmi_msm_bases* bases, const void* scalars, size_t batch,
                    void* out);
+int zkmi_msm_bases_load_image(zkmi_ctx* ctx, int group, const void* bases, size_t n,
+                              int window_bits, int image, zkmi_msm_bases** out);
+int zkmi_msm_batch_rows(zkmi_ctx* ctx, const zkmi_msm_bases* bases, const void* scalars,
+                        size_t n_rows, const uint32_t* row_idx, size_t batch, int image, int uniform,
+                        void* out);
 uint32_t zkmi_comb_min_groups_per_chunk(void);
 int zkmi_fixed_base_mul(zkmi_ctx* ctx, int group, const void* base, const void* scalars, size_t n,
                         void* out);
```

Result: faster. 8184, median of 6 (+1.3%).
